# samson6460/tf2_YOLO

Hardware: AMD Instinct MI355X
Metric: images/sec training YOLOv3 416x416 bs=32/GPU (higher is better)
Workload: dtype f32-storage/fp16x2-mfma

## Files before the change

include/yolo_hip.h:

```cpp
#ifndef YOLO_HIP_H_
#define YOLO_HIP_H_

#include <stddef.h>
#include <stdint.h>

#ifdef __cplusplus
extern "C" {
#endif

typedef enum yolo_status {
  YOLO_OK = 0,
  YOLO_ERR_INVALID_ARG = -1,
  YOLO_ERR_LAUNCH = -2,
  YOLO_ERR_WORKSPACE = -3
} yolo_status;

enum { YOLO_ACT_LINEAR = 0, YOLO_ACT_LEAKY = 1, YOLO_ACT_MISH = 2 };
enum { YOLO_HEAD_V3 = 3, YOLO_HEAD_V2 = 2, YOLO_HEAD_V1 = 1, YOLO_HEAD_V4 = 4 };
enum { YOLO_NMS_HARD = 1, YOLO_NMS_SOFT = 2, YOLO_NMS_DIOU = 3 };

const char* yolo_last_error(void);
int yolo_abi_version(void);
int yolo_device_available(void);
int yolo_mfma_probe(const void* operands_f16, float* sink, int workgroups, int iters, double* flops_host, void* stream);

enum { YOLO_OPT_CONV_WIN = 0, YOLO_OPT_STAMPS = 1, YOLO_OPT_CONV_SK = 2, YOLO_OPT_CONV_PATCH = 5, YOLO_OPT_WGRAD_WIN = 6,
       YOLO_OPT_NMS_WALK = 7 ,
       YOLO_OPT_AB = 8  };
int yolo_set_option(int key, int value);
const char* yolo_last_conv_kernel(int* launches_host);
size_t yolo_conv_workspace_bytes(void);
int yolo_set_conv_workspace(void* p, size_t bytes, void* stream);
int yolo_set_debug_buffer(void* p, size_t bytes);

typedef struct yolo_conv_desc {
  int N, H, W, Cin;
  int Cout, kh, kw;
  int Ho, Wo;
  int sh, sw;
  int pad_t, pad_l;
} yolo_conv_desc;

#define YOLO_BN_STAT_SLOTS 64
#define YOLO_BN_RED_SLOTS 512
#define YOLO_SPLIT_BATCH_UNITS 4

int yolo_conv2d_fwd(const yolo_conv_desc* d, const float* x, const float* w,
                    const float* bias, float* y, double* stats, void* stream);
int yolo_conv2d_fwd_absmax(const yolo_conv_desc* d, const float* x, const float* w, const float* bias,
                           float* y, double* stats, unsigned* absmax, void* stream);

int yolo_conv2d_dgrad(const yolo_conv_desc* d, const float* dy, const float* wT,
                      float* dx, int accumulate, void* stream);

int yolo_conv2d_wgrad(const yolo_conv_desc* d, const float* x, const float* dy,
                      float* dw, float* dbias, void* stream);

int yolo_conv2d_wgrad_bias(const float* dy, long long P, int Cout, float* dbias, void* stream);

int yolo_filter_transpose(const float* w, float* wT, int Cout, int taps, int Cin, void* stream);

size_t yolo_planes_bytes(long long rows, int C);
int yolo_split_planes(const float* x, long long rows, int C, void* planes, void* stream);
int yolo_split_planes_padded(const float* x, long long rows, int C_src, int C, void* planes, void* stream);

int yolo_split_planes_batch(const void* jobs, int njobs, long long total_blocks, void* stream);
int yolo_filter_transpose_batch(const void* jobs, int njobs, long long total_blocks, void* stream);

int yolo_conv2d_fwd_planes(const yolo_conv_desc* d, const void* x_planes, const void* w_planes,
                           const float* bias, float* y, double* stats, unsigned* absmax, void* stream);
int yolo_conv2d_dgrad_planes(const yolo_conv_desc* d, const void* dy_planes, const void* wT_planes,
                             float* dx, int accumulate, void* stream);
enum { YOLO_EPI_NONE = 0, YOLO_EPI_AFFINE = 1, YOLO_EPI_AFFINE_LEAKY = 2, YOLO_EPI_AFFINE_MISH = 3 };
int yolo_conv2d_fwd_planes_epi(const yolo_conv_desc* d, const void* x_planes, const void* w_planes, const float* bias,
                               int epilogue, const float* scale, const float* shift, const float* residual, float* y,
                               unsigned* absmax, void* stream);
int yolo_split_planes_absmax(const float* x, long long rows, int C, const unsigned* absmax, const float* extra_bound,
                             void* planes, float* out_bound, void* stream);
#define YOLO_INFER_BOUND_WORDS 4096
int yolo_conv_pred_bound(const float* w, int Cout, int kdim, const float* scale, const float* shift, const float* bias,
                         float* pred2, void* stream);
int yolo_conv2d_fwd_infer_unit(const yolo_conv_desc* d, const void* x_planes, const void* w_planes, const float* bias,
                               int epilogue, const float* scale, const float* shift, const float* residual, float* y,
                               unsigned* absmax, const float* pred2, const void* in_bound, int in_n,
                               const void* residual_bound, int residual_n, void* out_planes, unsigned* out_words,
                               float* out_bound, int* out_n_host, void* stream);
int yolo_fold_bound(const void* words, int n, float* out_bound, void* stream);
int yolo_absmax_words(const float* x, long long n, unsigned* words, int* n_words_host, void* stream);
int yolo_stem_filter_prep(const float* w, const float* bias, float* wt, void* stream);
int yolo_stem_fwd_infer_unit(const yolo_conv_desc* d, const float* x, const float* wt, int epilogue, const float* scale,
                             const float* shift, const float* pred2, const void* in_bound, int in_n, float* y,
                             void* out_planes, unsigned* out_words, int* out_n_host, void* stream);
int yolo_split_planes_concat(const float* const* srcs_host, const int* channels_host, const float* const* bounds_host,
                             int nsrc, long long rows, void* planes, float* dst32, float* out_bound, void* stream);
int yolo_split_planes_concat_ex(const float* const* srcs_host, const int* channels_host, const float* const* bounds_host,
                                const int* bound_words_host, const int* upsample_host, int H, int W, int nsrc,
                                long long rows, void* planes, float* dst32, float* out_bound, void* stream);
int yolo_conv2d_fwd_head_unit(const yolo_conv_desc* d, const void* x_planes, const void* w_planes, const float* bias,
                              int A, int C, int version, const float* anchors, float* t, float* y, void* stream);
enum { YOLO_PREC_F32 = 0, YOLO_PREC_F16 = 1 };
int yolo_conv2d_fwd_planes_ex(const yolo_conv_desc* d, const void* x_planes, const void* w_planes, const float* bias,
                              float* y, double* stats, unsigned* absmax, int precision, void* stream);
int yolo_conv2d_fwd_planes_epi_ex(const yolo_conv_desc* d, const void* x_planes, const void* w_planes, const float* bias,
                                  int epilogue, const float* scale, const float* shift, const float* residual, float* y,
                                  unsigned* absmax, int precision, void* stream);
int yolo_conv2d_fwd_infer_unit_ex(const yolo_conv_desc* d, const void* x_planes, const void* w_planes, const float* bias,
                                  int epilogue, const float* scale, const float* shift, const float* residual, float* y,
                                  unsigned* absmax, const float* pred2, const void* in_bound, int in_n,
                                  const void* residual_bound, int residual_n, void* out_planes, unsigned* out_words,
                                  float* out_bound, int* out_n_host, int precision, void* stream);
int yolo_conv2d_fwd_head_unit_ex(const yolo_conv_desc* d, const void* x_planes, const void* w_planes, const float* bias,
                                 int A, int C, int version, const float* anchors, float* t, float* y, int precision,
                                 void* stream);
int yolo_conv2d_wgrad_planes(const yolo_conv_desc* d, const void* x_planes, const void* dy_planes,
                             float* dw, void* stream);

size_t yolo_wgrad_workspace_bytes(void);
int yolo_set_wgrad_workspace(void* p, size_t bytes);


int yolo_bn_stats(const float* x, long long P, int C, double* stats, void* stream);

int yolo_bn_finalize(double* stats, long long P, int C, const float* gamma, const float* beta,
                     float eps, float momentum, int unbiased_moving_var,
                     float* moving_mean, float* moving_var,
                     float* scale, float* shift, float* save_mean, float* save_invstd,
                     void* stream);

int yolo_bn_fold_inference(int C, const float* gamma, const float* beta,
                           const float* moving_mean, const float* moving_var, float eps,
                           float* scale, float* shift, void* stream);

int yolo_bn_act_fwd(const float* x, long long P, int C, const float* scale, const float* shift,
                    int act, const float* residual, float* out, void* stream);

int yolo_bn_act_bwd_reduce(const float* x, const float* dout, long long P, int C,
                           const float* scale, const float* shift,
                           const float* save_mean, const float* save_invstd,
                           int act, double* red, void* stream);
int yolo_bn_act_bwd_apply(const float* x, const float* dout, long long P, int C,
                          const float* gamma, const float* scale, const float* shift,
                          const float* save_mean, const float* save_invstd,
                          int act, double* red, float* dgamma, float* dbeta,
                          float* dx, void* stream);

int yolo_bn_finalize_bound(double* stats, long long P, int C, const float* gamma, const float* beta, float eps,
                           float momentum, int unbiased_moving_var, float* moving_mean, float* moving_var,
// ... 18 lines not shown
int yolo_bn_act_bwd_reduce_bound(const float* x, const float* dout, long long P, int C, const float* scale,
                                 const float* shift, const float* save_mean, const float* save_invstd,
                                 int act, double* red, unsigned* bound_aux, void* stream);
size_t yolo_stem_bwd_scratch_bytes(void);
int yolo_stem_bn_bwd_wgrad(const yolo_conv_desc* d, const float* y, const float* dout, const float* image, const float* scale,
                           const float* shift, const float* save_mean, const float* save_invstd, int act, const double* red,
                           float* dgamma, float* dbeta, float* dw, void* scratch, size_t scratch_bytes, void* stream);
int yolo_bn_act_bwd_apply_planes(const float* x, const float* dout, long long P, int C, const float* gamma,
                                 const float* scale, const float* shift, const float* save_mean,
                                 const float* save_invstd, int act, double* red, float* dgamma, float* dbeta,
                                 float* dx, void* planes, const unsigned* bound_aux, void* stream);
int yolo_bn_act_bwd_reduce_bound_ld(const float* x, const float* dout, long long ld_dout, long long P, int C,
                                    const float* scale, const float* shift, const float* save_mean,
                                    const float* save_invstd, int act, double* red, unsigned* bound_aux, void* stream);
#define YOLO_BN_FOLD_TICKET_WORDS 36
int yolo_bn_act_bwd_reduce_fold_ld(const float* x, const float* dout, long long ld_dout, long long P, int C,
                                   const float* scale, const float* shift, const float* save_mean,
                                   const float* save_invstd, int act, double* red, unsigned* bound_aux,
                                   unsigned* tickets, void* stream);
int yolo_bn_act_bwd_apply_planes_ld(const float* x, const float* dout, long long ld_dout, long long P, int C,
                                    const float* gamma, const float* scale, const float* shift, const float* save_mean,
                                    const float* save_invstd, int act, double* red, float* dgamma, float* dbeta,
                                    float* dx, void* planes, const unsigned* bound_aux, void* stream);

int yolo_bnred_slots_cap(const yolo_conv_desc* d);
int yolo_conv2d_dgrad_planes_bnred(const yolo_conv_desc* d, const void* dy_planes, const void* wT_planes, float* dx,
                                   int accumulate, const float* y, const float* scale, const float* shift,
                                   const float* save_mean, const float* save_invstd, int act, float* partials,
                                   int slots_cap, unsigned* bound_aux, int* nslots, void* stream);
int yolo_bn_act_bwd_sum_partials(const float* partials, int nslots, long long P, int C, const float* scale, double* red,
                                 unsigned* bound_aux, void* stream);

int yolo_act_fwd(const float* x, long long n, int act, float* out, void* stream);
int yolo_act_bwd(const float* x, const float* dout, long long n, int act, float* dx, void* stream);

int yolo_copy_channels_in(const float* src, long long P, int Csrc, float* dst, int Cdst,
                          int c_off, void* stream);
int yolo_copy_channels_out(const float* src, long long P, int Csrc, int c_off, float* dst,
                           int Cdst, int accumulate, void* stream);
int yolo_upsample2x_fwd(const float* x, int N, int H, int W, int C, float* y, int Cy, int c_off,
                        void* stream);
int yolo_upsample2x_bwd(const float* dy, int N, int H, int W, int C, int Cy, int c_off, float* dx,
                        int accumulate, void* stream);
int yolo_axpy(float* a, const float* b, long long n, void* stream);
int yolo_maxpool_fwd(const float* x, int N, int H, int W, int C, int k, int s, int pad_t, int pad_l,
                     int Ho, int Wo, float* y, int Cy, int c_off, int* argmax, void* stream);
int yolo_maxpool_bwd(const float* dy, int N, int Ho, int Wo, int C, int Cy, int c_off,
                     const int* argmax, float* dx, void* stream);
int yolo_maxpool_bwd_same(const float* dy, int N, int H, int W, int C, int Cy, int c_off, const int* argmax, int k,
                          int pad_t, int pad_l, float* dx, void* stream);
int yolo_maxpool2x2_bwd(const float* dy, int N, int Ho, int Wo, int C, const int* argmax, float* dx, int accumulate,
                        void* stream);
int yolo_space_to_depth2_fwd(const float* x, int N, int H, int W, int C, float* y, int Cy, int c_off,
                             void* stream);
int yolo_space_to_depth2_bwd(const float* dy, int N, int H, int W, int C, int Cy, int c_off, float* dx,
                             int accumulate, void* stream);

int yolo_head_act_fwd(const float* t, long long P, int A, int C, int version,
                      const float* anchors, float* y, void* stream);
int yolo_head_act_bwd(const float* y, const float* dy, long long P, int A, int C, int version,
                      const float* anchors, float* dt, float* danchors, void* stream);

typedef struct yolo_loss_cfg {
  int version;
  int N, gh, gw, A, C;
  float anchors[32];
  int   use_anchors;
  float binary_weight;
  float loss_weight[4];
  float ignore_thresh;
  int   use_focal_loss;
  float focal_gamma;
  int   use_scale;
  float wh_reg_weight;
  float truth_thresh;
  float label_smooth;
} yolo_loss_cfg;

size_t yolo_loss_workspace_bytes(const yolo_loss_cfg* cfg);
int yolo_loss_fwd_bwd(const yolo_loss_cfg* cfg, const float* y_true, const float* y_pred,
                      double* loss_out, float* dpred, float grad_scale,
                      void* workspace, size_t workspace_bytes, void* stream);

int yolo_metrics(const yolo_loss_cfg* cfg, const float* y_true, const float* y_pred,
                 float recall_thresh, double* out, void* stream);

int yolo_gap_fwd(const float* x, int N, int H, int W, int C, float* g, void* stream);
int yolo_gap_bwd(const float* dg, int N, int H, int W, int C, float* dx, int accumulate, void* stream);
int yolo_dense_softmax_fwd(const float* g, const float* W, const float* b, int N, int C, int K, float* logits, float* p,
                           void* stream);
int yolo_dense_softmax_bwd(const float* dp, const float* p, const float* g, const float* W, int N, int C, int K, float* dz,
                           float* dg, float* dW, float* db, void* stream);
int yolo_cce_fwd_bwd(const float* t, const float* p, int N, int K, double* loss_out, float* dpred, float grad_scale,
                     void* stream);
int yolo_bn_act_any_fwd(const float* y, long long P, int C, const float* gamma, const float* beta, float* moving_mean,
                        float* moving_var, const float* mean_offset, float eps, float momentum, int unbiased_moving_var,
                        int training, int act, float* scale, float* shift, float* save_mean, float* save_invstd, float* out,
                        void* stream);
int yolo_bn_act_any_bwd(const float* y, const float* dout, long long P, int C, const float* gamma, const float* scale,
                        const float* shift, const float* save_mean, const float* save_invstd, int act, float* dgamma,
                        float* dbeta, float* dy, void* stream);
int yolo_categorical_accuracy(const float* t, const float* p, int N, int K, double* out, void* stream);

int yolo_adam_step(float* p, float* g, float* m, float* v, long long n, float lr, float beta1,
                   float beta2, float eps, int step, float grad_scale, int zero_grad, void* stream);
float yolo_adam_lr_t(float lr, float beta1, float beta2, int step);
int yolo_adam_step_dev(float* p, float* g, float* m, float* v, long long n, const float* hyper, int zero_grad, void* stream);
int yolo_sgd_step(float* p, float* g, long long n, float lr, float grad_scale, int zero_grad,
                  void* stream);
int yolo_fill(float* p, long long n, float value, void* stream);

size_t yolo_grad_sqnorm_workspace_bytes(int n_chunks);
int yolo_grad_sqnorm(const float* g, const long long* chunk_off, const int* chunk_len, int n_chunks,
                     const int* var_first, int n_vars, double* var_sq, double* total_sq, void* workspace,
                     size_t workspace_bytes, void* stream);
int yolo_clip_factors(const double* var_sq, int n_vars, const double* total_sq, const double* total_sq_extra,
                      const float* hyper, int mode, float* factors, float* norm_out, void* stream);
int yolo_adam_step_clip(float* p, float* g, float* m, float* v, float* vhat, const long long* chunk_off,
                        const int* chunk_len, const int* chunk_var, int n_chunks, const float* hyper,
                        const float* factors, int clip_mode, int zero_grad, void* stream);
int yolo_sgd_step_clip(float* p, float* g, float* accum, int nesterov, const long long* chunk_off,
                       const int* chunk_len, const int* chunk_var, int n_chunks, const float* hyper,
                       const float* factors, int clip_mode, int zero_grad, void* stream);

int yolo_decode_level(const float* pred, int gh, int gw, int A, int C, int version,
                      float threshold, double* rows_out, int max_rows, int* count,
                      void* workspace, size_t workspace_bytes, void* stream);
int yolo_decode_level_f64(const double* pred, int gh, int gw, int A, int C, int version,
                          double threshold, double* rows_out, int max_rows, int* count,
                          void* workspace, size_t workspace_bytes, void* stream);
size_t yolo_decode_workspace_bytes(int gh, int gw, int A, int C);

size_t yolo_nms_workspace_bytes(int n, int class_num);
int yolo_nms(const double* rows, int n, int class_num, int mode, double nms_threshold,
             double conf_threshold, double sigma, unsigned char* keep_out,
             void* workspace, size_t workspace_bytes, void* stream);
int yolo_nms_select(const double* rows, int n, int class_num, int mode, double nms_threshold, double conf_threshold,
                    double sigma, unsigned char* keep_out, double* rows_out, int* count_out, void* workspace,
                    size_t workspace_bytes, void* stream);

size_t yolo_decode_batch_workspace_bytes(int levels, const int* gh, const int* gw, const int* A, int C, int B);
int yolo_decode_batch_count(const void* const* preds, const int* is_f64, int levels, int B, const int* gh, const int* gw,
                            const int* A, int C, int version, const double* thresholds, int* img_off, void* workspace,
                            size_t workspace_bytes, void* stream);
int yolo_decode_batch_write(const void* const* preds, const int* is_f64, int levels, int B, const int* gh, const int* gw,
                            const int* A, int C, int version, const double* thresholds, double* rows_out, int max_rows,
                            void* workspace, size_t workspace_bytes, void* stream);
size_t yolo_nms_batch_workspace_bytes(int n, int B, int class_num);
int yolo_nms_batch_prepare(const double* rows, int n, const int* img_off, int B, int class_num, long long* mask_words_out,
                           void* workspace, size_t workspace_bytes, void* stream);
int yolo_nms_batch_select(const double* rows, int n, int B, int class_num, int mode, double nms_threshold,
                          double conf_threshold, double sigma, void* mask, long long mask_words, unsigned char* keep_out,
                          double* rows_out, int* kept_off_out, void* workspace, size_t workspace_bytes, void* stream);

int yolo_cal_iou(const void* xywh_true, const void* xywh_pred, void* out, void* out2, int is_f64, int mode, int ndim,
                 const long long* shape_host, const long long* true_strides_host, const long long* pred_strides_host,
                 double grid_w, double grid_h, void* stream);


int yolo_match_detections(const double* gt_rows, int ngt, const double* det_rows, int ndet, int class_num,
                          double iou_threshold, int* best_gt, unsigned char* matched, double* best_iou,
                          unsigned char* gt_flags, long long* class_counts, void* stream);

int yolo_rank_desc(const double* key, const int* segment, int n, int* rank, void* stream);

size_t yolo_pr_curve_workspace_bytes(int n, int num_gts);
// ... 21 lines not shown
```

tf2_yolo_amd/_lib.py:

```python
import ctypes
import os
from ctypes import (POINTER, Structure, c_char_p, c_double, c_float, c_int, c_longlong,
                    c_size_t, c_void_p)

from . import tape as _tape

_HERE = os.path.dirname(os.path.abspath(__file__))
LIB_PATH = os.path.join(_HERE, "libyolo_hip.so")

ACT_LINEAR, ACT_LEAKY, ACT_MISH = 0, 1, 2
PREC_F32, PREC_F16 = 0, 1
_PRECISIONS = {"fp32": PREC_F32, "fp16": PREC_F16}


def precision_enum(precision):
    try:
        return _PRECISIONS[precision]
    except (KeyError, TypeError):
        raise ValueError(f"precision must be 'fp32' or 'fp16', got {precision!r}") from None
NMS_HARD, NMS_SOFT, NMS_DIOU = 1, 2, 3


class YoloHipError(RuntimeError):
    pass


class ConvDesc(Structure):
    _fields_ = [(n, c_int) for n in
                ("N", "H", "W", "Cin", "Cout", "kh", "kw", "Ho", "Wo", "sh", "sw", "pad_t", "pad_l")]


class LossCfg(Structure):
    _fields_ = [("version", c_int), ("N", c_int), ("gh", c_int), ("gw", c_int), ("A", c_int),
                ("C", c_int), ("anchors", c_float * 32), ("use_anchors", c_int),
                ("binary_weight", c_float), ("loss_weight", c_float * 4),
                ("ignore_thresh", c_float), ("use_focal_loss", c_int), ("focal_gamma", c_float),
                ("use_scale", c_int), ("wh_reg_weight", c_float), ("truth_thresh", c_float),
                ("label_smooth", c_float)]


_P = c_void_p
_LL = c_longlong
SIGNATURES = {
    "yolo_last_error": (c_char_p, []),
    "yolo_abi_version": (c_int, []),
    "yolo_device_available": (c_int, []),
    "yolo_set_option": (c_int, [c_int, c_int]),
    "yolo_last_conv_kernel": (c_char_p, [POINTER(c_int)]),
    "yolo_mfma_probe": (c_int, [_P, _P, c_int, c_int, POINTER(c_double), _P]),
    "yolo_set_debug_buffer": (c_int, [_P, c_size_t]),
    "yolo_encode_labels": (c_int, [_P, _P, _P, c_int, c_double, c_double, c_int, c_int, c_int, _P, _P, _P]),
    "yolo_down2xlabel": (c_int, [_P, c_int, c_int, c_int, c_int, _P, _P, _P]),
    "yolo_conv_workspace_bytes": (c_size_t, []),
    "yolo_set_conv_workspace": (c_int, [_P, c_size_t, _P]),
    "yolo_conv2d_fwd": (c_int, [POINTER(ConvDesc), _P, _P, _P, _P, _P, _P]),
    "yolo_conv2d_dgrad": (c_int, [POINTER(ConvDesc), _P, _P, _P, c_int, _P]),
    "yolo_conv2d_wgrad": (c_int, [POINTER(ConvDesc), _P, _P, _P, _P, _P]),
    "yolo_conv2d_wgrad_bias": (c_int, [_P, _LL, c_int, _P, _P]),
    "yolo_filter_transpose": (c_int, [_P, _P, c_int, c_int, c_int, _P]),
    "yolo_planes_bytes": (c_size_t, [_LL, c_int]),
    "yolo_split_planes": (c_int, [_P, _LL, c_int, _P, _P]),
    "yolo_split_planes_padded": (c_int, [_P, _LL, c_int, c_int, _P, _P]),
    "yolo_split_planes_batch": (c_int, [_P, c_int, _LL, _P]),
    "yolo_filter_transpose_batch": (c_int, [_P, c_int, _LL, _P]),
    "yolo_conv2d_fwd_planes": (c_int, [POINTER(ConvDesc), _P, _P, _P, _P, _P, _P, _P]),
    "yolo_stem_bwd_scratch_bytes": (c_size_t, []),
    "yolo_stem_bn_bwd_wgrad": (c_int, [POINTER(ConvDesc), _P, _P, _P, _P, _P, _P, _P, c_int, _P, _P, _P, _P, _P, c_size_t, _P]),
    "yolo_conv2d_fwd_planes_epi": (c_int, [POINTER(ConvDesc), _P, _P, _P, c_int, _P, _P, _P, _P, _P, _P]),
    "yolo_split_planes_absmax": (c_int, [_P, _LL, c_int, _P, _P, _P, _P, _P]),
    "yolo_conv_pred_bound": (c_int, [_P, c_int, c_int, _P, _P, _P, _P, _P]),
    "yolo_conv2d_fwd_infer_unit": (c_int, [POINTER(ConvDesc), _P, _P, _P, c_int, _P, _P, _P, _P, _P, _P, _P, c_int, _P, c_int,
                                           _P, _P, _P, POINTER(c_int), _P]),
    "yolo_fold_bound": (c_int, [_P, c_int, _P, _P]),
    "yolo_absmax_words": (c_int, [_P, _LL, _P, POINTER(c_int), _P]),
    "yolo_stem_filter_prep": (c_int, [_P, _P, _P, _P]),
    "yolo_stem_fwd_infer_unit": (c_int, [POINTER(ConvDesc), _P, _P, c_int, _P, _P, _P, _P, c_int, _P, _P, _P, POINTER(c_int), _P]),
    "yolo_split_planes_concat": (c_int, [POINTER(c_void_p), POINTER(c_int), POINTER(c_void_p), c_int, _LL, _P, _P, _P, _P]),
    "yolo_split_planes_concat_ex": (c_int, [POINTER(c_void_p), POINTER(c_int), POINTER(c_void_p), POINTER(c_int), POINTER(c_int),
                                            c_int, c_int, c_int, _LL, _P, _P, _P, _P]),
    "yolo_conv2d_fwd_head_unit": (c_int, [POINTER(ConvDesc), _P, _P, _P, c_int, c_int, c_int, _P, _P, _P, _P]),
    "yolo_conv2d_fwd_planes_ex": (c_int, [POINTER(ConvDesc), _P, _P, _P, _P, _P, _P, c_int, _P]),
    "yolo_conv2d_fwd_planes_epi_ex": (c_int, [POINTER(ConvDesc), _P, _P, _P, c_int, _P, _P, _P, _P, _P, c_int, _P]),
    "yolo_conv2d_fwd_infer_unit_ex": (c_int, [POINTER(ConvDesc), _P, _P, _P, c_int, _P, _P, _P, _P, _P, _P, _P, c_int, _P, c_int,
                                              _P, _P, _P, POINTER(c_int), c_int, _P]),
    "yolo_conv2d_fwd_head_unit_ex": (c_int, [POINTER(ConvDesc), _P, _P, _P, c_int, c_int, c_int, _P, _P, _P, c_int, _P]),
    "yolo_conv2d_fwd_absmax": (c_int, [POINTER(ConvDesc), _P, _P, _P, _P, _P, _P, _P]),
    "yolo_conv2d_dgrad_planes": (c_int, [POINTER(ConvDesc), _P, _P, _P, c_int, _P]),
    "yolo_conv2d_wgrad_planes": (c_int, [POINTER(ConvDesc), _P, _P, _P, _P]),
    "yolo_wgrad_workspace_bytes": (c_size_t, []),
    "yolo_set_wgrad_workspace": (c_int, [_P, c_size_t]),
    "yolo_bn_stats": (c_int, [_P, _LL, c_int, _P, _P]),
    "yolo_bn_finalize": (c_int, [_P, _LL, c_int, _P, _P, c_float, c_float, c_int, _P, _P, _P, _P, _P, _P, _P]),
    "yolo_bn_fold_inference": (c_int, [c_int, _P, _P, _P, _P, c_float, _P, _P, _P]),
    "yolo_bn_act_fwd": (c_int, [_P, _LL, c_int, _P, _P, c_int, _P, _P, _P]),
    "yolo_bn_act_bwd_reduce": (c_int, [_P, _P, _LL, c_int, _P, _P, _P, _P, c_int, _P, _P]),
    "yolo_bn_act_bwd_apply": (c_int, [_P, _P, _LL, c_int, _P, _P, _P, _P, _P, c_int, _P, _P, _P, _P, _P]),
    "yolo_bn_act_fwd_planes": (c_int, [_P, _LL, c_int, _P, _P, c_int, _P, _P, _P, _P, _P, _P, _P]),
    "yolo_bn_act_fwd_res_planes": (c_int, [_P, _LL, c_int, _P, _P, c_int, _P, _P, _P, _P, _P, _P]),
    "yolo_bn_act_bwd_apply_planes": (c_int, [_P, _P, _LL, c_int, _P, _P, _P, _P, _P, c_int, _P, _P, _P, _P, _P, _P,
                                             _P]),
    "yolo_bn_infer_bound": (c_int, [c_int, _P, _P, _P, _P, _P]),
    "yolo_bn_finalize_bound": (c_int, [_P, _LL, c_int, _P, _P, c_float, c_float, c_int, _P, _P, _P, _P, _P, _P, _P,
                                       _P, _P]),
    "yolo_bn_finalize_offset": (c_int, [_P, _LL, c_int, _P, _P, c_float, c_float, c_int, _P, _P, _P, _P, _P, _P, _P,
                                        _P, _P, _P]),
    "yolo_bn_act_bwd_reduce_bound": (c_int, [_P, _P, _LL, c_int, _P, _P, _P, _P, c_int, _P, _P, _P]),
    "yolo_bn_act_bwd_reduce_bound_ld": (c_int, [_P, _P, _LL, _LL, c_int, _P, _P, _P, _P, c_int, _P, _P, _P]),
    "yolo_bn_act_bwd_reduce_fold_ld": (c_int, [_P, _P, _LL, _LL, c_int, _P, _P, _P, _P, c_int, _P, _P, _P, _P]),
    "yolo_bn_act_bwd_apply_planes_ld": (c_int, [_P, _P, _LL, _LL, c_int, _P, _P, _P, _P, _P, c_int, _P, _P, _P, _P, _P, _P,
                                                _P]),
    "yolo_bnred_slots_cap": (c_int, [POINTER(ConvDesc)]),
    "yolo_conv2d_dgrad_planes_bnred": (c_int, [POINTER(ConvDesc), _P, _P, _P, c_int, _P, _P, _P, _P, _P, c_int, _P, c_int, _P,
                                               POINTER(c_int), _P]),
    "yolo_bn_act_bwd_sum_partials": (c_int, [_P, c_int, _LL, c_int, _P, _P, _P, _P]),
    "yolo_allreduce_bucket": (c_int, [_P, _P, _LL, _P]),
    "yolo_act_fwd": (c_int, [_P, _LL, c_int, _P, _P]),
    "yolo_act_bwd": (c_int, [_P, _P, _LL, c_int, _P, _P]),
    "yolo_copy_channels_in": (c_int, [_P, _LL, c_int, _P, c_int, c_int, _P]),
    "yolo_copy_channels_out": (c_int, [_P, _LL, c_int, c_int, _P, c_int, c_int, _P]),
    "yolo_upsample2x_fwd": (c_int, [_P, c_int, c_int, c_int, c_int, _P, c_int, c_int, _P]),
    "yolo_upsample2x_bwd": (c_int, [_P, c_int, c_int, c_int, c_int, c_int, c_int, _P, c_int, _P]),
    "yolo_axpy": (c_int, [_P, _P, _LL, _P]),
    "yolo_maxpool_fwd": (c_int, [_P, c_int, c_int, c_int, c_int, c_int, c_int, c_int, c_int, c_int, c_int,
                                 _P, c_int, c_int, _P, _P]),
    "yolo_maxpool_bwd": (c_int, [_P, c_int, c_int, c_int, c_int, c_int, c_int, _P, _P, _P]),
    "yolo_maxpool2x2_bwd": (c_int, [_P, c_int, c_int, c_int, c_int, _P, _P, c_int, _P]),
    "yolo_bn_act_maxpool2x2_fwd": (c_int, [_P, c_int, c_int, c_int, c_int, _P, _P, c_int, _P, _P, _P, _P, _P, _P]),
    "yolo_maxpool_bwd_same": (c_int, [_P, c_int, c_int, c_int, c_int, c_int, c_int, _P, c_int, c_int, c_int, _P, _P]),
    "yolo_space_to_depth2_fwd": (c_int, [_P, c_int, c_int, c_int, c_int, _P, c_int, c_int, _P]),
    "yolo_space_to_depth2_bwd": (c_int, [_P, c_int, c_int, c_int, c_int, c_int, c_int, _P, c_int, _P]),
    "yolo_head_act_fwd": (c_int, [_P, _LL, c_int, c_int, c_int, _P, _P, _P]),
    "yolo_head_act_bwd": (c_int, [_P, _P, _LL, c_int, c_int, c_int, _P, _P, _P, _P]),
    "yolo_loss_workspace_bytes": (c_size_t, [POINTER(LossCfg)]),
    "yolo_loss_fwd_bwd": (c_int, [POINTER(LossCfg), _P, _P, _P, _P, c_float, _P, c_size_t, _P]),
    "yolo_metrics": (c_int, [POINTER(LossCfg), _P, _P, c_float, _P, _P]),
    "yolo_gap_fwd": (c_int, [_P, c_int, c_int, c_int, c_int, _P, _P]),
    "yolo_gap_bwd": (c_int, [_P, c_int, c_int, c_int, c_int, _P, c_int, _P]),
    "yolo_dense_softmax_fwd": (c_int, [_P, _P, _P, c_int, c_int, c_int, _P, _P, _P]),
    "yolo_dense_softmax_bwd": (c_int, [_P, _P, _P, _P, c_int, c_int, c_int, _P, _P, _P, _P, _P]),
    "yolo_bn_act_any_fwd": (c_int, [_P, _LL, c_int, _P, _P, _P, _P, _P, c_float, c_float, c_int, c_int, c_int, _P, _P, _P, _P, _P,
                                    _P]),
    "yolo_bn_act_any_bwd": (c_int, [_P, _P, _LL, c_int, _P, _P, _P, _P, _P, c_int, _P, _P, _P, _P]),
    "yolo_cce_fwd_bwd": (c_int, [_P, _P, c_int, c_int, _P, _P, c_float, _P]),
    "yolo_categorical_accuracy": (c_int, [_P, _P, c_int, c_int, _P, _P]),
    "yolo_adam_step": (c_int, [_P, _P, _P, _P, _LL, c_float, c_float, c_float, c_float, c_int, c_float, c_int, _P]),
    "yolo_adam_lr_t": (c_float, [c_float, c_float, c_float, c_int]),
    "yolo_adam_step_dev": (c_int, [_P, _P, _P, _P, _LL, _P, c_int, _P]),
    "yolo_sgd_step": (c_int, [_P, _P, _LL, c_float, c_float, c_int, _P]),
    "yolo_fill": (c_int, [_P, _LL, c_float, _P]),
    "yolo_grad_sqnorm_workspace_bytes": (c_size_t, [c_int]),
    "yolo_grad_sqnorm": (c_int, [_P, _P, _P, c_int, _P, c_int, _P, _P, _P, c_size_t, _P]),
    "yolo_clip_factors": (c_int, [_P, c_int, _P, _P, _P, c_int, _P, _P, _P]),
    "yolo_adam_step_clip": (c_int, [_P, _P, _P, _P, _P, _P, _P, _P, c_int, _P, _P, c_int, c_int, _P]),
    "yolo_sgd_step_clip": (c_int, [_P, _P, _P, c_int, _P, _P, _P, c_int, _P, _P, c_int, c_int, _P]),
    "yolo_decode_level": (c_int, [_P, c_int, c_int, c_int, c_int, c_int, c_float, _P, c_int, _P, _P, c_size_t, _P]),
    "yolo_decode_level_f64": (c_int, [_P, c_int, c_int, c_int, c_int, c_int, c_double, _P, c_int, _P, _P,
                                      c_size_t, _P]),
    "yolo_decode_workspace_bytes": (c_size_t, [c_int, c_int, c_int, c_int]),
    "yolo_nms_workspace_bytes": (c_size_t, [c_int, c_int]),
    "yolo_cal_iou": (c_int, [_P, _P, _P, _P, c_int, c_int, c_int, POINTER(c_longlong), POINTER(c_longlong),
                             POINTER(c_longlong), c_double, c_double, _P]),
    "yolo_match_detections": (c_int, [_P, c_int, _P, c_int, c_int, c_double, _P, _P, _P, _P, _P, _P]),
    "yolo_rank_desc": (c_int, [_P, _P, c_int, _P, _P]),
    "yolo_pr_curve_workspace_bytes": (c_size_t, [c_int, c_int]),
    "yolo_pr_curve": (c_int, [_P, _P, _P, c_int, c_int, c_int, _P, c_size_t, _P, _P, _P]),
    "yolo_nms": (c_int, [_P, c_int, c_int, c_int, c_double, c_double, c_double, _P, _P, c_size_t, _P]),
    "yolo_nms_select": (c_int, [_P, c_int, c_int, c_int, c_double, c_double, c_double, _P, _P, _P, _P, c_size_t, _P]),
    "yolo_decode_batch_workspace_bytes": (c_size_t, [c_int, POINTER(c_int), POINTER(c_int), POINTER(c_int), c_int, c_int]),
    "yolo_decode_batch_count": (c_int, [POINTER(c_void_p), POINTER(c_int), c_int, c_int, POINTER(c_int), POINTER(c_int),
                                        POINTER(c_int), c_int, c_int, POINTER(c_double), _P, _P, c_size_t, _P]),
    "yolo_decode_batch_write": (c_int, [POINTER(c_void_p), POINTER(c_int), c_int, c_int, POINTER(c_int), POINTER(c_int),
                                        POINTER(c_int), c_int, c_int, POINTER(c_double), _P, c_int, _P, c_size_t, _P]),
    "yolo_nms_batch_workspace_bytes": (c_size_t, [c_int, c_int, c_int]),
    "yolo_nms_batch_prepare": (c_int, [_P, c_int, _P, c_int, c_int, _P, _P, c_size_t, _P]),
    "yolo_nms_batch_select": (c_int, [_P, c_int, c_int, c_int, c_int, c_double, c_double, c_double, _P, _LL, _P, _P, _P, _P,
                                      c_size_t, _P]),
    "yolo_image_prepare": (c_int, [_P, _LL, _P, c_int, c_int, c_int, c_float, c_float, _P, _P]),
}

_lib = None

_QUERIES = {"yolo_last_error", "yolo_last_conv_kernel", "yolo_abi_version", "yolo_bnred_slots_cap", "yolo_device_available", "yolo_conv_workspace_bytes", "yolo_planes_bytes",
            "yolo_stem_bwd_scratch_bytes", "yolo_loss_workspace_bytes", "yolo_decode_workspace_bytes",
            "yolo_nms_workspace_bytes", "yolo_pr_curve_workspace_bytes", "yolo_wgrad_workspace_bytes", "yolo_adam_lr_t",
            "yolo_grad_sqnorm_workspace_bytes", "yolo_decode_batch_workspace_bytes", "yolo_nms_batch_workspace_bytes",
            "yolo_set_option", "yolo_set_debug_buffer", "yolo_set_conv_workspace", "yolo_set_wgrad_workspace"}


class _Recorded:
    __slots__ = ("f", "name")

    def __init__(self, f, name):
        self.f, self.name = f, name

    def __call__(self, *a):
        rc = self.f(*a)
        if _tape.ACTIVE is not None:
            _tape.ACTIVE.c(self.f, a, self.name)
        return rc


class _Lib:

    def __init__(self, cdll):
        self._cdll = cdll

    def __getattr__(self, name):
        f = getattr(self._cdll, name)
        if name not in _QUERIES and name in SIGNATURES:
            f = _Recorded(f, name)
        setattr(self, name, f)
        return f


def load():
    global _lib
    if _lib is not None:
# ... 26 lines not shown
```

tf2_yolo_amd/capture.py:

```python
import torch

from ._lib import YoloHipError


_LEAKED = []


class _StaticInputs:

    def __init__(self, x, y_list):
        self.x = x.clone()
        self.ys = [y.clone() for y in y_list]
        self._last = [(x, x._version)] + [(y, y._version) for y in y_list]

    def load(self, x, y_list):
        for i, (dst, src) in enumerate(zip([self.x] + self.ys, [x] + list(y_list))):
            last, ver = self._last[i]
            if src is last and src._version == ver:
                continue
            dst.copy_(src, non_blocking=True)
            self._last[i] = (src, src._version)


class StepGraphs:

    def __init__(self, model, x, y_list):
        self.model = model
        self.key = self.key_of(model, x)
        net = model.net
        opt = model.optimizer
        if not getattr(opt, "capturable", False):
            raise YoloHipError("this optimizer has no capturable form")
        self.inputs = _StaticInputs(x, y_list)
        self.x, self.ys = self.inputs.x, self.inputs.ys
        self.segments = []
        opt._hyper_buffers()
        net.mark_params_changed()
        torch.cuda.synchronize()
        self._capture(net, opt)

    @staticmethod
    def key_of(model, x):
        return (tuple(x.shape), getattr(model.net, "alloc_gen", 0), tuple(id(l) for l in model.loss), id(model.optimizer),
                id(model._reducer), model.net.anchors_trainable)

    def _capture(self, net, opt):
        model = self.model
        red = model._reducer if (model._reducer is not None and model._reducer.active) else None
        pool = torch.cuda.graph_pool_handle()
        stream = torch.cuda.Stream()
        stream.wait_stream(torch.cuda.current_stream())
        state = {"g": None}

        def begin():
            g = torch.cuda.CUDAGraph()
            g.capture_begin(pool=pool, capture_error_mode="thread_local")
            state["g"] = g

        def end(action):
            state["g"].capture_end()
            self.segments.append((state["g"], action))
            state["g"] = None

        net._dyp_events = [None, None]
        net._wp_event = net._wT_event = None
        old_hook, old_overlap = net.grad_ready_hook, net._overlap_wgrad
        net._overlap_wgrad = False
        if red is not None:
            index = model._dp_unit_index

            def cut_hook(u):
                for b in red.closes[index[id(u)]]:
                    net._join_wgrad()
                    net._dyp_events = [None, None]
                    end(("reduce", b))
                    begin()
            net.grad_ready_hook = cut_hook
        try:
            with torch.cuda.stream(stream):
                begin()
                outs = net.forward(self.x, training=True)
                for i, (o, yt) in enumerate(zip(outs, self.ys)):
                    model.loss[i].fwd_bwd(yt, o, grad_scale=1.0, dpred=model._dpred[i], loss_out=model._loss_bufs[i])
                net.backward(model._dpred)
                net._dyp_events = [None, None]
                if red is not None:
                    end(("finish",))
                    begin()
                opt.step_captured()
                end(None)
        except Exception:
            _LEAKED.extend(g for g, _ in self.segments)
            if state["g"] is not None:
                _LEAKED.append(state["g"])
                try:
                    if net._wgrad_stream is not None:
                        torch.cuda.current_stream().wait_stream(net._wgrad_stream)
                    state["g"].capture_end()
                except Exception:
                    pass
            self.segments = []
            net._dyp_events = [None, None]
            net._wp_event = net._wT_event = None
            net._wgrad_pending = False
            raise
        finally:
            net.grad_ready_hook = old_hook
            net._overlap_wgrad = old_overlap
        torch.cuda.current_stream().wait_stream(stream)
        net.mark_params_changed()

    def replay(self, x, y_list):
        model, net, opt = self.model, self.model.net, self.model.optimizer
        red = model._reducer if (model._reducer is not None and model._reducer.active) else None
        self.inputs.load(x, y_list)
        opt.refresh_hyper(grad_scale=(1.0 / red.world) if red is not None else 1.0)
        for g, action in self.segments:
            g.replay()
            if action is None:
                continue
            if action[0] == "reduce":
                red.reduce_bucket(action[1])
            else:
                if net.anchors_trainable and red.world > 1:
                    import torch.distributed as dist
                    dist.all_reduce(net.anchor_grads, group=red.pg)
                red.finish()
        net.mark_params_changed()
        return model._loss_bufs


class StepTape:

    def __init__(self, model, x, y_list):
        from . import tape as tape_mod
        self.model = model
        self.key = StepGraphs.key_of(model, x)
        opt, net = model.optimizer, model.net
        if not getattr(opt, "capturable", False):
            raise YoloHipError("this optimizer has no capturable form")
        self.inputs = _StaticInputs(x, y_list)
        self.x, self.ys = self.inputs.x, self.inputs.ys
        opt._hyper_buffers()
        red = model._reducer if (model._reducer is not None and model._reducer.active) else None
        net._dyp_events = [None, None]
        net.mark_params_changed()
        self.tape = tape_mod.Tape()
        opt.refresh_hyper(grad_scale=(1.0 / red.world) if red is not None else 1.0)
        tape_mod.ACTIVE = self.tape
        try:
            outs = net.forward(self.x, training=True)
            for i, (o, yt) in enumerate(zip(outs, self.ys)):
                model.loss[i].fwd_bwd(yt, o, grad_scale=1.0, dpred=model._dpred[i], loss_out=model._loss_bufs[i])
            net.backward(model._dpred)
            if red is not None:
                if net.anchors_trainable and red.world > 1:
                    import torch.distributed as dist
                    tape_mod.host_call(lambda: dist.all_reduce(net.anchor_grads, group=red.pg))
                tape_mod.host_call(red.finish)
            opt.step_captured()
        finally:
            tape_mod.ACTIVE = None
        net.mark_params_changed()

    def replay(self, x, y_list):
        model, net, opt = self.model, self.model.net, self.model.optimizer
        red = model._reducer if (model._reducer is not None and model._reducer.active) else None
        self.inputs.load(x, y_list)
        opt.refresh_hyper(grad_scale=(1.0 / red.world) if red is not None else 1.0)
        self.tape.replay()
        net.mark_params_changed()
        return model._loss_bufs
```

tf2_yolo_amd/csrc/conv.hip:

```cpp
#include "conv_args.hpp"
#include <cstdlib>
#include <type_traits>

namespace yolo {

template <int BM, int BN, int WGM, int WGN, bool FLAT>
__global__ __launch_bounds__(256) void gather_conv_kernel(const GatherConvArgs a) {
  constexpr int BK = 32;
  constexpr int LD = BK + 4;
  constexpr int TM = BM / WGM / 32;
  constexpr int TN = BN / WGN / 32;
  constexpr int AR = BM / 32;
  constexpr int BR = BN / 32;
  static_assert(WGM * WGN == 4, "4 waves per block");
  static_assert(TM >= 1 && TN >= 1, "wave tile");

  extern __shared__ __attribute__((aligned(16))) float smem[];
  constexpr int BUF = (BM + BN) * LD;

  const int tid = threadIdx.x;
  const int lane = tid & 63;
  const int wave = tid >> 6;
  const int wm = wave / WGN, wn = wave % WGN;

// ... 980 lines not shown
                                           const float* const* bounds_host, const int* bound_words_host,
                                           const int* upsample_host, int H, int W, int nsrc, long long rows, void* planes,
                                           float* dst32, float* out_bound, void* stream) {
  YOLO_REQUIRE(srcs_host && channels_host && bounds_host && planes && nsrc >= 1 && nsrc <= 4 && rows > 0,
               "split_planes_concat: 1..4 sources, non-null tables");
  int C = 0;
  bool any_up = false;
  for (int i = 0; i < nsrc; ++i) {
    YOLO_REQUIRE(srcs_host[i] && bounds_host[i] && channels_host[i] > 0 && (channels_host[i] % 8) == 0,
                 "split_planes_concat: every source needs a pointer, a bound and a channel count that is a multiple of 8");
    YOLO_REQUIRE(bound_words_host == nullptr || (bound_words_host[i] >= 1 && bound_words_host[i] <= YOLO_INFER_BOUND_WORDS),
                 "split_planes_concat: a bound is 1..%d words", YOLO_INFER_BOUND_WORDS);
    any_up = any_up || (upsample_host != nullptr && upsample_host[i] != 0);
    C += channels_host[i];
  }
  YOLO_REQUIRE((C % 16) == 0, "split_planes_concat: the concatenated channel count must be a multiple of 16");
  YOLO_REQUIRE(!any_up || (H > 0 && W > 0 && (H % 2) == 0 && (W % 2) == 0 && rows % ((long long)H * W) == 0),
               "split_planes_concat: an upsampled source needs even H, W with rows = N * H * W (H=%d W=%d rows=%lld)", H, W, rows);
  return launch_split_planes_concat(srcs_host, channels_host, bounds_host, nsrc, rows, planes, dst32, out_bound,
                                    as_stream(stream), bound_words_host, upsample_host, H, W);
}

extern "C" int yolo_conv2d_fwd_head_unit(const yolo_conv_desc* d, const void* x_planes, const void* w_planes,
                                         const float* bias, int A, int C, int version, const float* anchors, float* t,
                                         float* y, void* stream) {
  return yolo_conv2d_fwd_head_unit_ex(d, x_planes, w_planes, bias, A, C, version, anchors, t, y, YOLO_PREC_F32, stream);
}

extern "C" int yolo_conv2d_fwd_head_unit_ex(const yolo_conv_desc* d, const void* x_planes, const void* w_planes,
                                            const float* bias, int A, int C, int version, const float* anchors, float* t,
                                            float* y, int precision, void* stream) {
  if (int rc = validate_desc(d)) return rc;
  YOLO_REQUIRE_PRECISION(precision, "conv_fwd_head_unit");
  YOLO_REQUIRE(x_planes && w_planes && t && y && A > 0 && C > 0, "conv_fwd_head_unit: bad args");
  YOLO_REQUIRE(d->Cout == A * (5 + C), "conv_fwd_head_unit: Cout = %d is not A (5 + C) = %d", d->Cout, A * (5 + C));
  GatherConvArgs a{};
  a.src = reinterpret_cast<const float*>(x_planes);
  a.wgt = reinterpret_cast<const float*>(w_planes);
  a.bias = bias;
  a.dst = t;
  fill_fwd_args(d, a);
  a.one_pass = precision == YOLO_PREC_F16;
  YOLO_REQUIRE(gather_planes_supported(a), "conv_fwd_head_unit: needs Cin %% 16 == 0 and Cout >= 32");
  if ((version == YOLO_HEAD_V3 || version == YOLO_HEAD_V4) && anchors != nullptr) {
    a.head_y = y;
    a.head_anchors = anchors;
    a.head_A = A;
    a.head_C = C;
    if (conv_small_head_supported(a)) {
      int nwg = 0;
      return launch_conv_small(a, as_stream(stream), &nwg);
    }
    a.head_y = nullptr;
  }
  if (int rc = launch_gather_planes(a, as_stream(stream))) return rc;
  return yolo_head_act_fwd(t, (long long)d->N * d->Ho * d->Wo, A, C, version, anchors, y, stream);
}

extern "C" size_t yolo_planes_bytes(long long rows, int C) {
  if (rows <= 0 || C <= 0 || (C % 16) != 0) return 0;
  return (size_t)planes_bytes(rows, C);
}

extern "C" int yolo_split_planes_batch(const void* jobs, int njobs, long long total_blocks, void* stream) {
  YOLO_REQUIRE(jobs, "split_planes_batch: null job table");
  return launch_split_planes_batch(jobs, njobs, total_blocks, as_stream(stream));
}

extern "C" int yolo_filter_transpose_batch(const void* jobs, int njobs, long long total_blocks, void* stream) {
  YOLO_REQUIRE(jobs, "filter_transpose_batch: null job table");
  return launch_filter_transpose_batch(jobs, njobs, total_blocks, as_stream(stream));
}

extern "C" int yolo_split_planes(const float* x, long long rows, int C, void* planes, void* stream) {
  YOLO_REQUIRE(x && planes, "split_planes: null pointer");
  return launch_split_planes(x, rows, C, planes, as_stream(stream));
}

extern "C" int yolo_split_planes_padded(const float* x, long long rows, int C_src, int C, void* planes, void* stream) {
  YOLO_REQUIRE(x && planes, "split_planes_padded: null pointer");
  return launch_split_planes_padded(x, rows, C_src, C, planes, as_stream(stream));
}

struct BnRedArgs {
  const float* y;
  const float* scale;
  const float* shift;
  const float* mean;
  const float* invstd;
  int act;
  float* part;
  int cap;
  unsigned* aux;
  int nslots;
};
static void set_bnred(GatherConvArgs& a, const BnRedArgs* b) {
  if (b == nullptr) return;
  a.bwd_y = b->y; a.bwd_scale = b->scale; a.bwd_shift = b->shift; a.bwd_mean = b->mean; a.bwd_invstd = b->invstd;
  a.bwd_act = b->act; a.bwd_part = b->part; a.bwd_cap = b->cap; a.bwd_aux = b->aux;
}

static int dgrad_impl(const yolo_conv_desc* d, const float* dy, const float* wT, float* dx, int accumulate,
                      void* stream, bool planes, BnRedArgs* bnred = nullptr) {
  if (int rc = validate_desc(d)) return rc;
  YOLO_REQUIRE(dy && wT && dx, "conv_dgrad: null pointer");
  const bool flat = (d->Cout % 32) != 0;
  YOLO_REQUIRE(!flat || (d->kh == 1 && d->kw == 1 && d->sh == 1 && d->sw == 1),
               "conv_dgrad: Cout %% 32 != 0 only supported for 1x1 stride-1 (head) convs");
  static const bool fuse_classes = env_int("YOLO_DGRAD_CLASSES", 1) != 0;
  if (planes && fuse_classes && d->sh * d->sw > 1 && d->sh * d->sw <= 4) {
    GatherConvArgs a{};
    a.src = dy;
    a.wgt = wT;
    a.dst = dx;
    a.N = d->N; a.Hs = d->Ho; a.Ws = d->Wo; a.Cs = d->Cout;
    a.sy = 1; a.sx = 1;
    a.Hd = d->H; a.Wd = d->W; a.Cd = d->Cin;
    a.osy = d->sh; a.osx = d->sw;
    a.Cout = d->Cin;
    a.ldw = d->kh * d->kw * d->Cout;
    a.accumulate = accumulate;
    a.kw = 1;
    int nt = 0, nc = 0;
    bool ok = true;
    for (int py = 0; py < d->sh && ok; ++py)
      for (int px = 0; px < d->sw && ok; ++px) {
        ClassGeom& c = a.cls[nc++];
        c.Hg = (d->H - py + d->sh - 1) / d->sh;
        c.Wg = (d->W - px + d->sw - 1) / d->sw;
        c.M = (long long)d->N * c.Hg * c.Wg;
        c.ooy = py; c.oox = px; c.tap0 = nt; c.ntaps = 0;
        for (int r = 0; r < d->kh; ++r) {
          const int ty = py + d->pad_t - r;
          if (((ty % d->sh) + d->sh) % d->sh != 0) continue;
          for (int s = 0; s < d->kw; ++s) {
            const int tx = px + d->pad_l - s;
            if (((tx % d->sw) + d->sw) % d->sw != 0) continue;
            a.taps[nt++] = Tap{ty / d->sh, tx / d->sw, (r * d->kw + s) * d->Cout};
            ++c.ntaps;
          }
        }
        if (c.ntaps == 0 || c.Hg <= 0 || c.Wg <= 0) ok = false;
      }
    if (ok) {
      a.ncls = nc;
      a.M = a.cls[0].M; a.Hg = a.cls[0].Hg; a.Wg = a.cls[0].Wg; a.ooy = 0; a.oox = 0; a.ntaps = a.cls[0].ntaps;
      YOLO_REQUIRE(gather_planes_supported(a), "conv_dgrad_planes: needs Cout %% 16 == 0 and Cin >= 32");
      set_bnred(a, bnred);
      const int rc = launch_gather_planes(a, as_stream(stream));
      if (bnred != nullptr) bnred->nslots = a.bwd_nslots;
      return rc;
    }
  }
  YOLO_REQUIRE(bnred == nullptr || d->sh * d->sw == 1,
               "conv_dgrad_planes_bnred: a strided data gradient needs its parity classes in one launch");
  for (int py = 0; py < d->sh; ++py) {
    for (int px = 0; px < d->sw; ++px) {
      GatherConvArgs a{};
      a.src = dy;
      a.wgt = wT;
      a.bias = nullptr;
      a.dst = dx;
      a.N = d->N; a.Hs = d->Ho; a.Ws = d->Wo; a.Cs = d->Cout;
      a.Hg = (d->H - py + d->sh - 1) / d->sh;
      a.Wg = (d->W - px + d->sw - 1) / d->sw;
      if (a.Hg <= 0 || a.Wg <= 0) continue;
// ... 154 lines not shown
```

tf2_yolo_amd/csrc/conv_args.hpp:

```cpp
#pragma once
#include "common.hpp"

namespace yolo {

constexpr int MAX_TAPS = 49;

struct Tap {
  int oy, ox, woff;
};

struct ClassGeom {
  long long M;
  int Hg, Wg, ooy, oox, tap0, ntaps;
};

struct GatherConvArgs {
  const float* src;
  const float* wgt;
  const float* bias;
  float* dst;
  double* stats;
  unsigned* absmax;
  long long M;
  int N, Hs, Ws, Cs;
// ... 10 lines not shown
  int zero_blk_src, zero_blk_wgt;
  int nt_store;
  int vec_store;
  int kc;
  int dbg;
  int one_pass;
  const float* epi_scale;
  const float* epi_shift;
  const float* epi_res;
  int epi_act;
  unsigned char* out_planes;
  const float* pl_pred;
  const unsigned* pl_in_bound;
  const unsigned* pl_res_bound;
  int pl_in_n, pl_res_n;
  unsigned* pl_out_words;
  float* head_y;
  const float* head_anchors;
  int head_A, head_C;
  int sk_grid;
  int tile_order;
  float* sk_slabs;
  unsigned* sk_tickets;
  int split_parts;
  int ncls;
  ClassGeom cls[4];
  unsigned long long* stamps;
  const float* bwd_y;
  const float* bwd_scale;
  const float* bwd_shift;
  const float* bwd_mean;
  const float* bwd_invstd;
  float* bwd_part;
  unsigned* bwd_aux;
  int bwd_act;
  int bwd_nslots;
  int bwd_cap;
  Tap taps[MAX_TAPS];
};

#define YOLO_BNRED_CHECK(a)                                                                                          \
  if ((a).bwd_y != nullptr && (a).bwd_nslots > (a).bwd_cap) {                                                        \
    set_error("conv_dgrad(bn reduce): %d partial slots needed, room for %d", (a).bwd_nslots, (a).bwd_cap);           \
    return YOLO_ERR_INVALID_ARG;                                                                                     \
  }

__device__ __forceinline__ int xcd_remap(int bid, int nblocks) {
  const int xcd = bid & 7, idx = bid >> 3;
  const int q = nblocks >> 3, r = nblocks & 7;
  const int start = (xcd < r) ? xcd * (q + 1) : r * (q + 1) + (xcd - r) * q;
  return start + idx;
}


struct WgradArgs {
  const float* src;
  const float* dy;
  float* dw;
  long long M;
  int N, Hs, Ws, Cs;
  int Hg, Wg;
  int sy, sx;
  int Cout, ldw;
  int ntaps;
  int kw, pad_t, pad_l;
  int tiles_co, tiles_j;
  int nblocks;
  long long chunk;
  unsigned src_bytes, dy_bytes;
  int zero_blk_src, zero_blk_dy;
  float* slabs;
  int splits;
};

int launch_gather_split(GatherConvArgs& a, hipStream_t st);
bool gather_split_supported(const GatherConvArgs& a);
long long planes_bytes(long long rows, int C);
int launch_split_planes(const float* x, long long rows, int C, void* planes, hipStream_t st);
int launch_split_planes_absmax(const float* x, long long rows, int C, const unsigned* absmax, const float* extra_bound, int extra_n,
                               void* planes, float* out_bound, hipStream_t st);
int launch_split_planes_concat(const float* const* xs, const int* Cs, const float* const* bounds, int nsrc, long long rows,
                               void* planes, float* dst32, float* out_bound, hipStream_t st,
                               const int* bound_words = nullptr, const int* upsample = nullptr, int H = 0, int W = 0);
int launch_split_planes_padded(const float* x, long long rows, int Csrc, int C, void* planes, hipStream_t st);
int launch_split_planes_batch(const void* jobs, int njobs, long long total_blocks, hipStream_t st);
int launch_filter_transpose_batch(const void* jobs, int njobs, long long total_blocks, hipStream_t st);
int launch_gather_planes(GatherConvArgs& a, hipStream_t st);
bool conv_small_supported(const GatherConvArgs& a);
bool conv_small_head_supported(const GatherConvArgs& a);
int launch_conv_small(GatherConvArgs& a, hipStream_t st, int* nwg);
bool gather_planes_supported(const GatherConvArgs& a);
int conv_split_parts(const GatherConvArgs& a, long long nb, int bm, int min_cb, int idle_div);
int launch_split_reduce(GatherConvArgs& a, int bm, hipStream_t st);
float* conv_split_slabs();
int launch_conv_win(GatherConvArgs& a, int variant, hipStream_t st);
bool conv_win_supported(const GatherConvArgs& a);
enum { OPT_CONV_WIN = 0, OPT_STAMPS = 1, OPT_CONV_SK = 2, OPT_DBG = 3, OPT_TILE_ORDER = 4, OPT_CONV_PATCH = 5, OPT_WGRAD_WIN = 6, OPT_NMS_WALK = 7, OPT_EXP = 8, OPT_COUNT = 16 };
int set_conv_workspace(void* p, size_t bytes, hipStream_t st);
extern void* g_dbg_buf;
extern size_t g_dbg_bytes;
extern int g_opt[OPT_COUNT];
void init_options();
void note_conv_launch(const char* family, int a = 0, int b = 0, int c = 0, int d = 0);
int launch_wgrad_planes(WgradArgs& a, hipStream_t st);
bool wgrad_planes_supported(const WgradArgs& a);
int launch_wgrad_win(WgradArgs& a, hipStream_t st);
bool wgrad_win_supported(const WgradArgs& a);
constexpr size_t WGRAD_WS_COLSUM_BYTES = 1 << 20;
void* wgrad_workspace(size_t* bytes);
bool stem_fwd_supported(const yolo_conv_desc* d);
struct StemEpiArgs {
  const float* scale;
  const float* shift;
  int act;
  void* planes;
  const float* pred;
  const unsigned* in_words;
  int in_n;
  unsigned* out_words;
};
bool stem_infer_supported(const yolo_conv_desc* d);
int launch_stem_filter_prep(const float* w, const float* bias, float* wt, hipStream_t st);
int launch_absmax_words(const float* x, long long n, unsigned* words, int* n_words, hipStream_t st);
int launch_stem_infer(const yolo_conv_desc* d, const float* x, const float* wt, float* y, const StemEpiArgs& e, int* out_n,
                      hipStream_t st);
size_t stem_bwd_scratch_bytes();
int launch_stem_bn_bwd_wgrad(const yolo_conv_desc* d, const float* y, const float* dout, const float* img, const float* scale,
                             const float* shift, const float* smean, const float* sinv, int act, const double* redsum,
                             float* dgamma, float* dbeta, float* dw, float* scratch, size_t scratch_bytes, hipStream_t st);
int launch_stem_fwd(const yolo_conv_desc* d, const float* x, const float* w, const float* bias, float* y, double* stats,
                    unsigned* absmax, hipStream_t st);
int launch_wgrad_split(WgradArgs& a, hipStream_t st);
bool wgrad_split_supported(const WgradArgs& a);

}
```

tf2_yolo_amd/csrc/conv_planes.hip:

```cpp
#include "planes_epilogue.hpp"
#include <algorithm>
#include <cstdlib>
#include <type_traits>

namespace yolo {

__global__ __launch_bounds__(256) void planes_amax_kernel(const float* __restrict__ x, long long n4,
                                                         unsigned* __restrict__ header) {
  float m = 0.f;
  for (long long i = (long long)blockIdx.x * 256 + threadIdx.x; i < n4; i += (long long)gridDim.x * 256) {
    const f32x4 v = reinterpret_cast<const f32x4*>(x)[i];
    m = fmaxf(fmaxf(m, fmaxf(fabsf(v[0]), fabsf(v[1]))), fmaxf(fabsf(v[2]), fabsf(v[3])));
  }
#pragma unroll
  for (int o = 32; o > 0; o >>= 1) m = fmaxf(m, __shfl_xor(m, o, 64));
  __shared__ float wmax[4];
  if ((threadIdx.x & 63) == 0) wmax[threadIdx.x >> 6] = m;
  __syncthreads();
  if (threadIdx.x == 0) {
    m = fmaxf(fmaxf(wmax[0], wmax[1]), fmaxf(wmax[2], wmax[3]));
    if (__builtin_bit_cast(unsigned, m) > *reinterpret_cast<volatile unsigned*>(header))
      atomicMax(header, __builtin_bit_cast(unsigned, m));
  }
}
// ... 696 lines not shown
  const BatchJob j = jobs[find_job(jobs, njobs, blockIdx.x)];
  const float* x = reinterpret_cast<const float*>(j.src);
  unsigned char* out = reinterpret_cast<unsigned char*>(j.dst);
  const long long rows = j.a;
  const int C = (int)j.b;
  unsigned* header = reinterpret_cast<unsigned*>(out + planes_body_bytes(rows, C));
  const unsigned bound = j.c != 0 ? *reinterpret_cast<const unsigned*>(j.c) : header[0];
  const float sc = planes_scale_from_bound(bound);
  const long long rows_padded = ((rows + 15) / 16 + 1) * 16;
  if ((long long)blockIdx.x == j.first_block && threadIdx.x == 0) {
    header[0] = bound;
    reinterpret_cast<float*>(header)[1] = sc;
    reinterpret_cast<float*>(header)[2] = 1.f / sc;
  }
  const BatchPos p = batch_pos(j);
  if (!p.live) return;
  f32x4 v[BATCH_UNITS][2];
#pragma unroll
  for (int u = 0; u < BATCH_UNITS; ++u) {
    const long long row = p.row0 + 16 * u;
    v[u][0] = v[u][1] = f32x4{0.f, 0.f, 0.f, 0.f};
    if (row < rows) {
      const float* q = x + row * C + p.g * 8;
      v[u][0] = *reinterpret_cast<const f32x4*>(q);
      v[u][1] = *reinterpret_cast<const f32x4*>(q + 4);
    }
  }
#pragma unroll
  for (int u = 0; u < BATCH_UNITS; ++u) {
    const long long row = p.row0 + 16 * u;
    if (row >= rows_padded) continue;
    const Planes8 s8 = split8(v[u][0], v[u][1], sc);
    unsigned char* o = out + planes_unit_offset(row, p.g, C);
    *reinterpret_cast<u32x4*>(o) = s8.h;
    *reinterpret_cast<u32x4*>(o + 512) = s8.l;
  }
}

__global__ __launch_bounds__(256) void filter_transpose_batch_kernel(const BatchJob* __restrict__ jobs, int njobs) {
  __shared__ float tile[32][33];
  const BatchJob j = jobs[find_job(jobs, njobs, blockIdx.x)];
  const float* w = reinterpret_cast<const float*>(j.src);
  float* wT = reinterpret_cast<float*>(j.dst);
  const int Cout = (int)j.a, taps = (int)j.b, Cin = (int)j.c;
  const int bx = (Cin + 31) / 32, by = (Cout + 31) / 32;
  const int lb = (int)((long long)blockIdx.x - j.first_block);
  const int t = lb / (bx * by);
  const int rem = lb - t * (bx * by);
  const int co0 = (rem / bx) * 32, ci0 = (rem % bx) * 32;
  const int tx = threadIdx.x & 31, ty = threadIdx.x >> 5;
  for (int r = ty; r < 32; r += 8) {
    const int co = co0 + r, ci = ci0 + tx;
    tile[r][tx] = (co < Cout && ci < Cin) ? w[((long long)co * taps + t) * Cin + ci] : 0.f;
  }
  __syncthreads();
  for (int r = ty; r < 32; r += 8) {
    const int ci = ci0 + r, co = co0 + tx;
    if (ci < Cin && co < Cout) wT[((long long)ci * taps + t) * Cout + co] = tile[tx][r];
  }
}

int launch_split_planes_batch(const void* jobs, int njobs, long long total_blocks, hipStream_t st) {
  if (njobs <= 0 || total_blocks <= 0 || total_blocks > 0x7fffffffLL) {
    set_error("split_planes_batch: bad job table");
    return YOLO_ERR_INVALID_ARG;
  }
  const BatchJob* jb = reinterpret_cast<const BatchJob*>(jobs);
  hipLaunchKernelGGL(planes_header_clear_batch_kernel, dim3((njobs + 255) / 256), dim3(256), 0, st, jb, njobs);
  hipLaunchKernelGGL(planes_amax_batch_kernel, dim3((unsigned)total_blocks), dim3(256), 0, st, jb, njobs);
  hipLaunchKernelGGL(split_planes_batch_kernel, dim3((unsigned)total_blocks), dim3(256), 0, st, jb, njobs);
  return check_launch("split_planes_batch_kernel");
}

int launch_filter_transpose_batch(const void* jobs, int njobs, long long total_blocks, hipStream_t st) {
  if (njobs <= 0 || total_blocks <= 0 || total_blocks > 0x7fffffffLL) {
    set_error("filter_transpose_batch: bad job table");
    return YOLO_ERR_INVALID_ARG;
  }
  hipLaunchKernelGGL(filter_transpose_batch_kernel, dim3((unsigned)total_blocks), dim3(256), 0, st,
                     reinterpret_cast<const BatchJob*>(jobs), njobs);
  return check_launch("filter_transpose_batch_kernel");
}

int launch_split_planes_padded(const float* x, long long rows, int Csrc, int C, void* planes, hipStream_t st) {
  if (C % 16 != 0 || rows <= 0 || Csrc <= 0 || Csrc > C || C - Csrc >= 16) {
    set_error("split_planes_padded: need 0 < Csrc <= C < Csrc + 16, C %% 16 == 0, rows > 0");
    return YOLO_ERR_INVALID_ARG;
  }
  const long long rows_padded = ((rows + 15) / 16 + 1) * 16;
  const long long blocks = (rows_padded * (C / 8) + 255) / 256;
  if (blocks > 0x7fffffffLL) {
    set_error("split_planes_padded: tensor too large");
    return YOLO_ERR_INVALID_ARG;
  }
  unsigned char* out = reinterpret_cast<unsigned char*>(planes);
  unsigned* header = reinterpret_cast<unsigned*>(out + planes_body_bytes(rows, C));
  if (hipMemsetAsync(header, 0, 16, st) != hipSuccess) {
    set_error("split_planes_padded: hipMemsetAsync failed");
    return YOLO_ERR_LAUNCH;
  }
  const long long n = rows * Csrc, n4 = n / 4;
  if (n4 > 0) hipLaunchKernelGGL(planes_amax_kernel, dim3(stream_grid(n4, 256)), dim3(256), 0, st, x, n4, header);
  if (n > 4 * n4)
    hipLaunchKernelGGL(planes_amax_scalar_kernel, dim3(1), dim3(256), 0, st, x + 4 * n4, n - 4 * n4, header);
  hipLaunchKernelGGL(split_planes_padded_kernel, dim3((unsigned)blocks), dim3(256), 0, st, x, rows, Csrc, C, out,
                     rows_padded);
  return check_launch("split_planes_padded_kernel");
}

int launch_split_planes_absmax(const float* x, long long rows, int C, const unsigned* absmax, const float* extra_bound, int extra_n,
                               void* planes, float* out_bound, hipStream_t st) {
  if (C % 16 != 0 || rows <= 0) {
    set_error("split_planes_absmax: C %% 16 != 0 or rows <= 0");
    return YOLO_ERR_INVALID_ARG;
  }
  const long long rows_padded = ((rows + 15) / 16 + 1) * 16;
  const long long blocks = ((rows_padded / 16 + SPLIT_BLOCKS_PER_WG - 1) / SPLIT_BLOCKS_PER_WG) * ((C / 8 + 15) / 16);
  if (blocks > 0x7fffffffLL) {
    set_error("split_planes_absmax: tensor too large");
    return YOLO_ERR_INVALID_ARG;
  }
  hipLaunchKernelGGL(split_planes_absmax_kernel, dim3((unsigned)blocks), dim3(256), 0, st, x, rows, C, absmax, extra_bound,
                     extra_n, reinterpret_cast<unsigned char*>(planes), rows_padded, out_bound);
  return check_launch("split_planes_absmax_kernel");
}

int launch_split_planes(const float* x, long long rows, int C, void* planes, hipStream_t st) {
  if (C % 16 != 0 || rows <= 0) {
    set_error("split_planes: C %% 16 != 0 or rows <= 0");
    return YOLO_ERR_INVALID_ARG;
  }
  const long long rows_padded = ((rows + 15) / 16 + 1) * 16;
  const long long blocks = ((rows_padded / 16 + SPLIT_BLOCKS_PER_WG - 1) / SPLIT_BLOCKS_PER_WG) * ((C / 8 + 15) / 16);
  if (blocks > 0x7fffffffLL) {
    set_error("split_planes: tensor too large");
    return YOLO_ERR_INVALID_ARG;
  }
  unsigned char* out = reinterpret_cast<unsigned char*>(planes);
  unsigned* header = reinterpret_cast<unsigned*>(out + planes_body_bytes(rows, C));
  if (hipMemsetAsync(header, 0, 16, st) != hipSuccess) {
    set_error("split_planes: hipMemsetAsync failed");
    return YOLO_ERR_LAUNCH;
  }
  const long long n4 = rows * (C / 4);
  hipLaunchKernelGGL(planes_amax_kernel, dim3(stream_grid(n4, 256)), dim3(256), 0, st, x, n4, header);
  hipLaunchKernelGGL(split_planes_kernel, dim3((unsigned)blocks), dim3(256), 0, st, x, rows, C, out, rows_padded);
  return check_launch("split_planes_kernel");
}

}
```

tf2_yolo_amd/csrc/conv_small.hip:

```cpp
#include "act.hpp"
#include "planes.hpp"
#include <cstdlib>

namespace yolo {

constexpr int SM_WAVES = 8;

template <int TM, int TN, int CH, int PASSES = 3>
struct SmallBuf {
  u32x4 ah[CH][TM], al[CH][TM], bh[CH][TN], bl[CH][TN];
};
template <int TM, int TN, int CH>
struct SmallBuf<TM, TN, CH, 1> {
  u32x4 ah[CH][TM], bh[CH][TN];
};

template <int TM, int TN, int NT>
struct SmallLds {
  static constexpr int NB = TM * TN;
  static constexpr int RED = 0;
  static constexpr int T32 = RED + NB * SM_WAVES * 16 * 64 * 4;
  static constexpr int AOFF = T32 + NB * 32 * 33 * 4;
  static constexpr int MX = AOFF + NT * 32 * TM * 4;
  static constexpr int BYTES = MX + 3 * SM_WAVES * 4;
};

template <int NT, int TM, int TN, int CH, bool HEAD = false, int PASSES = 3>
__global__ __launch_bounds__(64 * SM_WAVES) void conv_small_kernel(const GatherConvArgs a) {
  static_assert(planes_passes_ok(PASSES), "1 or 3 MFMA passes");
  constexpr int BMT = 32 * TM, BNT = 32 * TN, NB = TM * TN;
  constexpr int NTASK = (4 * NB + SM_WAVES - 1) / SM_WAVES;
  using LDS = SmallLds<TM, TN, NT>;
  extern __shared__ unsigned char smem[];
  float (*red)[SM_WAVES][16][64] = reinterpret_cast<float (*)[SM_WAVES][16][64]>(smem + LDS::RED);
  float (*t32)[32][33] = reinterpret_cast<float (*)[32][33]>(smem + LDS::T32);
  unsigned (*s_aoff)[BMT] = reinterpret_cast<unsigned (*)[BMT]>(smem + LDS::AOFF);
  float (*s_mx)[SM_WAVES] = reinterpret_cast<float (*)[SM_WAVES]>(smem + LDS::MX);
  const int tid = threadIdx.x, lane = tid & 63;
  const int wave = __builtin_amdgcn_readfirstlane(tid >> 6);
  const int r = lane & 31, hf = lane >> 5;
  const int tiles_m = (int)((a.M + BMT - 1) / BMT);
  const int logical = xcd_remap(blockIdx.x, a.nblocks);
  const int tile_n = logical / tiles_m, tile_m = logical - tile_n * tiles_m;
  const int KB = a.Cs >> 4;
  const int nsteps = NT * KB;
  const unsigned char* srcp = reinterpret_cast<const unsigned char*>(a.src);
  const unsigned char* wgtp = reinterpret_cast<const unsigned char*>(a.wgt);
  const unsigned lane_unit = (unsigned)(hf * 256);
  auto src_row_offset = [&](const long long mp, const int t) -> unsigned {
    long long ms = (long long)a.zero_blk_src * 16 + (mp & 15);
    if (mp < a.M) {
      const int HgWg = a.Hg * a.Wg;
      const int n = (int)(mp / HgWg);
      const int rem = (int)(mp - (long long)n * HgWg);
      const int y = rem / a.Wg, x = rem - y * a.Wg;
      const int ys = y * a.sy + a.taps[t].oy, xs = x * a.sx + a.taps[t].ox;
      if (ys >= 0 && ys < a.Hs && xs >= 0 && xs < a.Ws) ms = ((long long)n * a.Hs + ys) * a.Ws + xs;
    }
    return (unsigned)((ms >> 4) * KB) * PL_RECORD + (unsigned)(ms & 15) * 16;
  };
  unsigned aoff1[TM];
  if constexpr (NT == 1) {
    if (a.sy == 1 && a.sx == 1 && a.Hg == a.Hs && a.Wg == a.Ws && a.taps[0].oy == 0 && a.taps[0].ox == 0) {
#pragma unroll
      for (int i = 0; i < TM; ++i) {
        const long long mp = (long long)tile_m * BMT + 32 * i + r;
        const long long ms = mp < a.M ? mp : (long long)a.zero_blk_src * 16 + (mp & 15);
        aoff1[i] = (unsigned)((ms >> 4) * KB) * PL_RECORD + (unsigned)(ms & 15) * 16 + lane_unit;
      }
    } else {
#pragma unroll
      for (int i = 0; i < TM; ++i) aoff1[i] = src_row_offset((long long)tile_m * BMT + 32 * i + r, 0) + lane_unit;
    }
  } else {
    for (int e = tid; e < NT * BMT; e += 64 * SM_WAVES) {
      const int t = e / BMT, rr = e - t * BMT;
      s_aoff[t][rr] = src_row_offset((long long)tile_m * BMT + rr, t);
    }
  }
  unsigned boff[TN];
#pragma unroll
  for (int j = 0; j < TN; ++j) {
    const int crow = tile_n * BNT + 32 * j + r;
// ... 81 lines not shown
#pragma unroll
    for (int u = 0; u < CH; ++u)
#pragma unroll
      for (int i = 0; i < TM; ++i)
#pragma unroll
        for (int j = 0; j < TN; ++j) {
          const f16x8 ah = __builtin_bit_cast(f16x8, b.ah[u][i]), bh = __builtin_bit_cast(f16x8, b.bh[u][j]);
          if constexpr (PASSES == 3) {
            const f16x8 al = __builtin_bit_cast(f16x8, b.al[u][i]), bl = __builtin_bit_cast(f16x8, b.bl[u][j]);
            acc[i][j] = __builtin_amdgcn_mfma_f32_32x32x16_f16(al, bh, acc[i][j], 0, 0, 0);
            acc[i][j] = __builtin_amdgcn_mfma_f32_32x32x16_f16(ah, bl, acc[i][j], 0, 0, 0);
          }
          acc[i][j] = __builtin_amdgcn_mfma_f32_32x32x16_f16(ah, bh, acc[i][j], 0, 0, 0);
        }
  };
  Buf b0, b1;
  load(b0);
  for (int c = 0; c < nch; c += 2) {
    load(b1);
    mma(b0);
    load(b0);
    mma(b1);
  }

#pragma unroll
  for (int i = 0; i < TM; ++i)
#pragma unroll
    for (int j = 0; j < TN; ++j)
#pragma unroll
      for (int k = 0; k < 16; ++k) red[i * TN + j][wave][k][lane] = acc[i][j][k];
  if constexpr (!HEAD) {
#pragma unroll
    for (int o = 32; o > 0; o >>= 1) {
      ib = fmaxf(ib, __shfl_xor(ib, o, 64));
      rb = fmaxf(rb, __shfl_xor(rb, o, 64));
    }
    if (lane == 0) {
      s_mx[1][wave] = ib;
      s_mx[2][wave] = rb;
    }
  }
  __syncthreads();
  float psc = 1.f;
  if constexpr (!HEAD) {
    float in_b = 0.f, res_b = 0.f;
#pragma unroll
    for (int w = 0; w < SM_WAVES; ++w) {
      in_b = fmaxf(in_b, s_mx[1][w]);
      res_b = fmaxf(res_b, s_mx[2][w]);
    }
    const float bnd = (a.pl_pred[0] * in_b + a.pl_pred[1] + res_b) * 1.001f + 1e-30f;
    psc = planes_scale_from_bound(__builtin_bit_cast(unsigned, bnd));
    if (blockIdx.x == 0 && tid == 0) {
      unsigned* header = reinterpret_cast<unsigned*>(a.out_planes + planes_body_bytes(a.M, a.Cout));
      header[0] = __builtin_bit_cast(unsigned, bnd);
      reinterpret_cast<float*>(header)[1] = psc;
      reinterpret_cast<float*>(header)[2] = 1.f / psc;
    }
  }
  float mxf = 0.f;
  const int D = HEAD ? 5 + a.head_C : 1;
#pragma unroll
  for (int k = 0; k < NTASK; ++k) {
    const int t = wave + SM_WAVES * k;
    if (t < 4 * NB) {
      const int b = t >> 2, q = t & 3, bi = b / TN, bj = b - bi * TN;
      const int col = tile_n * BNT + 32 * bj + r;
      const long long mrow = (long long)tile_m * BMT + 32 * bi + 8 * q + 4 * hf;
      float anc = 0.f;
      int kk = 0;
      if constexpr (HEAD) {
        kk = col % D;
        if (col < a.Cout && (kk == 2 || kk == 3)) anc = a.head_anchors[(col / D) * 2 + (kk - 2)];
      }
#pragma unroll
      for (int e = 0; e < 4; ++e) {
        float sum = red[b][0][4 * q + e][lane];
#pragma unroll
        for (int w = 1; w < SM_WAVES; ++w) sum += red[b][w][4 * q + e][lane];
        if constexpr (HEAD) {
          if (mrow + e < a.M && col < a.Cout) {
            const float v = fmaf(sum, unscale, bv[k]);
            if (a.dst != nullptr) a.dst[(mrow + e) * a.Cd + col] = v;
            a.head_y[(mrow + e) * a.Cd + col] = (kk == 2 || kk == 3) ? expf(v) * anc : 1.f / (1.f + expf(-v));
          }
        } else {
          float v = 0.f;
          if (mrow + e < a.M) {
            v = fmaf(sum, unscale, bv[k]);
            v = act_fwd(fmaf(esc[k], v, esh[k]), a.epi_act);
            v += rv[k][e];
            a.dst[(mrow + e) * a.Cd + col] = v;
            mxf = fmaxf(mxf, fabsf(v));
          }
          t32[b][8 * q + 4 * hf + e][r] = v;
        }
      }
    }
  }
  if constexpr (HEAD) return;
#pragma unroll
  for (int o = 32; o > 0; o >>= 1) mxf = fmaxf(mxf, __shfl_xor(mxf, o, 64));
  if (lane == 0) s_mx[0][wave] = mxf;
  __syncthreads();
  for (int u = tid; u < NB * 128; u += 64 * SM_WAVES) {
    const int b = u >> 7, rr = (u >> 2) & 31, g = u & 3, bi = b / TN, bj = b - bi * TN;
    const long long mo = (long long)tile_m * BMT + 32 * bi + rr;
    const int c0 = tile_n * BNT + 32 * bj + g * 8;
    if (mo < a.M) {
      const f32x4 o0 = {t32[b][rr][g * 8 + 0], t32[b][rr][g * 8 + 1], t32[b][rr][g * 8 + 2], t32[b][rr][g * 8 + 3]};
      const f32x4 o1 = {t32[b][rr][g * 8 + 4], t32[b][rr][g * 8 + 5], t32[b][rr][g * 8 + 6], t32[b][rr][g * 8 + 7]};
      store_planes8(a.out_planes, mo, c0 >> 3, a.Cout, o0, o1, psc);
    }
  }
  if (tid == 0) {
    float m = 0.f;
#pragma unroll
    for (int w = 0; w < SM_WAVES; ++w) m = fmaxf(m, s_mx[0][w]);
    a.pl_out_words[blockIdx.x] = __builtin_bit_cast(unsigned, m);
  }
}

template <int NT, int TM, int TN, int CH, bool HEAD = false>
static bool small_limit_ok() {
  return lds_limit_ok<conv_small_kernel<NT, TM, TN, CH, HEAD>, SmallLds<TM, TN, NT>::BYTES>("conv_small_kernel");
}
static bool small_tile_fits(int ntaps, int tile, bool head) {
  if (head) return tile != 22 ? small_limit_ok<1, 1, 1, 4, true>() : small_limit_ok<1, 2, 2, 2, true>();
  if (ntaps == 1) return tile == 22 ? small_limit_ok<1, 2, 2, 2>() : tile == 21 ? small_limit_ok<1, 2, 1, 4>() : small_limit_ok<1, 1, 1, 4>();
  return tile == 22 ? small_limit_ok<9, 2, 2, 2>() : tile == 21 ? small_limit_ok<9, 2, 1, 4>() : small_limit_ok<9, 1, 1, 4>();
}

static int small_tile_policy(const GatherConvArgs& a) {
  static const int on = env_int("YOLO_CONV_SMALL", 1);
  static const int tile_env = env_int("YOLO_CONV_SMALL_TILE", 0);
  static const int grid_env = env_int("YOLO_CONV_SMALL_GRID", 0);
  if (!on) return 0;
  if (a.ntaps != 1 && a.ntaps != 9) return 0;
  if ((a.Cs % 16) != 0 || (a.Cout % 32) != 0 || a.ldw != a.ntaps * a.Cs) return 0;
  if (a.stats != nullptr || a.accumulate || a.bwd_y != nullptr || a.ncls > 1) return 0;
  if (a.out_planes == nullptr || a.epi_scale == nullptr || a.pl_pred == nullptr || a.pl_out_words == nullptr) return 0;
  if (a.osy != 1 || a.osx != 1 || a.ooy != 0 || a.oox != 0 || a.Hd != a.Hg || a.Wd != a.Wg || a.Cd != a.Cout) return 0;
  for (int t = 0; t < a.ntaps; ++t)
    if (a.taps[t].woff != t * a.Cs) return 0;
  const long long g11 = ((a.M + 31) / 32) * (a.Cout / 32);
  const long long g22 = (a.Cout % 64) == 0 ? ((a.M + 63) / 64) * (a.Cout / 64) : (1LL << 40);
  if (tile_env) {
    const long long cap = grid_env > 0 ? grid_env : 2048;
    if (g11 > (cap < YOLO_INFER_BOUND_WORDS ? cap : YOLO_INFER_BOUND_WORDS)) return 0;
    return (tile_env == 22 && (a.Cout % 64) != 0) ? 21 : tile_env;
  }
  const long long cap = grid_env > 0 ? grid_env : 256;
  if (a.ntaps == 9 && on != 3) {
    const int steps = a.ntaps * (a.Cs >> 4);
    static const int two_rounds = env_int("YOLO_CONV_SMALL_2R", 1);
    return (g22 >= 128 && ((g22 <= cap && steps <= 72) || (two_rounds && g22 <= 2 * cap && steps <= 36))) ? 22 : 0;
  }
  if (g11 <= cap) return 11;
  if (g22 <= cap) return 22;
  return 0;
}

static int small_tile(const GatherConvArgs& a) {
  const int tile = small_tile_policy(a);
  return tile != 0 && small_tile_fits(a.ntaps, tile, false) ? tile : 0;
}

// ... 68 lines not shown
```

tf2_yolo_amd/csrc/elementwise.hip:

```cpp
#include "common.hpp"
#include "planes.hpp"
#include <cfloat>

namespace yolo {

__global__ void copy_in_kernel(const float* __restrict__ src, long long P, int Cs, float* __restrict__ dst, int Cd,
                               int c_off, int vec) {
  if (vec) {
    const int Cs4 = Cs >> 2;
    const long long n = P * Cs4;
    for (long long i = (long long)blockIdx.x * blockDim.x + threadIdx.x; i < n;
         i += (long long)gridDim.x * blockDim.x) {
      const long long p = i / Cs4;
      const int c = (int)(i - p * Cs4) * 4;
      *reinterpret_cast<f32x4*>(dst + p * Cd + c_off + c) = *reinterpret_cast<const f32x4*>(src + p * Cs + c);
    }
  } else {
    const long long n = P * Cs;
    for (long long i = (long long)blockIdx.x * blockDim.x + threadIdx.x; i < n;
         i += (long long)gridDim.x * blockDim.x) {
      const long long p = i / Cs;
      const int c = (int)(i - p * Cs);
      dst[p * Cd + c_off + c] = src[i];
    }
  }
}

__global__ void copy_out_kernel(const float* __restrict__ src, long long P, int Cs, int c_off,
                                float* __restrict__ dst, int Cd, int accumulate, int vec) {
  if (vec) {
    const int Cd4 = Cd >> 2;
    const long long n = P * Cd4;
    for (long long i = (long long)blockIdx.x * blockDim.x + threadIdx.x; i < n;
         i += (long long)gridDim.x * blockDim.x) {
      const long long p = i / Cd4;
      const int c = (int)(i - p * Cd4) * 4;
      f32x4 v = *reinterpret_cast<const f32x4*>(src + p * Cs + c_off + c);
      if (accumulate) {
        const f32x4 o = *reinterpret_cast<const f32x4*>(dst + p * Cd + c);
        v += o;
      }
      *reinterpret_cast<f32x4*>(dst + p * Cd + c) = v;
    }
  } else {
    const long long n = P * Cd;
    for (long long i = (long long)blockIdx.x * blockDim.x + threadIdx.x; i < n;
         i += (long long)gridDim.x * blockDim.x) {
      const long long p = i / Cd;
      const int c = (int)(i - p * Cd);
      float v = src[p * Cs + c_off + c];
      if (accumulate) v += dst[i];
      dst[i] = v;
    }
  }
}

__global__ void upsample_fwd_kernel(const float* __restrict__ x, int N, int H, int W, int C4, float* __restrict__ y,
                                    int Cy, int c_off) {
  const int Ho = 2 * H, Wo = 2 * W;
  const long long n = (long long)N * Ho * Wo * C4;
  for (long long i = (long long)blockIdx.x * blockDim.x + threadIdx.x; i < n; i += (long long)gridDim.x * blockDim.x) {
    const int c = (int)(i % C4);
    long long p = i / C4;
    const int wo = (int)(p % Wo);
    p /= Wo;
    const int ho = (int)(p % Ho);
    const int b = (int)(p / Ho);
    const f32x4 v = *reinterpret_cast<const f32x4*>(x + (((long long)b * H + (ho >> 1)) * W + (wo >> 1)) * (C4 * 4) + c * 4);
    *reinterpret_cast<f32x4*>(y + (((long long)b * Ho + ho) * Wo + wo) * Cy + c_off + c * 4) = v;
  }
}

__global__ void upsample_bwd_kernel(const float* __restrict__ dy, int N, int H, int W, int C4, int Cy, int c_off,
                                    float* __restrict__ dx, int accumulate) {
  const int Ho = 2 * H, Wo = 2 * W;
  const long long n = (long long)N * H * W * C4;
  for (long long i = (long long)blockIdx.x * blockDim.x + threadIdx.x; i < n; i += (long long)gridDim.x * blockDim.x) {
    const int c = (int)(i % C4);
    long long p = i / C4;
    const int w = (int)(p % W);
    p /= W;
    const int h = (int)(p % H);
    const int b = (int)(p / H);
// ... 164 lines not shown
      if ((unsigned)h >= (unsigned)H) continue;
      const int idx = (h * W + wo) * POOL_CG + c;
      const unsigned short ra = rarg[idx];
      if (ra == 0xFFFF) continue;
      const float v = rval[idx];
      if (arg < 0 || v > best) {
        best = v;
        arg = h * W + ra;
      }
    }
    y[(base + p) * Cy + c_off + c0 + c] = best;
    if (argmax) argmax[(base + p) * C + c0 + c] = arg < 0 ? -1 : (int)((base + arg) * C + c0 + c);
  }
}

__global__ __launch_bounds__(256) void maxpool_plane_bwd_kernel(const float* __restrict__ dy, int H, int W, int C, int Cy,
                                                                int c_off, const int* __restrict__ argmax, int k, int pad_t,
                                                                int pad_l, float* __restrict__ dx) {
  extern __shared__ __attribute__((aligned(16))) unsigned char pool_sm[];
  const int HW = H * W, n = HW * POOL_CG;
  float* dyv = reinterpret_cast<float*>(pool_sm);
  unsigned short* win = reinterpret_cast<unsigned short*>(dyv + n);
  const int groups = C / POOL_CG;
  const int b = blockIdx.x / groups, c0 = (blockIdx.x - b * groups) * POOL_CG;
  const long long base = (long long)b * HW;
  for (int e = threadIdx.x; e < n; e += 256) {
    const int p = e / POOL_CG, c = e - p * POOL_CG;
    dyv[e] = dy[(base + p) * Cy + c_off + c0 + c];
    const int a = argmax[(base + p) * C + c0 + c];
    win[e] = (unsigned short)(a < 0 ? 0xFFFF : (int)((long long)a / C - base));
  }
  __syncthreads();
  for (int e = threadIdx.x; e < n; e += 256) {
    const int p = e / POOL_CG, c = e - p * POOL_CG;
    const int h = p / W, w = p - h * W;
    const int ho_lo = h + pad_t - (k - 1) < 0 ? 0 : h + pad_t - (k - 1), ho_hi = h + pad_t >= H ? H - 1 : h + pad_t;
    const int wo_lo = w + pad_l - (k - 1) < 0 ? 0 : w + pad_l - (k - 1), wo_hi = w + pad_l >= W ? W - 1 : w + pad_l;
    float sum = 0.f;
    for (int ho = ho_lo; ho <= ho_hi; ++ho)
      for (int wo = wo_lo; wo <= wo_hi; ++wo) {
        const int idx = (ho * W + wo) * POOL_CG + c;
        if (win[idx] == (unsigned short)p) sum += dyv[idx];
      }
    dx[(base + p) * C + c0 + c] += sum;
  }
}

static bool pool_plane_ok(int H, int W, int C, int k, int s, int Ho, int Wo) {
  static const bool on = env_int("YOLO_POOL_PLANE", 1) != 0;
  return on && s == 1 && Ho == H && Wo == W && k >= 4 && (C % POOL_CG) == 0 && H * W <= 1024;
}

__global__ void s2d_fwd_kernel(const float* __restrict__ x, int N, int H, int W, int C, float* __restrict__ y, int Cy,
                               int c_off) {
  const long long n = (long long)N * H * W * C;
  const int Ho = H >> 1, Wo = W >> 1;
  for (long long i = (long long)blockIdx.x * blockDim.x + threadIdx.x; i < n; i += (long long)gridDim.x * blockDim.x) {
    const int c = (int)(i % C);
    long long p = i / C;
    const int w = (int)(p % W);
    p /= W;
    const int h = (int)(p % H);
    const int b = (int)(p / H);
    y[(((long long)b * Ho + (h >> 1)) * Wo + (w >> 1)) * Cy + c_off + ((h & 1) * 2 + (w & 1)) * C + c] = x[i];
  }
}
__global__ void s2d_bwd_kernel(const float* __restrict__ dy, int N, int H, int W, int C, int Cy, int c_off,
                               float* __restrict__ dx, int accumulate) {
  const long long n = (long long)N * H * W * C;
  const int Ho = H >> 1, Wo = W >> 1;
  for (long long i = (long long)blockIdx.x * blockDim.x + threadIdx.x; i < n; i += (long long)gridDim.x * blockDim.x) {
    const int c = (int)(i % C);
    long long p = i / C;
    const int w = (int)(p % W);
    p /= W;
    const int h = (int)(p % H);
    const int b = (int)(p / H);
    float v = dy[(((long long)b * Ho + (h >> 1)) * Wo + (w >> 1)) * Cy + c_off + ((h & 1) * 2 + (w & 1)) * C + c];
    if (accumulate) v += dx[i];
    dx[i] = v;
  }
}

__device__ __forceinline__ float sigmoid_f(float x) { return 1.f / (1.f + expf(-x)); }

__global__ void head_fwd_pointwise_kernel(const float* __restrict__ t, long long P, int A, int C,
                                          const float* __restrict__ anchors, float* __restrict__ y) {
  const int D = 5 + C;
  const long long n = P * A * D;
  for (long long i = (long long)blockIdx.x * blockDim.x + threadIdx.x; i < n; i += (long long)gridDim.x * blockDim.x) {
    const int k = (int)(i % D);
    const int a = (int)((i / D) % A);
    const float v = t[i];
    float o;
    if (k == 2 || k == 3) o = expf(v) * anchors[a * 2 + (k - 2)];
    else o = sigmoid_f(v);
    y[i] = o;
  }
}

__global__ void head_softmax_fwd_kernel(const float* __restrict__ t, long long groups, int D, int off, int C,
                                        float* __restrict__ y) {
  for (long long g = (long long)blockIdx.x * blockDim.x + threadIdx.x; g < groups;
       g += (long long)gridDim.x * blockDim.x) {
    const float* tp = t + g * D + off;
    float* yp = y + g * D + off;
    float m = -FLT_MAX;
    for (int c = 0; c < C; ++c) m = fmaxf(m, tp[c]);
    float s = 0.f;
    for (int c = 0; c < C; ++c) s += expf(tp[c] - m);
    const float inv = 1.f / s;
    for (int c = 0; c < C; ++c) yp[c] = expf(tp[c] - m) * inv;
  }
}

__global__ void head_sigmoid_fwd_kernel(const float* __restrict__ t, long long P, int D, int nsig,
                                        float* __restrict__ y) {
  const long long n = P * nsig;
  for (long long i = (long long)blockIdx.x * blockDim.x + threadIdx.x; i < n; i += (long long)gridDim.x * blockDim.x) {
    const long long p = i / nsig;
    const int k = (int)(i - p * nsig);
    y[p * D + k] = sigmoid_f(t[p * D + k]);
  }
}

__global__ void head_bwd_pointwise_kernel(const float* __restrict__ y, const float* __restrict__ dy, long long P,
                                          int A, int C, int sigmoid_classes, float* __restrict__ dt) {
  const int D = 5 + C;
  const long long n = P * A * D;
  for (long long i = (long long)blockIdx.x * blockDim.x + threadIdx.x; i < n; i += (long long)gridDim.x * blockDim.x) {
    const int k = (int)(i % D);
    if (k >= 5 && !sigmoid_classes) continue;
    const float yv = y[i], g = dy[i];
    dt[i] = (k == 2 || k == 3) ? g * yv : g * yv * (1.f - yv);
  }
}

__global__ void head_softmax_bwd_kernel(const float* __restrict__ y, const float* __restrict__ dy, long long groups,
                                        int D, int off, int C, float* __restrict__ dt) {
  for (long long g = (long long)blockIdx.x * blockDim.x + threadIdx.x; g < groups;
       g += (long long)gridDim.x * blockDim.x) {
    const float* yp = y + g * D + off;
    const float* gp = dy + g * D + off;
    float* dp = dt + g * D + off;
    float dot = 0.f;
    for (int c = 0; c < C; ++c) dot += gp[c] * yp[c];
    for (int c = 0; c < C; ++c) dp[c] = yp[c] * (gp[c] - dot);
  }
}

__global__ void head_sigmoid_bwd_kernel(const float* __restrict__ y, const float* __restrict__ dy, long long P, int D,
                                        int nsig, float* __restrict__ dt) {
  const long long n = P * nsig;
  for (long long i = (long long)blockIdx.x * blockDim.x + threadIdx.x; i < n; i += (long long)gridDim.x * blockDim.x) {
    const long long p = i / nsig;
    const int k = (int)(i - p * nsig);
    const float yv = y[p * D + k];
    dt[p * D + k] = dy[p * D + k] * yv * (1.f - yv);
  }
}

__global__ void head_danchor_kernel(const float* __restrict__ y, const float* __restrict__ dy, long long P, int A,
                                    int C, const float* __restrict__ anchors, float* __restrict__ danchors) {
  const int D = 5 + C;
  const int slot = blockIdx.y;
  const int a = slot >> 1, j = slot & 1;
  double s = 0.0;
  for (long long p = (long long)blockIdx.x * blockDim.x + threadIdx.x; p < P; p += (long long)gridDim.x * blockDim.x) {
    const long long i = (p * A + a) * D + 2 + j;
    s += (double)dy[i] * (double)y[i];
  }
  s = wave_reduce_sum(s);
  if ((threadIdx.x & 63) == 0) atomicAdd(&danchors[slot], (float)(s / (double)anchors[slot]));
}

__global__ __launch_bounds__(256) void adam_kernel(float* __restrict__ p, float* __restrict__ g,
                                                   float* __restrict__ m, float* __restrict__ v, long long n,
                                                   float lr_t, float b1, float b2, float eps, float gs, int zero,
                                                   const float* __restrict__ hyper) {
  if (hyper != nullptr) {
    lr_t = hyper[0];
    b1 = hyper[1];
    b2 = hyper[2];
    eps = hyper[3];
    gs = hyper[4];
  }
  const long long n4 = n >> 2;
  for (long long i = (long long)blockIdx.x * blockDim.x + threadIdx.x; i < n4; i += (long long)gridDim.x * blockDim.x) {
    f32x4 pv = reinterpret_cast<f32x4*>(p)[i];
    f32x4 gv = reinterpret_cast<f32x4*>(g)[i];
    f32x4 mv = reinterpret_cast<f32x4*>(m)[i];
    f32x4 vv = reinterpret_cast<f32x4*>(v)[i];
#pragma unroll
    for (int e = 0; e < 4; ++e) {
      const float gg = gv[e] * gs;
      mv[e] = b1 * mv[e] + (1.f - b1) * gg;
      vv[e] = b2 * vv[e] + (1.f - b2) * gg * gg;
      pv[e] -= lr_t * mv[e] / (sqrtf(vv[e]) + eps);
    }
    reinterpret_cast<f32x4*>(p)[i] = pv;
    reinterpret_cast<f32x4*>(m)[i] = mv;
    reinterpret_cast<f32x4*>(v)[i] = vv;
    if (zero) reinterpret_cast<f32x4*>(g)[i] = f32x4{0.f, 0.f, 0.f, 0.f};
  }
  for (long long i = (n4 << 2) + (long long)blockIdx.x * blockDim.x + threadIdx.x; i < n;
       i += (long long)gridDim.x * blockDim.x) {
    const float gg = g[i] * gs;
    const float mm = b1 * m[i] + (1.f - b1) * gg;
    const float vv = b2 * v[i] + (1.f - b2) * gg * gg;
    m[i] = mm;
    v[i] = vv;
    p[i] -= lr_t * mm / (sqrtf(vv) + eps);
    if (zero) g[i] = 0.f;
  }
}

__global__ void sgd_kernel(float* __restrict__ p, float* __restrict__ g, long long n, float lr, float gs, int zero) {
// ... 246 lines not shown
```

tf2_yolo_amd/csrc/loss.hip:

```cpp
#include "common.hpp"
#include "conv_args.hpp"
#include <cfloat>
#include <cstdlib>

namespace yolo {

constexpr float LEPS = 1e-7f;
constexpr float ONE_M_EPS = (float)(1.0 - 1e-7);

struct D4 {
  float v;
  float d[4];
};
__device__ __forceinline__ D4 dconst(float v) { return D4{v, {0.f, 0.f, 0.f, 0.f}}; }
__device__ __forceinline__ D4 dvar(float v, int i) {
  D4 r = dconst(v);
  r.d[i] = 1.f;
  return r;
}
__device__ __forceinline__ D4 operator+(const D4& a, const D4& b) {
  D4 r{a.v + b.v, {}};
  for (int i = 0; i < 4; ++i) r.d[i] = a.d[i] + b.d[i];
  return r;
}
__device__ __forceinline__ D4 operator-(const D4& a, const D4& b) {
  D4 r{a.v - b.v, {}};
  for (int i = 0; i < 4; ++i) r.d[i] = a.d[i] - b.d[i];
  return r;
}
__device__ __forceinline__ D4 operator*(const D4& a, const D4& b) {
  D4 r{a.v * b.v, {}};
  for (int i = 0; i < 4; ++i) r.d[i] = a.d[i] * b.v + a.v * b.d[i];
  return r;
}
__device__ __forceinline__ D4 operator/(const D4& a, const D4& b) {
  D4 r{a.v / b.v, {}};
  for (int i = 0; i < 4; ++i) r.d[i] = a.d[i] / b.v - (a.v / b.v) / b.v * b.d[i];
  return r;
}
__device__ __forceinline__ D4 dmax(const D4& x, const D4& y) { return (x.v >= y.v) ? x : y; }
__device__ __forceinline__ D4 dmin(const D4& x, const D4& y) { return (x.v <= y.v) ? x : y; }
__device__ __forceinline__ D4 dsq(const D4& a) {
  D4 r{a.v * a.v, {}};
  for (int i = 0; i < 4; ++i) r.d[i] = 2.f * a.v * a.d[i];
  return r;
}
__device__ __forceinline__ D4 datan(const D4& a) {
  D4 r{atanf(a.v), {}};
  const float g = 1.f / (1.f + a.v * a.v);
  for (int i = 0; i < 4; ++i) r.d[i] = g * a.d[i];
  return r;
}

struct IouOut {
  D4 iou;
  D4 ciou;
};

template <bool CIOU>
__device__ __forceinline__ IouOut iou_dual(const float* T, const float* P, float gw, float gh) {
  const D4 px = dvar(P[0], 0), py = dvar(P[1], 1), pw = dvar(P[2], 2), ph = dvar(P[3], 3);
  const D4 cx = px / dconst(gw), cy = py / dconst(gh);
  const float tcx = T[0] / gw, tcy = T[1] / gh, tw = T[2], th = T[3];
  const float thw = tw / 2.f, thh = th / 2.f;
  const float tminx = tcx - thw, tmaxx = tcx + thw, tminy = tcy - thh, tmaxy = tcy + thh;
  const D4 hw = pw / dconst(2.f), hh = ph / dconst(2.f);
  const D4 minx = cx - hw, maxx = cx + hw, miny = cy - hh, maxy = cy + hh;
  const D4 iminx = dmax(minx, dconst(tminx)), iminy = dmax(miny, dconst(tminy));
  const D4 imaxx = dmin(maxx, dconst(tmaxx)), imaxy = dmin(maxy, dconst(tmaxy));
  const D4 iw = dmax(imaxx - iminx, dconst(0.f)), ih = dmax(imaxy - iminy, dconst(0.f));
  const D4 inter = iw * ih;
  const float tarea = tw * th;
  const D4 parea = pw * ph;
  const D4 uni = parea + dconst(tarea) - inter;
  IouOut o;
  o.iou = inter / (uni + dconst(LEPS));
  o.ciou = o.iou;
  if constexpr (CIOU) {
    const D4 eminx = dmin(minx, dconst(tminx)), eminy = dmin(miny, dconst(tminy));
    const D4 emaxx = dmax(maxx, dconst(tmaxx)), emaxy = dmax(maxy, dconst(tmaxy));
    const D4 ewx = emaxx - eminx, ewy = emaxy - eminy;
    const D4 c2 = dsq(ewx) + dsq(ewy);
    const D4 rho2 = dsq(dconst(tcx) - cx) + dsq(dconst(tcy) - cy);
    const float atan_t = atanf(tw / (th + LEPS));
// ... 91 lines not shown
      const float lo = obj * ((1.f - p) * (1.f - p));
      const float ln = noobj * (p * p);
      part[3] += (double)lo;
      part[4] += (double)ln;
      part[0] += (double)c.loss_weight[2] * ((double)lo + (double)c.binary_weight * (double)ln);
      g = c.loss_weight[2] * (-2.f * obj * (1.f - p) + 2.f * c.binary_weight * noobj * p);
    } else if (VER == 3) {
      const float cc = fminf(fmaxf(p, LEPS), ONE_M_EPS);
      const float pass = (p >= LEPS && p <= ONE_M_EPS) ? 1.f : 0.f;
      const float gm = c.focal_gamma;
      const bool g2 = gm == 2.f;
      const float a1 = g2 ? (1.f - cc) * (1.f - cc) : powf(1.f - cc, gm), l1 = logf(cc);
      const float a0 = g2 ? cc * cc : powf(cc, gm), l0 = logf(1.f - cc);
      const float lo = -obj * a1 * l1;
      const float ln = -noobj * a0 * l0;
      part[3] += (double)lo;
      part[4] += (double)ln;
      part[0] += (double)c.loss_weight[2] * ((double)lo + (double)c.binary_weight * (double)ln);
      const float d1 = -obj * (-gm * (g2 ? (1.f - cc) : powf(1.f - cc, gm - 1.f)) * l1 + a1 / cc);
      const float d0 = -noobj * (gm * (g2 ? cc : powf(cc, gm - 1.f)) * l0 - a0 / (1.f - cc));
      g = c.loss_weight[2] * (d1 + c.binary_weight * d0) * pass;
    } else {
      const float cc = fminf(fmaxf(p, LEPS), ONE_M_EPS);
      const float pass = (p >= LEPS && p <= ONE_M_EPS) ? 1.f : 0.f;
      const float gm = c.focal_gamma;
      float eo, en, deo, den;
      float omo, omn;
      if (c.label_smooth > 0.f) {
        const float uo = 1.f - c.label_smooth - cc;
        const float un = c.label_smooth - cc;
        eo = fabsf(uo);
        en = fabsf(un);
        deo = (uo > 0.f) ? -1.f : (uo < 0.f ? 1.f : 0.f);
        den = (un > 0.f) ? -1.f : (un < 0.f ? 1.f : 0.f);
        omo = 1.f - eo;
        omn = 1.f - en;
      } else {
        eo = 1.f - cc;
        en = cc;
        deo = -1.f;
        den = 1.f;
        omo = cc;
        omn = 1.f - cc;
      }
      const bool g2 = gm == 2.f;
      const float ao = g2 ? eo * eo : powf(eo, gm), lo_ = logf(omo);
      const float an_ = g2 ? en * en : powf(en, gm), ln_ = logf(omn);
      const float lo = -obj * ao * lo_;
      const float ln = -noobj * an_ * ln_;
      part[3] += (double)lo;
      part[4] += (double)ln;
      part[0] += (double)c.loss_weight[1] * ((double)lo + (double)c.binary_weight * (double)ln);
      const float dfo = gm * (g2 ? eo : powf(eo, gm - 1.f)) * lo_ - ao / omo;
      const float dfn = gm * (g2 ? en : powf(en, gm - 1.f)) * ln_ - an_ / omn;
      g = c.loss_weight[1] * (-obj * dfo * deo - c.binary_weight * noobj * dfn * den) * pass;
    }
  } else {
    const float tk = tk_cur;
    const float pc = fminf(fmaxf(p, LEPS), ONE_M_EPS);
    const float pass = (p >= LEPS && p <= ONE_M_EPS) ? 1.f : 0.f;
    const float wcls = (VER == 4) ? c.loss_weight[2] : c.loss_weight[3];
    if (VER != 1 && obj == 0.f) {
      g = 0.f;
    } else if (VER == 3 || VER == 4) {
      const float l = -obj * (tk * logf(pc) + (1.f - tk) * logf(1.f - pc));
      part[5] += (double)l;
      part[0] += (double)wcls * (double)l;
      g = -wcls * obj * (tk / pc - (1.f - tk) / (1.f - pc)) * pass;
    } else if (VER == 2) {
      const float l = -obj * (tk * logf(pc));
      part[5] += (double)l;
      part[0] += (double)wcls * (double)l;
      g = -wcls * obj * (tk / pc) * pass;
    } else {
      const float l = -t4 * tk * logf(pc);
      part[5] += (double)l;
      part[0] += (double)wcls * (double)l;
      g = -wcls * t4 * (tk / pc) * pass;
    }
  }
  return g;
}

template <int VER, bool PREF>
__global__ __launch_bounds__(256) void loss_kernel(const LossParams lp, const float* __restrict__ y_true,
                                                   const float* __restrict__ y_pred, float* __restrict__ dpred,
                                                   double* __restrict__ out) {
  const yolo_loss_cfg& c = lp.c;
  const int A = c.A, C = c.C;
  const int TD = 5 + C;
  const int PD = (VER == 1) ? 5 * A + C : A * (5 + C);
  const int lane = threadIdx.x & 63;
  const long long wave0 = ((long long)blockIdx.x * blockDim.x + threadIdx.x) >> 6;
  const long long nwaves = ((long long)gridDim.x * blockDim.x) >> 6;
  const float gw = (float)c.gw, gh = (float)c.gh;
  const double invN = 1.0 / (double)c.N;

  double part[7] = {0, 0, 0, 0, 0, 0, 0};

  float my_anchor = 1.f;
#pragma unroll
  for (int j = 0; j < 32; ++j)
    if (lane == j) my_anchor = c.use_anchors ? c.anchors[j] : 1.f;

  auto chan_of = [&](int idx, int& b, int& k) {
    if (VER == 1) {
      if (idx < 5 * A) {
        b = idx / 5;
        k = idx - b * 5;
      } else {
        b = 0;
        k = 5 + (idx - 5 * A);
      }
    } else {
      b = idx / TD;
      k = idx - b * TD;
    }
  };
  auto cell_head = [&](long long cell, const float (&Tb)[4], const float t4, const float (&Pb)[4], float& iou, float (&dI)[4],
                       int& resp) {
    iou = -1.f;
    float ciou = 0.f;
    dI[0] = dI[1] = dI[2] = dI[3] = 0.f;
    if (lane < A) {
      const IouOut o = iou_dual<VER == 4>(Tb, Pb, gw, gh);
      iou = o.iou.v;
      ciou = o.ciou.v;
      const D4& src = (VER == 4) ? o.ciou : o.iou;
      for (int i = 0; i < 4; ++i) dI[i] = src.d[i];
    }
    resp = 0;
    float best = __shfl(iou, 0, 64);
    for (int b = 1; b < A; ++b) {
      const float ib = __shfl(iou, b, 64);
      if (ib > best) {
        best = ib;
        resp = b;
      }
    }
    if (lp.dec != nullptr) {
      const unsigned long long ign = __ballot(lane < A && iou < c.ignore_thresh);
      const unsigned long long tru = __ballot(lane < A && iou > c.truth_thresh);
      if (lane == 0) {
        lp.dec[cell * 2] = resp;
        lp.dec[cell * 2 + 1] = (int)((unsigned)(ign & 0xffffu) | ((unsigned)(tru & 0xffffu) << 16));
      }
    }
    if (VER == 4 && lane < A) {
      float obj = t4 * (lane == resp ? 1.f : 0.f);
      if (c.truth_thresh < 1.f) obj = obj + ((iou > c.truth_thresh) ? 1.f : 0.f) * (1.f - obj);
      const double box = (double)(obj * (1.f - ciou));
      part[1] += box;
      part[0] += (double)c.loss_weight[0] * box;
    }
  };

  if constexpr (PREF) {
    constexpr int NCK = 4;
    float pn[NCK], tkn[NCK], tbn, pbn[4];
    auto prefetch = [&](long long cell) {
      const float* T = y_true + cell * TD;
      const float* Pc = y_pred + cell * PD;
#pragma unroll
      for (int q = 0; q < NCK; ++q) {
        int idx = q * 64 + lane;
        idx = idx < PD ? idx : PD - 1;
        int b, k;
        chan_of(idx, b, k);
        pn[q] = Pc[idx];
        tkn[q] = T[k >= 5 ? k : 4];
      }
      tbn = T[lane < 5 ? lane : 4];
      const float* P = Pc + (lane < A ? lane : 0) * TD;
#pragma unroll
      for (int j = 0; j < 4; ++j) pbn[j] = P[j];
    };
    long long cell = wave0;
    if (cell < lp.cells) prefetch(cell);
    for (; cell < lp.cells; cell += nwaves) {
      float pc[NCK], tkc[NCK], Pb[4];
#pragma unroll
      for (int q = 0; q < NCK; ++q) {
        pc[q] = pn[q];
        tkc[q] = tkn[q];
      }
#pragma unroll
      for (int j = 0; j < 4; ++j) Pb[j] = pbn[j];
      const float tbc = tbn;
      if (cell + nwaves < lp.cells) prefetch(cell + nwaves);
      float* G = dpred ? dpred + cell * PD : nullptr;
      const float Tb[4] = {__shfl(tbc, 0, 64), __shfl(tbc, 1, 64), __shfl(tbc, 2, 64), __shfl(tbc, 3, 64)};
      const float t4 = __shfl(tbc, 4, 64);
      float iou, dI[4];
      int resp;
      cell_head(cell, Tb, t4, Pb, iou, dI, resp);
#pragma unroll
      for (int q = 0; q < NCK; ++q) {
        const int base = q * 64;
        if (base < PD) {
          const bool active = (base + lane) < PD;
          const int idx = active ? (base + lane) : (PD - 1);
          int b, k;
          chan_of(idx, b, k);
          const float iou_b = __shfl(iou, b, 64);
          const float d0 = __shfl(dI[0], b, 64), d1 = __shfl(dI[1], b, 64);
          const float d2 = __shfl(dI[2], b, 64), d3 = __shfl(dI[3], b, 64);
          const float an = __shfl(my_anchor, (b * 2 + ((k == 3) ? 1 : 0)) & 31, 64);
          const float r_b = (b == resp) ? 1.f : 0.f;
          if (active) {
            const float g = loss_channel<VER>(c, b, k, pc[q], tkc[q], t4, Tb, iou_b, d0, d1, d2, d3, an, 0.f, r_b, part);
            if (G) G[idx] = g * lp.inv_n;
          }
        }
      }
    }
  } else {
  for (long long cell = wave0; cell < lp.cells; cell += nwaves) {
    const float* T = y_true + cell * TD;
    const float* Pc = y_pred + cell * PD;
    float* G = dpred ? dpred + cell * PD : nullptr;

    const float t4 = T[4];
    const float Tb[4] = {T[0], T[1], T[2], T[3]};
    float Pb[4] = {0.f, 0.f, 0.f, 0.f};
    if (lane < A) {
      const float* P = Pc + ((VER == 1) ? lane * 5 : lane * (5 + C));
      for (int j = 0; j < 4; ++j) Pb[j] = P[j];
    }
    float iou, dI[4];
    int resp;
    cell_head(cell, Tb, t4, Pb, iou, dI, resp);

    float p_nxt, tk_nxt;
    {
      const int idx0 = lane < PD ? lane : (PD - 1);
      int b0, k0;
      chan_of(idx0, b0, k0);
      p_nxt = Pc[idx0];
      tk_nxt = T[k0 >= 5 ? k0 : 4];
    }
    for (int base = 0; base < PD; base += 64) {
      const bool active = (base + lane) < PD;
      const int idx = active ? (base + lane) : (PD - 1);
      int b, k;
      chan_of(idx, b, k);
      const float p = p_nxt, tk_cur = tk_nxt;
      if (base + 64 < PD) {
        const int idn = (base + 64 + lane) < PD ? (base + 64 + lane) : (PD - 1);
        int bn, kn;
        chan_of(idn, bn, kn);
        p_nxt = Pc[idn];
        tk_nxt = T[kn >= 5 ? kn : 4];
      }
      const float iou_b = __shfl(iou, b, 64);
      const float d0 = __shfl(dI[0], b, 64), d1 = __shfl(dI[1], b, 64);
      const float d2 = __shfl(dI[2], b, 64), d3 = __shfl(dI[3], b, 64);
      const float an = __shfl(my_anchor, (b * 2 + ((k == 3) ? 1 : 0)) & 31, 64);
      const float cb = (VER == 1) ? Pc[b * 5 + 4] : 0.f;
      const float r_b = (b == resp) ? 1.f : 0.f;
      if (!active) continue;
      const float g = loss_channel<VER>(c, b, k, p, tk_cur, t4, Tb, iou_b, d0, d1, d2, d3, an, cb, r_b, part);
      if (G) G[idx] = g * lp.inv_n;
    }
  }
  }

  __shared__ double red[7][4];
  const int wave = threadIdx.x >> 6;
#pragma unroll
  for (int q = 0; q < 7; ++q) {
    const double s = wave_reduce_sum(part[q]);
    if (lane == 0) red[q][wave] = s;
  }
  __syncthreads();
  if (threadIdx.x < 7) {
    const double s = red[threadIdx.x][0] + red[threadIdx.x][1] + red[threadIdx.x][2] + red[threadIdx.x][3];
    atomicAdd(&out[threadIdx.x], s * invN);
  }
}

template <int VER>
__global__ __launch_bounds__(256) void metrics_kernel(const LossParams lp, const float* __restrict__ y_true,
                                                      const float* __restrict__ y_pred, float recall_thresh,
                                                      double* __restrict__ out) {
  const yolo_loss_cfg& c = lp.c;
  const int A = c.A, C = c.C;
  const int TD = 5 + C;
  const int PD = (VER == 1) ? 5 * A + C : A * (5 + C);
  const int lane = threadIdx.x & 63;
  const long long wave0 = ((long long)blockIdx.x * blockDim.x + threadIdx.x) >> 6;
  const long long nwaves = ((long long)gridDim.x * blockDim.x) >> 6;
  const float gw = (float)c.gw, gh = (float)c.gh;
  double part[5] = {0, 0, 0, 0, 0};

  for (long long cell = wave0; cell < lp.cells; cell += nwaves) {
    const float* T = y_true + cell * TD;
    const float* Pc = y_pred + cell * PD;
    const float t4 = T[4];
    float iou = -FLT_MAX, conf = -FLT_MAX;
    if (lane < A) {
      const float* P = Pc + ((VER == 1) ? lane * 5 : lane * (5 + C));
      const float Tb[4] = {T[0], T[1], T[2], T[3]};
      const float Pb[4] = {P[0], P[1], P[2], P[3]};
      iou = iou_dual<false>(Tb, Pb, gw, gh).iou.v;
      conf = P[4];
    }
    auto wave_argmax = [&](const float* v) -> int {
      float bv = -FLT_MAX;
      int bi = 0x7fffffff;
      for (int k = lane; k < C; k += 64) {
        const float x = v[k];
        if (x > bv) {
          bv = x;
          bi = k;
        }
      }
      for (int o = 32; o > 0; o >>= 1) {
        const float ov = __shfl_xor(bv, o, 64);
        const int oi = __shfl_xor(bi, o, 64);
        if (ov > bv || (ov == bv && oi < bi)) {
          bv = ov;
          bi = oi;
        }
      }
      return bi;
    };
    const int pi_true = wave_argmax(T + 5);
    float max_conf = -FLT_MAX, max_iou = -FLT_MAX, max_rec = -FLT_MAX;
    float eq_sum = 0.f;
    int pi_pred_cell = 0;
    if (VER == 1) pi_pred_cell = wave_argmax(Pc + 5 * A);
    for (int b = 0; b < A; ++b) {
      const float ib = __shfl(iou, b, 64);
      const float cb = __shfl(conf, b, 64);
      const int pi_pred = (VER == 1) ? pi_pred_cell : wave_argmax(Pc + b * TD + 5);
      const float eq = ((pi_pred == pi_true) ? 1.f : 0.f) * t4;
      max_conf = fmaxf(max_conf, cb);
      max_iou = fmaxf(max_iou, ib);
      max_rec = fmaxf(max_rec, ib * eq);
      eq_sum += eq;
    }
    if (lane == 0) {
      const float pred_bin = (max_conf > 0.5f) ? 1.f : 0.f;
      part[0] += (t4 == pred_bin) ? 1.0 : 0.0;
      part[1] += (double)(max_iou * t4);
      part[2] += (double)t4;
      part[3] += (VER == 1) ? (double)(((pi_pred_cell == pi_true) ? 1.f : 0.f) * t4) : (double)eq_sum;
      part[4] += (max_rec >= recall_thresh) ? 1.0 : 0.0;
    }
  }
  __shared__ double red[5][4];
  const int wave = threadIdx.x >> 6;
  if (lane == 0)
    for (int q = 0; q < 5; ++q) red[q][wave] = part[q];
  __syncthreads();
  if (threadIdx.x < 5) {
    const double s = red[threadIdx.x][0] + red[threadIdx.x][1] + red[threadIdx.x][2] + red[threadIdx.x][3];
    atomicAdd(&out[threadIdx.x], s);
  }
  if (blockIdx.x == 0 && threadIdx.x == 5) out[5] = (double)lp.cells;
}

static int validate_cfg(const yolo_loss_cfg* cfg) {
  YOLO_REQUIRE(cfg != nullptr, "loss: null cfg");
  YOLO_REQUIRE(cfg->version >= 1 && cfg->version <= 4, "loss: bad version %d", cfg->version);
  YOLO_REQUIRE(cfg->N > 0 && cfg->gh > 0 && cfg->gw > 0 && cfg->C > 0, "loss: bad shape");
  YOLO_REQUIRE(cfg->A > 0 && cfg->A <= 16, "loss: anchors per cell %d out of range [1,16]", cfg->A);
  return YOLO_OK;
}

}

using namespace yolo;

extern "C" size_t yolo_loss_workspace_bytes(const yolo_loss_cfg* cfg) {
  (void)cfg;
  return 0;
}

extern "C" int yolo_loss_fwd_bwd(const yolo_loss_cfg* cfg, const float* y_true, const float* y_pred, double* loss_out,
                                 float* dpred, float grad_scale, void* workspace, size_t workspace_bytes,
                                 void* stream) {
  if (int rc = validate_cfg(cfg)) return rc;
  YOLO_REQUIRE(y_true && y_pred && loss_out, "loss: null pointer");
  LossParams lp;
  lp.c = *cfg;
  lp.cells = (long long)cfg->N * cfg->gh * cfg->gw;
  lp.inv_n = grad_scale / (float)cfg->N;
  lp.dec = (workspace != nullptr && workspace_bytes >= (size_t)lp.cells * 8 && cfg->A <= 16) ? reinterpret_cast<int*>(workspace)
                                                                                              : nullptr;
  hipStream_t st = as_stream(stream);
  if (hipMemsetAsync(loss_out, 0, 8 * sizeof(double), st) != hipSuccess) {
    set_error("loss: memset failed");
    return YOLO_ERR_LAUNCH;
  }
  long long blocks = (lp.cells + 3) / 4;
  if (blocks > 2048) blocks = 2048;
  dim3 grid((unsigned)blocks), block(256);
  static const bool pref_env = env_int("YOLO_LOSS_PREFETCH", 1) != 0;
  const bool pref = pref_env && !(g_opt[OPT_EXP] & 8) && cfg->version != 1 && cfg->A * (5 + cfg->C) <= 256;
  switch (cfg->version) {
    case 1: hipLaunchKernelGGL((loss_kernel<1, false>), grid, block, 0, st, lp, y_true, y_pred, dpred, loss_out); break;
    case 2:
      if (pref) hipLaunchKernelGGL((loss_kernel<2, true>), grid, block, 0, st, lp, y_true, y_pred, dpred, loss_out);
      else hipLaunchKernelGGL((loss_kernel<2, false>), grid, block, 0, st, lp, y_true, y_pred, dpred, loss_out);
      break;
    case 3:
      if (pref) hipLaunchKernelGGL((loss_kernel<3, true>), grid, block, 0, st, lp, y_true, y_pred, dpred, loss_out);
      else hipLaunchKernelGGL((loss_kernel<3, false>), grid, block, 0, st, lp, y_true, y_pred, dpred, loss_out);
      break;
    default:
      if (pref) hipLaunchKernelGGL((loss_kernel<4, true>), grid, block, 0, st, lp, y_true, y_pred, dpred, loss_out);
      else hipLaunchKernelGGL((loss_kernel<4, false>), grid, block, 0, st, lp, y_true, y_pred, dpred, loss_out);
      break;
  }
  return check_launch("loss_kernel");
}

extern "C" int yolo_metrics(const yolo_loss_cfg* cfg, const float* y_true, const float* y_pred, float recall_thresh,
                            double* out, void* stream) {
  if (int rc = validate_cfg(cfg)) return rc;
  YOLO_REQUIRE(y_true && y_pred && out, "metrics: null pointer");
  LossParams lp;
  lp.c = *cfg;
  lp.cells = (long long)cfg->N * cfg->gh * cfg->gw;
  lp.inv_n = 0.f;
  hipStream_t st = as_stream(stream);
  if (hipMemsetAsync(out, 0, 8 * sizeof(double), st) != hipSuccess) {
    set_error("metrics: memset failed");
    return YOLO_ERR_LAUNCH;
  }
  long long blocks = (lp.cells + 3) / 4;
  if (blocks > 2048) blocks = 2048;
  dim3 grid((unsigned)blocks), block(256);
  switch (cfg->version) {
    case 1: hipLaunchKernelGGL(metrics_kernel<1>, grid, block, 0, st, lp, y_true, y_pred, recall_thresh, out); break;
    case 2: hipLaunchKernelGGL(metrics_kernel<2>, grid, block, 0, st, lp, y_true, y_pred, recall_thresh, out); break;
    case 3: hipLaunchKernelGGL(metrics_kernel<3>, grid, block, 0, st, lp, y_true, y_pred, recall_thresh, out); break;
    default: hipLaunchKernelGGL(metrics_kernel<4>, grid, block, 0, st, lp, y_true, y_pred, recall_thresh, out); break;
  }
  return check_launch("metrics_kernel");
}
```

tf2_yolo_amd/engine.py:

```python
import math

import contextlib

import numpy as np
import torch

from . import ops
from . import plan
from . import tape
from ._lib import ACT_LEAKY, ACT_LINEAR, ACT_MISH, YoloHipError
from .plan import AUX_WORDS, has_filter

ACT_NAMES = {ACT_LINEAR: "linear", ACT_LEAKY: "leaky", ACT_MISH: "mish"}


class ParamSpec:
    __slots__ = ("name", "shape", "offset", "size", "init", "trainable")

    def __init__(self, name, shape, offset, init, trainable):
        self.name, self.shape, self.offset = name, tuple(shape), offset
        self.size = int(np.prod(shape))
        self.init, self.trainable = init, trainable


# ... 239 lines not shown
        return out

    def softmax(self, src, name):
        if not src.rank2:
            raise ValueError(f"{name}: Softmax takes a [N, C] tensor (put gap() in front)")
        out = self._push(SoftmaxUnit(name, src), 1, 1, src.c)
        out.rank2 = True
        return out

    def output(self, t):
        if t not in self.outputs:
            self.outputs.append(t)
        return t


def count_params(builder):
    train = state = 0
    for u in builder.units:
        if has_filter(u):
            train += u.cout * u.k * u.k * u.src.c + (u.cout if u.bias else 0) + (2 * u.cout if u.bn else 0)
            state += 2 * u.cout if u.bn else 0
        elif u.kind == "dense_softmax":
            train += u.K * u.src.c + u.K
    return train, state


def conv_flops_per_image(builder):
    total = 0
    for u in builder.units:
        if has_filter(u):
            total += 2 * u.out.h * u.out.w * u.cout * u.src.c * u.k * u.k
    return total


_EPILOGUES = {ACT_LEAKY: ops.EPI_AFFINE_LEAKY, ACT_MISH: ops.EPI_AFFINE_MISH}


def _epilogue(u):
    return _EPILOGUES.get(u.act, ops.EPI_AFFINE)


class Network:
    def __init__(self, builder, device="cuda", seed=1234, unbiased_moving_var=True):
        if not torch.cuda.is_available():
            raise YoloHipError("tf2_yolo_amd needs a HIP device: there is no CPU fallback")
        self.device = torch.device(device)
        if self.device.index is not None and self.device.index != torch.cuda.current_device():
            raise YoloHipError(f"Network(device={device!r}): the kernels launch on the current device "
                               f"(cuda:{torch.cuda.current_device()}); call torch.cuda.set_device first "
                               "(one process per GPU)")
        self.tensors = builder.tensors
        self.units = builder.units
        self.input = builder.input
        self.outputs = list(builder.outputs)
        self.unbiased_moving_var = unbiased_moving_var
        self._opts = plan.Options.from_env()
        for k, v in vars(self._opts).items():
            setattr(self, "_" + k, v)
        g = self._plan = plan.plan_graph(self.units, self.tensors, self.input, self.outputs, self._opts)
        self._needs_grad, self._n_consumers = g.needs_grad, g.n_consumers
        self._bound_alias, self._up_producer = g.bound_alias, g.up_producer
        self.params = ParamStore()
        self.state = ParamStore()
        self._declare_params()
        rng = np.random.default_rng(seed)
        self.params.materialize(self.device, rng)
        self.state.materialize(self.device, rng)
        self.grads = torch.zeros_like(self.params.data)
        self._init_anchors()
        ops.create_side_streams(self.device)
        ops.ensure_conv_workspace()
        ops.ensure_wgrad_workspace()
        self._alloc_planned_buffers(g)
        self._wT_valid = self._wp_valid = self._wTp_valid = False
        self._jobs_wp = self._jobs_wTp = self._jobs_wT = None
        self._wp_event = self._wT_event = None
        self._infer_graphs = {}
        self._wgrad_stream = None
        self._wgrad_pending = False
        self.batch = None
        self.act = {}
        self.training = False
        self._precision = "fp32"
        self.grad_ready_hook = None
        self.backward_begin_hook = None
        self._infer_scale_valid = False
        self._twords = None
        self._tword_n = {}
        self._xplanes_infer = {}
        for u in self.units:
            u.concat_reads_through = False

    def _declare_params(self):
        for u in self.units:
            if u.kind == "conv":
                u.p_kernel = self.params.add(f"{u.name}_conv/kernel", (u.cout, u.k, u.k, u.src.c), u.kernel_init)
                u.p_bias = self.params.add(f"{u.name}_conv/bias", (u.cout,), init_zeros) if u.bias else None
                if u.bn:
                    u.p_gamma = self.params.add(f"{u.name}_bn/gamma", (u.cout,), init_ones)
                    u.p_beta = self.params.add(f"{u.name}_bn/beta", (u.cout,), init_zeros)
                    u.s_mean = self.state.add(f"{u.name}_bn/moving_mean", (u.cout,), init_zeros)
                    u.s_var = self.state.add(f"{u.name}_bn/moving_variance", (u.cout,), init_ones)
            elif u.kind == "head":
                u.p_kernel = self.params.add(f"{u.name}/kernel", (u.cout, 1, 1, u.src.c), u.kernel_init)
                u.p_bias = self.params.add(f"{u.name}/bias", (u.cout,), init_zeros)
            elif u.kind == "dense_softmax":
                u.p_kernel = self.params.add(f"{u.name}/kernel", (u.K, u.src.c), he_normal_dense)
                u.p_bias = self.params.add(f"{u.name}/bias", (u.K,), init_zeros)

    def _init_anchors(self):
        self._anchors_dev, self._anchor_grad_views = {}, {}
        heads = [u for u in self.units if u.kind == "head" and u.anchors is not None]
        n_anch = sum(2 * len(u.anchors) for u in heads)
        self.anchors_flat = torch.zeros(max(n_anch, 1), device=self.device, dtype=torch.float32)
        self.anchor_grads = torch.zeros_like(self.anchors_flat)
        self.anchors_trainable = False
        off = 0
        for u in heads:
            n = 2 * len(u.anchors)
            self.anchors_flat[off:off + n] = torch.tensor(np.array(u.anchors, dtype=np.float32).reshape(-1))
            self._anchors_dev[u.name] = self.anchors_flat[off:off + n]
            self._anchor_grad_views[u.name] = self.anchor_grads[off:off + n]
            off += n
        self.has_anchors = n_anch > 0

    def _alloc_planned_buffers(self, g):
        dev = self.device
        self._wT = torch.empty(g.wT_total, device=dev, dtype=torch.float32)
        self._bn_f32 = torch.zeros(max(g.bn_f32_total, 1), device=dev, dtype=torch.float32)
        self._bn_f64 = torch.zeros(max(g.bn_f64_total, 1), device=dev, dtype=torch.float64)
        self._bn_stats_total = g.bn_stats_total
        self._wplanes = torch.empty(g.wplanes_total, device=dev, dtype=torch.uint8) if g.wplanes_total else None
        self._aux = torch.zeros(g.aux_total, device=dev, dtype=torch.int32)
        self._tbound = self._aux[g.tbound_off:].view(torch.float32)
        self._tb = [self._tbound[i:i + 1] for i in range(len(self.tensors))]
        self._pred = torch.zeros(g.pred_total, device=dev, dtype=torch.float32)
        for u in self.units:
            a = u.aux_off
            u.bound = self._aux[a:a + 1]
            u.red_bound = self._aux[a + 1:a + 69]
            u.tickets = self._aux[a + 69:a + 69 + ops.BN_FOLD_TICKET_WORDS]
            u.pred = self._pred[u.pred_off:u.pred_off + 2]
            if u.kind == "conv" and u.bn:
                u.amax = self._aux[a + AUX_WORDS:a + AUX_WORDS + u.cout]
            if not has_filter(u):
                continue
            u.wT = self._wT[u.wT_off:u.wT_off + u.cout * u.k * u.k * u.src.c]
            u.wp = self._wplanes[u.wp_off:u.wp_off + u.wp_bytes] if u.planes_fwd else None
            u.wTp = self._wplanes[u.wTp_off:u.wTp_off + u.wTp_bytes] if u.planes_dgrad else None
            if u.cpad:
                u.wTp_pad = self._wplanes[u.wTp_pad_off:u.wTp_pad_off + u.wTp_pad_bytes]
                n = u.cpad * u.src.c
                u.w_pad = torch.zeros(n, device=dev, dtype=torch.float32)
                u.wT_pad = torch.empty(n, device=dev, dtype=torch.float32)
                u.dw_pad = torch.empty(n, device=dev, dtype=torch.float32)

    @property
    def num_params(self):
        return sum(self.params.specs[n].size for n in self.params.order)

    @property
    def num_state(self):
        return sum(self.state.specs[n].size for n in self.state.order)

    def allocate(self, N):
        if self.batch == N:
# ... 232 lines not shown
            side = self._wgrad_stream
            tape.wait_stream(side, torch.cuda.current_stream())
            with torch.cuda.stream(side):
                self._refresh_wplanes()
                self._wp_event = tape.record_event(side)
                self._refresh_wT()
                self._refresh_wTplanes()
                self._wT_event = tape.record_event(side)
        else:
            self._refresh_wplanes()

    def _fwd_conv(self, u, training):
        bias = self.params.view(u.p_bias.name) if u.p_bias is not None else None
        if not u.bn:
            self._conv_fwd(u, bias, u.y)
            if u.act != ACT_LINEAR:
                ops.act_fwd(u.y, u.act, out=u.a)
            if u.residual is not None:
                raise YoloHipError("residual without BN is not used by any reference graph")
            return
        scale, shift, smean, sinv, stats, _ = self._bn_bufs(u)
        if u.cout % 4:
            if u.residual is not None:
                raise YoloHipError(f"{u.name}: a residual Add needs a channel count that is a multiple of 4")
            self._conv_fwd(u, None if training else bias, u.y)
            ops.bn_act_any_fwd(u.y, u.cout, self.params.view(u.p_gamma.name), self.params.view(u.p_beta.name),
                               self.state.view(u.s_mean.name), self.state.view(u.s_var.name), scale, shift, smean, sinv, u.act,
                               u.a, training, mean_offset=bias, unbiased=self.unbiased_moving_var)
            return
        if training:
            amax = u.amax if self._tight_bound(u) else None
            self._conv_fwd(u, None, u.y, stats, amax)
            ops.bn_finalize(stats, u.y.numel() // u.cout, u.cout, self.params.view(u.p_gamma.name),
                            self.params.view(u.p_beta.name), self.state.view(u.s_mean.name), self.state.view(u.s_var.name),
                            scale, shift, smean, sinv, unbiased=self.unbiased_moving_var, bound=u.bound, absmax=amax,
                            mean_offset=bias)
            if u.pool_fuse is not None:
                return self._fwd_bn_act_pool(u, scale, shift)
        elif self._fuse_infer and (self._fused_infer_unit(u, bias, scale, shift)
                                   or (self._infer_onepass and self._stem_infer_unit(u, bias, scale, shift))):
            return
        else:
            self._conv_fwd(u, bias, u.y, absmax=u.amax)
            self._fold_infer_scale(u, scale, shift)
            ops.bn_infer_bound(u.cout, scale, shift, u.amax, u.bound)
        self._fwd_bn_act(u, training, scale, shift)

    def _fwd_bn_act_pool(self, u, scale, shift):
        pu = u.pool_fuse
        ppl = self._xplanes.get(pu.out.tid) if pu.out.c % 16 == 0 else None
        ops.bn_act_maxpool2x2_fwd(u.y, u.cout, scale, shift, u.act, pu.argmax,
                                  out=pu.buf if (pu.f32_needed or ppl is None) else None, planes=ppl,
                                  bn_bound=u.bound, out_bound=self._tb[pu.out.tid])
        self._tbound_set.add(pu.out.tid)
        if ppl is not None:
            self._xp_valid.add(pu.out.tid)
        pu.fused_this_pass = True

    def _fwd_bn_act(self, u, training, scale, shift):
        res = self.act[u.residual.tid] if u.residual is not None else None
        res_pl = None
        if (res is not None and training and self._res_from_planes and u.cout % 16 == 0
                and u.residual.tid in self._xp_valid and u.residual.tid in self._tbound_set):
            res_pl, res = self._xplanes[u.residual.tid], None
        pl = self._xplanes.get(u.out.tid) if u.cout % 16 == 0 else None
        if u.residual is not None and u.residual.tid not in self._tbound_set:
            pl = None
        else:
            self._tbound_set.add(u.out.tid)
        ops.bn_act_fwd(u.y, u.cout, scale, shift, u.act, res, out=u.a, planes=pl,
                       want_out=not (training and pl is not None and not u.a_needed), bn_bound=u.bound,
                       residual_bound=self._tb_float(u.residual.tid) if res is not None else None,
                       out_bound=self._tb[u.out.tid], residual_planes=res_pl)
        if pl is not None:
            self._xp_valid.add(u.out.tid)

    def _fwd_head(self, u, training):
        bias, anchors = self.params.view(u.p_bias.name), self._anchors_dev.get(u.name)
        if not training and self._infer_small_fuse and self._fuse_infer and u.planes_fwd:
            ops.conv2d_fwd_head_unit(u.desc, self._xp(u.src), u.wp, bias, u.A, u.C, u.version, anchors, u.t, u.yact,
                                     precision=self._precision)
            return
        self._conv_fwd(u, bias, u.t)
        ops.head_act_fwd(u.t, u.A, u.C, u.version, anchors, out=u.yact)

    def _fwd_upsample(self, u, training):
        if not training and self._infer_small_fuse and self._concat_planes and u.out.tid in self._up_producer:
            u.concat_reads_through = True
            return
        ops.upsample2x_fwd(self.act[u.src.tid], u.buf, u.out.c, 0)

    def _fwd_concat(self, u, training):
        pl = self._xplanes.get(u.out.tid) if self._concat_planes else None
        slots = [self._bound_alias.get(s.tid, s.tid) for s in u.srcs]
        ups = [self._up_producer.get(s.tid) for s in u.srcs]
        ups = [p if (p is not None and p.concat_reads_through) else None for p in ups]
        for p in ups:
            if p is not None:
                p.concat_reads_through = False
        rows, chans = self.batch * u.out.h * u.out.w, [s.c for s in u.srcs]
        dst32 = u.buf if u.f32_needed else None
        if (pl is not None and len(u.srcs) <= 4 and all(sl in self._tbound_set for sl in slots)
                and all(s.c % 8 == 0 for s in u.srcs)):
            if any(p is not None for p in ups):
                ops.split_planes_concat_ex([self.act[p.src.tid] if p is not None else self.act[s.tid]
                                            for s, p in zip(u.srcs, ups)], chans, [self._tb_words(sl) for sl in slots],
                                           rows, pl, upsample=[p is not None for p in ups], hw=(u.out.h, u.out.w),
                                           dst32=dst32, out_bound=self._tb[u.out.tid])
            else:
                ops.split_planes_concat([self.act[s.tid] for s in u.srcs], chans, [self._tb_float(sl) for sl in slots],
                                        rows, pl, dst32=dst32, out_bound=self._tb[u.out.tid])
            self._xp_valid.add(u.out.tid)
            self._tbound_set.add(u.out.tid)
            return
        for p in ups:
            if p is not None:
                ops.upsample2x_fwd(self.act[p.src.tid], p.buf, p.out.c, 0)
        off = 0
        for s in u.srcs:
            ops.copy_channels_in(self.act[s.tid], s.c, u.buf, u.out.c, off)
            off += s.c

    def _fwd_maxpool(self, u, training):
        if getattr(u, "fused_this_pass", False):
            u.fused_this_pass = False
            return
        ops.maxpool_fwd(self.act[u.src.tid], u.k, u.stride, u.pad_t, u.pad_l, u.out.h, u.out.w, u.buf,
                        u.out.c, 0, u.argmax if training else None)

    def _fwd_space_to_depth(self, u, training):
        ops.space_to_depth2_fwd(self.act[u.src.tid], u.buf, u.out.c, 0)

    def _fwd_gap(self, u, training):
        ops.gap_fwd(self.act[u.src.tid], out=u.buf)

    def _fwd_dense_softmax(self, u, training):
        ops.dense_softmax_fwd(self.act[u.src.tid], self.params.view(u.p_kernel.name), self.params.view(u.p_bias.name),
                              logits=u.logits, p=u.buf)

    def _stem_infer_unit(self, u, bias, scale, shift):
        pl = self._xplanes.get(u.out.tid)
        if u.residual is not None or pl is None or u.src.tid != self.input.tid or not ops.stem_infer_supported(u.desc):
            return False
        xin, w = self.act[u.src.tid], self.params.view(u.p_kernel.name)
        if self._fold_infer_scale(u, scale, shift):
            if getattr(u, "stem_wt", None) is None:
                u.stem_wt = torch.empty(28 * 32, device=self.device, dtype=torch.float32)
            ops.stem_filter_prep(w, bias, u.stem_wt)
            ops.zero_bytes(u.pred)
            ops.conv_pred_bound(w, u.cout, 27, scale, shift, bias, u.pred)
        row = self._tb_row(self.input.tid)
        n_in = ops.absmax_words(xin, row)
        nw = ops.stem_fwd_infer_unit(u.desc, xin, u.stem_wt, _epilogue(u), scale, shift, u.pred, row[:n_in],
                                     u.a if u.a_needed else None, pl, self._tb_row(u.out.tid))
        self._tword_n[u.out.tid] = nw
        self._tbound_set.add(u.out.tid)
        self._xp_valid.add(u.out.tid)
        return True

    def _fused_infer_unit(self, u, bias, scale, shift):
        if not u.planes_fwd or u.cout % 16 != 0:
            return False
        pl = self._xplanes.get(u.out.tid)
        own_planes = pl is not None
        if pl is None and self._infer_small_fuse and self._infer_onepass:
            rows = self.batch * u.out.h * u.out.w
            if rows <= 4096:
# ... 30 lines not shown
        self._tbound_set.add(u.out.tid)
        self._xp_valid.add(u.out.tid)
        return True

    def _stem_fused_bwd(self, u):
        return (self._stem_fused and not (u.planes_wgrad or u.planes_dgrad) and not self._needs_grad[u.src.tid]
                and ops.stem_bn_bwd_supported(u.desc))

    def _takes_grad_slice(self, u):
        return u.kind == "conv" and u.bn and u.residual is None and u.cout % 8 == 0 and not self._stem_fused_bwd(u)

    def _add_grad(self, grads, t, buf):
        if not self._needs_grad[t.tid]:
            return
        cur = grads.get(t.tid)
        if cur is None:
            grads[t.tid] = buf
        else:
            ops.axpy(cur, buf)

    def _grad_into(self, grads, t):
        cur = grads.get(t.tid)
        if cur is not None:
            return cur, True
        cur = grads[t.tid] = torch.empty((self.batch, t.h, t.w, t.c), device=self.device, dtype=torch.float32)
        return cur, False

    def _gview(self, spec):
        return self.grads[spec.offset:spec.offset + spec.size]

    def backward(self, douts):
        if not self.training:
            raise YoloHipError("backward() requires a preceding forward(training=True)")
        if self.backward_begin_hook is not None:
            tape.host_call(self.backward_begin_hook)
        if self._wT_event is not None:
            tape.wait_event(torch.cuda.current_stream(), self._wT_event)
            self._wT_event = None
        self._refresh_wT()
        self._refresh_wTplanes()
        for u in self.units:
            if getattr(u, "bnred", None) is not None:
                u.bnred_done = False
        grads = {t.tid: g for t, g in zip(self.outputs, douts)}
        for u in reversed(self.units):
            dout = grads.pop(u.out.tid, None)
            if dout is None:
                continue
            if isinstance(dout, ops.ChannelSlice) and not self._takes_grad_slice(u):
                dout = dout.dense((self.batch, u.out.h, u.out.w, u.out.c))
            getattr(self, "_bwd_" + u.kind)(u, dout, grads)
            if self.grad_ready_hook is not None and plan.has_params(u):
                tape.host_call(lambda u=u: self.grad_ready_hook(u))
        self._join_wgrad()

    def _bwd_conv(self, u, dout, grads):
        if u.bn and u.cout % 4:
            scale, shift, smean, sinv, _, _ = self._bn_bufs(u)
            dy = ops.bn_act_any_bwd(u.y, dout, u.cout, self.params.view(u.p_gamma.name), scale, shift, smean, sinv, u.act,
                                    self._gview(u.p_gamma), self._gview(u.p_beta))
            return self._filter_and_data_grad(u, dy, self._dyp(u, dy), None, grads)
        if u.bn:
            scale, shift, smean, sinv, _, red = self._bn_bufs(u)
            if u.residual is not None:
                self._add_grad(grads, u.residual, dout)
            if self._stem_fused_bwd(u):
                ops.stem_bn_bwd_wgrad(u.desc, self.act[u.src.tid], u.y, dout, scale, shift, smean, sinv, u.act, red,
                                      self._gview(u.p_gamma), self._gview(u.p_beta), self._gview(u.p_kernel),
                                      fused=self._take_fused(u, dout))
                return
            need_f32 = (not u.planes_wgrad) or (self._needs_grad[u.src.tid] and not u.planes_dgrad)
            dyp = self._next_dyp_buffer(u) if (u.planes_wgrad or u.planes_dgrad) else None
            dy = ops.bn_act_bwd(u.y, dout, u.cout, self.params.view(u.p_gamma.name), scale, shift, smean,
                                sinv, u.act, red, self._gview(u.p_gamma), self._gview(u.p_beta),
                                planes=dyp, want_dx=need_f32, bound_aux=u.red_bound, fused=self._take_fused(u, dout),
                                tickets=u.tickets if self._bn_fold else None)
        else:
            dy = ops.act_bwd(u.y, dout, u.act) if u.act != ACT_LINEAR else dout
            dyp = self._dyp(u, dy)
        dbias = self._gview(u.p_bias) if (u.p_bias is not None and not u.bn) else None
        self._filter_and_data_grad(u, dy, dyp, dbias, grads)

    def _bwd_head(self, u, dout, grads):
        dt = ops.head_act_bwd(u.yact, dout, u.A, u.C, u.version, self._anchors_dev.get(u.name),
                              danchors=self._anchor_grad_views.get(u.name) if self.anchors_trainable else None)
        if not u.cpad:
            return self._filter_and_data_grad(u, dt, self._dyp(u, dt), self._gview(u.p_bias), grads)
        rows = self.batch * u.out.h * u.out.w
        dtp = ops.split_planes_padded(dt, rows, u.out.c, out=self._next_dyp_buffer(u))
        with self._beside_backward(dt):
            ops.zero_bytes(u.dw_pad)
            ops.conv2d_wgrad_planes(u.desc_pad, self._xplanes[u.src.tid], dtp, u.dw_pad)
            ops.axpy(self._gview(u.p_kernel), u.dw_pad[:u.out.c * u.src.c])
            ops.conv2d_wgrad_bias(dt, rows, u.out.c, self._gview(u.p_bias))
        if self._needs_grad[u.src.tid]:
            had = grads.get(u.src.tid)
            b = self._bnred_of(u, had)
            cur, acc = self._grad_into(grads, u.src)
            ops.conv2d_dgrad_planes(u.desc_pad, dtp, u.wTp_pad, dx=cur, accumulate=acc, bnred=b)

    def _filter_and_data_grad(self, u, dy, dyp, dbias, grads):
        with self._beside_backward(dy):
            if u.planes_wgrad:
                ops.conv2d_wgrad_planes(u.desc, self._xplanes[u.src.tid], dyp, self._gview(u.p_kernel), dy=dy, dbias=dbias)
            else:
                ops.conv2d_wgrad(u.desc, self.act[u.src.tid], dy, self._gview(u.p_kernel), dbias)
        if not self._needs_grad[u.src.tid]:
            return
        b = self._bnred_of(u, grads.get(u.src.tid)) if u.planes_dgrad else None
        cur, acc = self._grad_into(grads, u.src)
        if u.planes_dgrad:
            ops.conv2d_dgrad_planes(u.desc, dyp, u.wTp, dx=cur, accumulate=acc, bnred=b)
        else:
            ops.conv2d_dgrad(u.desc, dy, u.wT, dx=cur, accumulate=acc)

    def _bwd_upsample(self, u, dout, grads):
        if self._needs_grad[u.src.tid]:
            cur, acc = self._grad_into(grads, u.src)
            ops.upsample2x_bwd(dout, u.out.c, 0, cur, accumulate=acc)

    def _bwd_concat(self, u, dout, grads):
        off = 0
        for s in u.srcs:
            if not self._needs_grad[s.tid]:
                pass
            elif (s.tid not in grads and self._concat_grad_slices and self._n_consumers.get(s.tid, 0) == 1
                    and s.producer is not None and self._takes_grad_slice(s.producer)
                    and s.c % 8 == 0 and off % 4 == 0 and u.out.c % 4 == 0):
                grads[s.tid] = ops.ChannelSlice(dout, u.out.c, off, s.c)
            else:
                cur, acc = self._grad_into(grads, s)
                ops.copy_channels_out(dout, u.out.c, off, cur, s.c, accumulate=acc)
            off += s.c

    def _bwd_maxpool(self, u, dout, grads):
        if not self._needs_grad[u.src.tid]:
            return
        N, had = self.batch, grads.get(u.src.tid)
        tiles = (u.k == 2 and u.stride == 2 and u.pad_t == 0 and u.pad_l == 0 and u.src.h == 2 * u.out.h
                 and u.src.w == 2 * u.out.w and u.out.c % 4 == 0 and torch.is_tensor(dout) and dout.is_contiguous()
                 and (had is None or torch.is_tensor(had)))
        cur, acc = self._grad_into(grads, u.src)
        if tiles:
            ops.maxpool2x2_bwd(dout, N, u.out.h, u.out.w, u.out.c, u.argmax, cur, acc)
            return
        if not acc:
            ops.zero_bytes(cur)
        if u.stride == 1 and (u.out.h, u.out.w) == (u.src.h, u.src.w):
            ops.maxpool_bwd_same(dout, N, u.out.h, u.out.w, u.out.c, u.out.c, 0, u.argmax, u.k, u.pad_t, u.pad_l, cur)
        else:
            ops.maxpool_bwd(dout, N, u.out.h, u.out.w, u.out.c, u.out.c, 0, u.argmax, cur)

    def _bwd_gap(self, u, dout, grads):
        if not self._needs_grad[u.src.tid]:
            return
        cur = grads.get(u.src.tid)
        if cur is None:
            grads[u.src.tid] = ops.gap_bwd(dout, u.dsrc, accumulate=False)
        else:
            ops.gap_bwd(dout, cur, accumulate=True)

    def _fwd_softmax(self, u, training):
        ops.dense_softmax_fwd(self.act[u.src.tid], None, None, p=u.buf)

    def _bwd_softmax(self, u, dout, grads):
        if self._needs_grad[u.src.tid]:
            ops.dense_softmax_bwd(dout, u.buf, None, None, u.dsrc)
            self._add_grad(grads, u.src, u.dsrc)

    def _bwd_dense_softmax(self, u, dout, grads):
        ops.dense_softmax_bwd(dout, u.buf, self.act[u.src.tid], self.params.view(u.p_kernel.name), u.dsrc,
                              dw=self._gview(u.p_kernel), db=self._gview(u.p_bias), dz=u.dz)
# ... 94 lines not shown
```

tf2_yolo_amd/model.py:

```python
import time

import numpy as np
import torch

from . import dp as dp_mod
from . import optimizers as opt_mod
from ._lib import YoloHipError, precision_enum
from .engine import Network


def _to_input(x):
    if torch.is_tensor(x):
        return x.to(device="cuda", dtype=torch.float32).contiguous()
    return torch.from_numpy(np.ascontiguousarray(np.asarray(x, dtype=np.float32))).cuda()


def _raw_images(x, what):
    if not (isinstance(x, (np.ndarray, list, tuple)) or torch.is_tensor(x)):
        raise TypeError(f"{what} with rescale= / resize= takes a uint8 array [N, h, w, 3] or a list of uint8 images, got "
                        f"{type(x).__name__}")
    return x


class LayerView:

    def __init__(self, model, name, getter, setter, trainable=True):
        self.model, self.name, self._get, self._set, self.trainable = model, name, getter, setter, trainable

    def get_weights(self):
        return self._get()

    def set_weights(self, weights):
        self.model.net.before_param_write()
        self._set(weights)
        self.model.net.mark_params_changed()


class Model:
    def __init__(self, builder, version, seed=1234, unbiased_moving_var=True):
        self.net = Network(builder, seed=seed, unbiased_moving_var=unbiased_moving_var)
        self.version = version
        self.single_output = len(self.net.outputs) == 1 and version in (0, 1, 2)
        self.optimizer = None
        self.loss = None
        self.metrics = None
        self._reducer = None
        self._loss_bufs = None
        self.stop_training = False
        self.history = None

    @property
    def input_shape(self):
        return (None, self.net.input.h, self.net.input.w, self.net.input.c)

    @property
    def output(self):
        outs = self.net.outputs
        return outs[0] if self.single_output else list(outs)

    @property
    def output_shape(self):
        outs = [o.shape for o in self.net.outputs]
        return outs[0] if self.single_output else outs

    def count_params(self):
        return self.net.num_params + self.net.num_state

    def trainable_count(self):
        return self.net.num_params

    @property
    def layers(self):
        return [self.get_layer(n) for n in self.layer_names()]

    def layer_names(self):
        names = []
        for u in self.net.units:
            if u.kind == "conv":
                names.append(f"{u.name}_conv")
                if u.bn:
                    names.append(f"{u.name}_bn")
            elif u.kind == "head":
# ... 257 lines not shown
        loss_names = {"categorical_crossentropy": loss_mod.CategoricalCrossentropy}
        metric_names = dict.fromkeys(("accuracy", "acc", "categorical_accuracy"), loss_mod.CategoricalAccuracy)
        loss = [named(l, loss_names, "loss") for l in loss] if isinstance(loss, (list, tuple)) else named(loss, loss_names, "loss")
        self.loss = list(loss) if isinstance(loss, (list, tuple)) else [loss] * nout
        if len(self.loss) != nout:
            raise ValueError(f"need {nout} losses, got {len(self.loss)}")
        if metrics is None:
            metrics = [[] for _ in range(nout)]
        elif nout == 1 and (not metrics or not isinstance(metrics[0], (list, tuple))):
            metrics = [list(metrics)]
        self.metrics = [[named(v, metric_names, "metric") for v in m] for m in metrics]
        self._loss_bufs = [torch.zeros(8, device="cuda", dtype=torch.float64) for _ in range(nout)]
        self._dpred = None
        self._drop_step_graphs()

    def enable_data_parallel(self, process_group=None, bucket_bytes=48 << 20):
        segs, units = dp_mod.network_segments(self.net)
        self._reducer = dp_mod.GradReducer(self.net.grads, segs, process_group, bucket_bytes)
        index = {id(u): i for i, u in enumerate(units)}
        self._dp_unit_index = index
        self._drop_step_graphs()
        self.net.grad_ready_hook = lambda u: self._reducer.segment_done(index[id(u)])
        self.net.backward_begin_hook = self._reducer.backward_begin
        net = self.net
        self._reducer.extra_streams = lambda: [net._wgrad_stream] if net._wgrad_stream is not None else []
        dp_mod.broadcast_parameters([self.net.params.data, self.net.state.data], 0, process_group)
        self.net.mark_params_changed()

    def _labels(self, y):
        ys = [y] if not isinstance(y, (list, tuple)) else list(y)
        out = []
        for a in ys:
            if torch.is_tensor(a):
                out.append(a.to(device="cuda", dtype=torch.float32).contiguous())
            else:
                out.append(torch.from_numpy(np.ascontiguousarray(np.asarray(a, dtype=np.float32))).cuda())
        return out

    def _drop_step_graphs(self):
        self._step_graphs = None
        self._eager_steps = {}

    def _captured_step(self, x, y_list):
        import os
        mode = os.environ.get("YOLO_STEP_MODE", "tape")
        if os.environ.get("YOLO_STEP_GRAPH", "1") == "0" or mode == "eager" or getattr(self, "_graphs_failed", False):
            return None
        if not getattr(self.optimizer, "capturable", False):
            return None
        if self.net.grad_ready_hook is not None and self._reducer is None:
            return None
        from .capture import StepGraphs, StepTape
        self.net.allocate(x.shape[0])
        key = StepGraphs.key_of(self, x)
        g = self._step_graphs
        if g is not None and g.key == key:
            return g.replay(x, y_list)
        n = self._eager_steps.get(key, 0)
        if os.environ.get("YOLO_STEP_DEBUG"):
            import sys
            print(f"[step] mode {mode} eager steps so far {n} key {key} known {list(self._eager_steps)}", file=sys.stderr)
        if n < 2 or self._dpred is None:
            self._eager_steps = {key: n + 1}
            self._step_graphs = None
            return None
        try:
            if mode == "graph":
                self._step_graphs = StepGraphs(self, x, y_list)
                return self._step_graphs.replay(x, y_list)
            self._step_graphs = StepTape(self, x, y_list)
            return self._loss_bufs
        except Exception as e:
            import sys
            import traceback
            print(f"[tf2_yolo_amd] step recording ({mode}) failed ({e!r}); training continues with eager launches\n"
                  + "".join(traceback.format_exc().splitlines(True)[-12:]), file=sys.stderr)
            self._graphs_failed = True
            self._step_graphs = None
            if mode != "graph":
                from . import ops as _ops
                _ops.zero_bytes(self.net.grads)
            return None

    def train_step_device(self, x, y_list, with_metrics=False):
        if self.optimizer is None:
            raise YoloHipError("compile() the model before training")
        from . import ops as _ops
        if not with_metrics and _ops.TIMER is None:
            bufs = self._captured_step(x, y_list)
            if bufs is not None:
                return bufs, None
        outs = self.net.forward(x, training=True)
        if self._dpred is None or self._dpred[0].shape != outs[0].shape:
            self._dpred = [torch.empty_like(o) for o in outs]
        for i, (o, yt) in enumerate(zip(outs, y_list)):
            self.loss[i].fwd_bwd(yt, o, grad_scale=1.0, dpred=self._dpred[i], loss_out=self._loss_bufs[i])
        mvals = None
        if with_metrics:
            mvals = [[m(yt, o) for m in ms] for ms, o, yt in zip(self.metrics, outs, y_list)]
        self.net.backward(self._dpred)
        if self._reducer is not None and self.net.anchors_trainable and self._reducer.world > 1:
            import torch.distributed as dist
            dist.all_reduce(self.net.anchor_grads, group=self._reducer.pg)
        scale = self._reducer.finish() if self._reducer is not None else 1.0
        self.optimizer.step(grad_scale=scale)
        return self._loss_bufs, mvals

    def train_on_batch(self, x, y, return_dict=False, rescale=None, **_):
        bufs, mvals = self.train_step_device(self._to_input(x, rescale), self._labels(y), with_metrics=bool(self.metrics))
        losses = [float(b[0].item()) for b in bufs]
        total = sum(losses)
        flat = [float(v.item()) for ms in (mvals or []) for v in ms]
        res = [total] + (losses if len(losses) > 1 else []) + flat
        return res if len(res) > 1 else res[0]

    def test_on_batch(self, x, y, rescale=None):
        outs = self.net.forward(self._to_input(x, rescale), training=False)
        ys = self._labels(y)
        losses = [float(l(yt, o).item()) for l, o, yt in zip(self.loss, outs, ys)]
        mvals = [float(m(yt, o).item()) for ms, o, yt in zip(self.metrics, outs, ys) for m in ms]
        return [sum(losses)] + (losses if len(losses) > 1 else []) + mvals

    def _iter_batches(self, x, y, batch_size, shuffle, rng):
        if y is None:
            order = np.arange(len(x))
            for i in order:
                yield x[int(i)]
            if hasattr(x, "on_epoch_end"):
                x.on_epoch_end()
            return
        n = len(x)
        order = rng.permutation(n) if shuffle else np.arange(n)
        ys = y if isinstance(y, (list, tuple)) else [y]
        for i in range(0, n, batch_size):
            sel = order[i:i + batch_size]
            yb = [a[sel] for a in ys]
            yield x[sel], (yb if isinstance(y, (list, tuple)) else yb[0])

    def _host_source(self, x, y, batch_size, shuffle, rng):
        if y is None:
            def batches():
                for i in range(len(x)):
                    yield x[int(i)]
                if hasattr(x, "on_epoch_end"):
                    x.on_epoch_end()
            return ("batches", batches())
        ys = list(y) if isinstance(y, (list, tuple)) else [y]
        if any(torch.is_tensor(a) and a.is_cuda for a in [x] + ys):
            return None
        n = len(x)
        order = rng.permutation(n) if shuffle else np.arange(n)
        return ("arrays", [x] + ys, order, batch_size)

    def fit(self, x=None, y=None, batch_size=None, epochs=1, verbose=1, validation_data=None, shuffle=True,
            initial_epoch=0, callbacks=None, rescale=None, **_):
        import os
        from .feeder import FeederBuffers, HostFeeder
        batch_size = batch_size or 32
        if rescale is not None and y is not None:
            from . import images
            images.check_batch(x, self._input_hw())
        rng = np.random.default_rng(0)
        hist = {"loss": []}
        pipelined = os.environ.get("YOLO_FIT_PIPELINE", "1") != "0"
        cbs = list(callbacks or [])

        def _cb(hook, *args):
            for c in cbs:
                f = getattr(c, hook, None)
                if f is not None:
                    f(*args)
        for c in cbs:
            if hasattr(c, "set_model"):
                c.set_model(self)
        self.stop_training = False
        _cb("on_train_begin", {})
        for ep in range(initial_epoch, epochs):
            t0 = time.time()
            _cb("on_epoch_begin", ep, {})
            tot, nb = 0.0, 0
            src = self._host_source(x, y, batch_size, shuffle, rng) if pipelined else None
            if src is not None:
                if getattr(self, "_feed_bufs", None) is None:
# ... 44 lines not shown
```

tf2_yolo_amd/ops.py:

```python
import ctypes
from ctypes import byref, c_void_p

import torch

from . import _lib
from . import tape as _tape
from ._lib import ConvDesc, LossCfg, YoloHipError, check

BN_EPS = 1e-3
BN_MOMENTUM = 0.99
BN_STAT_SLOTS = 64
BN_RED_SLOTS = 512
SPLIT_BATCH_UNITS = 4


class KernelTimer:

    def __init__(self):
        self.pending = []

    def bracket(self, flops, fn, layer=None):
        last, n = _lib.load().yolo_last_conv_kernel, ctypes.c_int(0)
        last(None)
        s, e = torch.cuda.Event(enable_timing=True), torch.cuda.Event(enable_timing=True)
# ... 158 lines not shown


def _chk_f32(*ts):
    for t in ts:
        if t is None:
            continue
        if not (t.is_cuda and t.dtype == torch.float32 and t.is_contiguous()):
            raise YoloHipError("expected a contiguous float32 CUDA tensor, got "
                               f"{t.dtype} {t.device} contiguous={t.is_contiguous()}")


def same_pad(size, k, s):
    out = -(-size // s)
    total = max((out - 1) * s + k - size, 0)
    return out, total // 2


def conv_desc(x_shape, cout, kh, kw, stride, padding):
    n, h, w, cin = x_shape
    if padding == "same":
        ho, pt = same_pad(h, kh, stride)
        wo, pl = same_pad(w, kw, stride)
    elif padding == "valid":
        ho, wo, pt, pl = (h - kh) // stride + 1, (w - kw) // stride + 1, 0, 0
    elif padding == "darknet_s2":
        ho, wo, pt, pl = (h + 1 - kh) // stride + 1, (w + 1 - kw) // stride + 1, 1, 1
    else:
        raise ValueError(f"bad padding {padding}")
    return ConvDesc(n, h, w, cin, cout, kh, kw, ho, wo, stride, stride, pt, pl)


def conv2d_fwd(d, x, w, bias=None, out=None, stats=None, absmax=None):
    _chk_f32(x, w, bias)
    if out is None:
        out = torch.empty((d.N, d.Ho, d.Wo, d.Cout), device=x.device, dtype=torch.float32)
    if x.numel() != d.N * d.H * d.W * d.Cin or w.numel() != d.Cout * d.kh * d.kw * d.Cin:
        raise YoloHipError("conv2d_fwd: tensor sizes do not match the descriptor")
    if out.numel() != d.N * d.Ho * d.Wo * d.Cout:
        raise YoloHipError("conv2d_fwd: output size does not match the descriptor")
    if stats is not None and stats.numel() != BN_STAT_SLOTS * 2 * d.Cout:
        raise YoloHipError("conv2d_fwd: stats must hold BN_STAT_SLOTS x 2 x Cout doubles")
    def run():
        check(_lib.load().yolo_conv2d_fwd_absmax(byref(d), _p(x), _p(w), _p(bias), _p(out), _p(stats), _p(absmax),
                                                 _stream()), "yolo_conv2d_fwd")
    if TIMER is not None:
        TIMER.bracket(_conv_flops(d), run)
    else:
        run()
    return out


def planes_bytes(rows, c):
    n = int(_lib.load().yolo_planes_bytes(int(rows), int(c)))
    if n == 0:
        raise YoloHipError(f"planes: unsupported shape rows={rows} C={c} (C must be a multiple of 16)")
    return n


def split_planes(x, rows, c, out=None):
    _chk_f32(x)
    if x.numel() != rows * c:
        raise YoloHipError("split_planes: tensor size does not match rows x C")
    n = planes_bytes(rows, c)
    if out is None:
        out = torch.empty(n, device=x.device, dtype=torch.uint8)
    elif out.numel() < n or out.dtype != torch.uint8:
        raise YoloHipError("split_planes: output buffer too small")
    check(_lib.load().yolo_split_planes(_p(x), int(rows), int(c), _p(out), _stream()), "yolo_split_planes")
    return out


def split_planes_padded(x, rows, c_src, out=None):
    _chk_f32(x)
    c = (c_src + 15) // 16 * 16
    if x.numel() != rows * c_src:
        raise YoloHipError("split_planes_padded: tensor size does not match rows x C_src")
    n = planes_bytes(rows, c)
    if out is None:
        out = torch.empty(n, device=x.device, dtype=torch.uint8)
    elif out.numel() < n or out.dtype != torch.uint8:
        raise YoloHipError("split_planes_padded: output buffer too small")
    check(_lib.load().yolo_split_planes_padded(_p(x), int(rows), int(c_src), int(c), _p(out), _stream()),
          "yolo_split_planes_padded")
    return out


class BatchJobs:

    def __init__(self, kind, device):
        self.kind, self.device = kind, device
        self.rows, self.blocks, self.table = [], 0, None

    def add_split(self, src, dst, rows, c, bound_from=None):
        nb = -(-((rows + 15) // 16 + 1) // SPLIT_BATCH_UNITS) * -(-c // 128)
        donor = 0 if bound_from is None else bound_from.data_ptr() + bound_from.numel() - 256
        self.rows.append([src.data_ptr(), dst.data_ptr(), rows, c, donor, self.blocks])
        self.blocks += nb

    def add_transpose(self, src, dst, cout, taps, cin):
        nb = -(-cin // 32) * -(-cout // 32) * taps
        self.rows.append([src.data_ptr(), dst.data_ptr(), cout, taps, cin, self.blocks])
        self.blocks += nb

    def run(self):
        if not self.rows:
            return
        if self.table is None:
            self.table = torch.tensor(self.rows, dtype=torch.int64).to(self.device)
        fn = _lib.load().yolo_split_planes_batch if self.kind == "split" else _lib.load().yolo_filter_transpose_batch
        check(fn(_p(self.table), len(self.rows), self.blocks, _stream()), "yolo_%s_batch" % self.kind)


precision_enum = _lib.precision_enum


def conv2d_fwd_planes(d, xp, wp, bias=None, out=None, stats=None, absmax=None, precision="fp32"):
    prec = precision_enum(precision)
    _chk_f32(bias)
    if out is None:
        out = torch.empty((d.N, d.Ho, d.Wo, d.Cout), device=xp.device, dtype=torch.float32)
    if xp.numel() < planes_bytes(d.N * d.H * d.W, d.Cin) or wp.numel() < planes_bytes(d.Cout, d.kh * d.kw * d.Cin):
        raise YoloHipError("conv2d_fwd_planes: planes buffers do not match the descriptor")
    if out.numel() != d.N * d.Ho * d.Wo * d.Cout:
        raise YoloHipError("conv2d_fwd_planes: output size does not match the descriptor")
    if stats is not None and stats.numel() != BN_STAT_SLOTS * 2 * d.Cout:
        raise YoloHipError("conv2d_fwd_planes: stats must hold BN_STAT_SLOTS x 2 x Cout doubles")
    def run():
        check(_lib.load().yolo_conv2d_fwd_planes_ex(byref(d), _p(xp), _p(wp), _p(bias), _p(out), _p(stats), _p(absmax),
                                                    prec, _stream()), "yolo_conv2d_fwd_planes_ex")
    if TIMER is not None:
        TIMER.bracket(_conv_flops(d), run, _layer_key(d, "fwd"))
    else:
        run()
    return out


EPI_NONE, EPI_AFFINE, EPI_AFFINE_LEAKY, EPI_AFFINE_MISH = 0, 1, 2, 3


def conv2d_fwd_planes_epi(d, xp, wp, bias, epilogue, scale, shift, residual=None, out=None, absmax=None, precision="fp32"):
    prec = precision_enum(precision)
    _chk_f32(bias, scale, shift, residual)
    if out is None:
        out = torch.empty((d.N, d.Ho, d.Wo, d.Cout), device=xp.device, dtype=torch.float32)
    if xp.numel() < planes_bytes(d.N * d.H * d.W, d.Cin) or wp.numel() < planes_bytes(d.Cout, d.kh * d.kw * d.Cin):
        raise YoloHipError("conv2d_fwd_planes_epi: planes buffers do not match the descriptor")
    if out.numel() != d.N * d.Ho * d.Wo * d.Cout or (residual is not None and residual.numel() != out.numel()):
        raise YoloHipError("conv2d_fwd_planes_epi: output / residual size does not match the descriptor")
    def run():
        check(_lib.load().yolo_conv2d_fwd_planes_epi_ex(byref(d), _p(xp), _p(wp), _p(bias), int(epilogue), _p(scale), _p(shift),
                                                        _p(residual), _p(out), _p(absmax), prec, _stream()),
              "yolo_conv2d_fwd_planes_epi_ex")
    if TIMER is not None:
        TIMER.bracket(_conv_flops(d), run, _layer_key(d, "fwd"))
    else:
        run()
    return out


def conv_pred_bound(w, cout, kdim, scale, shift, bias, pred2):
    _chk_f32(w, scale, shift, bias, pred2)
    if w.numel() != cout * kdim or pred2.numel() != 2:
        raise YoloHipError("conv_pred_bound: w must hold Cout x kdim floats, pred2 two")
    check(_lib.load().yolo_conv_pred_bound(_p(w), int(cout), int(kdim), _p(scale), _p(shift), _p(bias), _p(pred2), _stream()),
          "yolo_conv_pred_bound")

# ... 488 lines not shown
def maxpool_bwd_same(dy, N, H, W, C, Cy, c_off, argmax, k, pad_t, pad_l, dx):
    check(_lib.load().yolo_maxpool_bwd_same(_p(dy), N, H, W, C, Cy, c_off, _p(argmax), int(k), int(pad_t), int(pad_l), _p(dx),
                                            _stream()), "yolo_maxpool_bwd_same")


def space_to_depth2_fwd(x, y, Cy, c_off):
    n, h, w, c = x.shape
    check(_lib.load().yolo_space_to_depth2_fwd(_p(x), n, h, w, c, _p(y), Cy, c_off, _stream()),
          "yolo_space_to_depth2_fwd")


def space_to_depth2_bwd(dy, Cy, c_off, dx, accumulate=False):
    n, h, w, c = dx.shape
    check(_lib.load().yolo_space_to_depth2_bwd(_p(dy), n, h, w, c, Cy, c_off, _p(dx), int(bool(accumulate)),
                                               _stream()), "yolo_space_to_depth2_bwd")


def head_act_fwd(t, A, C, version, anchors_dev, out=None):
    if out is None:
        out = torch.empty_like(t)
    D = (5 * A + C) if version == 1 else A * (5 + C)
    P = t.numel() // D
    check(_lib.load().yolo_head_act_fwd(_p(t), P, A, C, version, _p(anchors_dev), _p(out), _stream()),
          "yolo_head_act_fwd")
    return out


def head_act_bwd(y, dy, A, C, version, anchors_dev, dt=None, danchors=None):
    if dt is None:
        dt = torch.empty_like(y)
    D = (5 * A + C) if version == 1 else A * (5 + C)
    P = y.numel() // D
    check(_lib.load().yolo_head_act_bwd(_p(y), _p(dy), P, A, C, version, _p(anchors_dev), _p(dt), _p(danchors),
                                        _stream()), "yolo_head_act_bwd")
    return dt


def make_loss_cfg(version, N, gh, gw, A, C, anchors=None, binary_weight=1.0, loss_weight=(1, 1, 1, 1),
                  ignore_thresh=0.6, use_focal_loss=False, focal_gamma=2.0, use_scale=True, wh_reg_weight=0.01,
                  truth_thresh=1.0, label_smooth=0.0):
    cfg = LossCfg()
    cfg.version, cfg.N, cfg.gh, cfg.gw, cfg.A, cfg.C = version, N, gh, gw, A, C
    if anchors is not None:
        flat = [float(v) for pair in anchors for v in pair]
        if len(flat) != 2 * A or len(flat) > 32:
            raise ValueError(f"need {A} (w,h) anchors, at most 16; got {len(flat) // 2}")
        for i, v in enumerate(flat):
            cfg.anchors[i] = v
        cfg.use_anchors = 1
    else:
        cfg.use_anchors = 0
    cfg.binary_weight = float(binary_weight)
    lw = list(loss_weight) + [0.0] * (4 - len(loss_weight))
    for i in range(4):
        cfg.loss_weight[i] = float(lw[i])
    cfg.ignore_thresh = float(ignore_thresh)
    cfg.use_focal_loss = int(bool(use_focal_loss))
    cfg.focal_gamma = float(focal_gamma)
    cfg.use_scale = int(bool(use_scale))
    cfg.wh_reg_weight = float(wh_reg_weight)
    cfg.truth_thresh = float(truth_thresh)
    cfg.label_smooth = float(label_smooth)
    return cfg


def loss_fwd_bwd(cfg, y_true, y_pred, loss_out=None, dpred=None, grad_scale=1.0, want_grad=True, decisions=None):
    _chk_f32(y_true, y_pred, dpred)
    cells = cfg.N * cfg.gh * cfg.gw
    pd = (5 * cfg.A + cfg.C) if cfg.version == 1 else cfg.A * (5 + cfg.C)
    if y_true.numel() != cells * (5 + cfg.C) or y_pred.numel() != cells * pd:
        raise YoloHipError(f"loss: tensor sizes do not match cfg (cells={cells}, C={cfg.C}, A={cfg.A})")
    if loss_out is None:
        loss_out = torch.empty(8, device=y_pred.device, dtype=torch.float64)
    if want_grad and dpred is None:
        dpred = torch.empty_like(y_pred)
    if decisions is not None and (decisions.dtype != torch.int32 or decisions.numel() < 2 * cells or not decisions.is_cuda):
        raise YoloHipError("loss: decisions must be an int32 CUDA tensor with 2 entries per cell")
    check(_lib.load().yolo_loss_fwd_bwd(byref(cfg), _p(y_true), _p(y_pred), _p(loss_out),
                                        _p(dpred if want_grad else None), float(grad_scale), _p(decisions),
                                        0 if decisions is None else decisions.numel() * 4, _stream()), "yolo_loss_fwd_bwd")
    return loss_out, dpred


def metrics(cfg, y_true, y_pred, recall_thresh=0.5, out=None):
    _chk_f32(y_true, y_pred)
    if out is None:
        out = torch.empty(8, device=y_pred.device, dtype=torch.float64)
    check(_lib.load().yolo_metrics(byref(cfg), _p(y_true), _p(y_pred), float(recall_thresh), _p(out), _stream()),
          "yolo_metrics")
    return out


def gap_fwd(x, out=None):
    _chk_f32(x, out)
    if x.dim() != 4:
        raise YoloHipError("gap_fwd: x must be [N, H, W, C]")
    n, h, w, c = x.shape
    if out is None:
        out = torch.empty((n, c), device=x.device, dtype=torch.float32)
    if out.numel() != n * c:
        raise YoloHipError("gap_fwd: the output must hold N * C floats")
    check(_lib.load().yolo_gap_fwd(_p(x), n, h, w, c, _p(out), _stream()), "yolo_gap_fwd")
    return out


def gap_bwd(dg, dx, accumulate=False):
    _chk_f32(dg, dx)
    if dx.dim() != 4:
        raise YoloHipError("gap_bwd: dx must be [N, H, W, C]")
    n, h, w, c = dx.shape
    if dg.numel() != n * c:
        raise YoloHipError("gap_bwd: dg must hold N * C floats")
    check(_lib.load().yolo_gap_bwd(_p(dg), n, h, w, c, _p(dx), int(bool(accumulate)), _stream()), "yolo_gap_bwd")
    return dx


def dense_softmax_fwd(g, w, b, logits=None, p=None):
    _chk_f32(g, w, b, logits, p)
    if g.dim() != 2 or (w is None) != (b is None):
        raise YoloHipError("dense_softmax_fwd: g must be [N, C]; kernel and bias come together")
    n, c = g.shape
    k = c if w is None else b.numel()
    if w is not None and w.numel() != k * c:
        raise YoloHipError(f"dense_softmax_fwd: the kernel must hold K * C = {k * c} floats, got {w.numel()}")
    if p is None:
        p = torch.empty((n, k), device=g.device, dtype=torch.float32)
    if w is None:
        logits = g
    elif logits is None:
        logits = torch.empty((n, k), device=g.device, dtype=torch.float32)
    if p.numel() != n * k or logits.numel() != n * k:
        raise YoloHipError("dense_softmax_fwd: logits and p must hold N * K floats")
    check(_lib.load().yolo_dense_softmax_fwd(_p(g), _p(w), _p(b), n, c, k, _p(None if w is None else logits), _p(p), _stream()),
          "yolo_dense_softmax_fwd")
    return logits, p


def dense_softmax_bwd(dp, p, g, w, dg, dw=None, db=None, dz=None):
    _chk_f32(dp, p, g, w, dg, dw, db, dz)
    if dp.dim() != 2 or p.shape != dp.shape:
        raise YoloHipError("dense_softmax_bwd: dp and p must be [N, K]")
    n, k = dp.shape
    if w is None:
        if dw is not None or db is not None or dg.numel() != n * k:
            raise YoloHipError("dense_softmax_bwd: without weights dg is [N, K] and there is no dw / db")
        c = k
    else:
        c = w.numel() // k
        if g is None or dw is None or db is None:
            raise YoloHipError("dense_softmax_bwd: the Dense form needs g, dw and db")
        if dz is None:
            dz = torch.empty_like(dp)
        if (w.numel() != k * c or g.numel() != n * c or dg.numel() != n * c or dw.numel() != k * c or db.numel() != k
                or dz.numel() != n * k):
            raise YoloHipError("dense_softmax_bwd: tensor sizes do not match N, C, K")
    check(_lib.load().yolo_dense_softmax_bwd(_p(dp), _p(p), _p(g), _p(w), n, c, k, _p(dz), _p(dg), _p(dw), _p(db), _stream()),
          "yolo_dense_softmax_bwd")
    return dg


def bn_act_any_fwd(y, C, gamma, beta, moving_mean, moving_var, scale, shift, save_mean, save_invstd, act, out, training,
                   mean_offset=None, eps=BN_EPS, momentum=BN_MOMENTUM, unbiased=False):
    _chk_f32(y, gamma, beta, moving_mean, moving_var, scale, shift, save_mean, save_invstd, out, mean_offset)
    if y.numel() % C or out.numel() != y.numel() or any(t.numel() != C for t in (gamma, beta, moving_mean, moving_var, scale,
                                                                                 shift, save_mean, save_invstd)):
        raise YoloHipError("bn_act_any_fwd: tensor sizes do not match C")
# ... 379 lines not shown
```

tf2_yolo_amd/plan.py:

```python
import os
from types import SimpleNamespace

from . import ops

AUX_WORDS = 112


class Options:

    @classmethod
    def from_env(cls, env=None):
        env = os.environ if env is None else env
        o = cls()

        def on(name):
            return env.get(name, "1") != "0"
        o.overlap_wgrad = on("YOLO_BWD_OVERLAP")
        o.prep_beside = on("YOLO_PREP_OVERLAP")
        o.stem_fused = on("YOLO_STEM_FUSED_BWD")
        o.bn_tight = int(env.get("YOLO_BN_TIGHT_BOUND", "0"))
        o.res_from_planes = on("YOLO_RES_PLANES")
        o.use_infer_graph = on("YOLO_INFER_GRAPH")
        o.fuse_infer = on("YOLO_INFER_FUSE")
        o.concat_grad_slices = on("YOLO_CONCAT_GRAD_SLICE")
        o.dyp_per_layer = on("YOLO_DYP_PER_LAYER")
        o.bn_fold = env.get("YOLO_BN_FOLD", "0") == "1"
        o.bn_fused_reduce = env.get("YOLO_BN_FUSED_REDUCE", "0")
        o.head_pad = on("YOLO_HEAD_PAD")
        o.pool_fuse = on("YOLO_POOL_FUSE")
        o.concat_planes = on("YOLO_CONCAT_PLANES")
        o.infer_onepass = on("YOLO_INFER_ONEPASS")
        o.infer_small_fuse = on("YOLO_INFER_SMALL_FUSE")
        o.dgrad_classes = on("YOLO_DGRAD_CLASSES")
        return o


def has_filter(u):
    return u.kind in ("conv", "head")


def has_params(u):
    return u.kind in ("conv", "head", "dense_softmax")


def reads_as_planes(c, t):
    return has_filter(c) and c.src.tid == t.tid and c.residual is not t and c.planes_fwd and c.planes_wgrad


def _fp32_read(t, g, also=lambda c: False):
    cs = g.consumers.get(t.tid, [])
    return t.tid in g.out_tids or not cs or any(not (reads_as_planes(c, t) or also(c)) for c in cs)


def plan_graph(units, tensors, input, outputs, opts):
    g = SimpleNamespace(out_tids={t.tid for t in outputs})
    g.needs_grad = {input.tid: False}
    for u in units:
        g.needs_grad[u.out.tid] = has_params(u) or any(g.needs_grad[t.tid] for t in u.inputs)
    g.consumers, g.n_consumers = {}, {}
    for u in units:
        for t in u.inputs:
            g.consumers.setdefault(t.tid, []).append(u)
            g.n_consumers[t.tid] = g.n_consumers.get(t.tid, 0) + 1
    for t in outputs:
        g.n_consumers[t.tid] = g.n_consumers.get(t.tid, 0) + 1
    _plan_param_buffers(g, units)
    _plan_fused_reduce(g, units, tensors, opts)
    _plan_filter_planes(g, units, opts)
    _plan_fp32_copies(g, units, opts)
    _plan_bounds(g, units, tensors)
    return g


def _plan_param_buffers(g, units):
    wT = f32 = f64 = 0
    for u in units:
        if u.kind == "conv" and u.bn:
            u.bn_f32_off = f32
            f32 += 4 * u.cout
            u.bn_f64_off = f64
            f64 += ops.BN_STAT_SLOTS * 2 * u.cout
        if has_filter(u):
            u.wT_off = wT
            wT += u.cout * u.k * u.k * u.src.c
    g.bn_stats_total = f64
    for u in units:
        if u.kind == "conv" and u.bn:
            u.bn_red_off = f64
            f64 += (ops.BN_RED_SLOTS + 1) * 2 * u.cout
    g.wT_total, g.bn_f32_total, g.bn_f64_total = wT, f32, f64


def _plan_fused_reduce(g, units, tensors, opts):
    last = {}
    for u in reversed(units):
        u.bnred_for = None
        if u.kind == "conv" and u.bn and u.residual is not None and g.needs_grad[u.residual.tid]:
            last[u.residual.tid] = ("add", u)
        if has_filter(u):
            if g.needs_grad[u.src.tid]:
                last[u.src.tid] = ("dgrad", u)
        else:
            for t in u.inputs:
                if g.needs_grad[t.tid]:
                    last[t.tid] = ("other", u)
    mode = opts.bn_fused_reduce
    if mode == "0":
        return
    for tid, (how, w) in last.items():
        p = tensors[tid].producer
        if how != "dgrad":
            continue
        one_launch = w.stride == 1 or (w.stride == 2 and w.k == 3 and opts.dgrad_classes)
        if not (one_launch and p is not None and p.kind == "conv" and p.bn and p.cout % 4 == 0):
            continue
        if w.kind == "head":
# ... 120 lines not shown
```

Measured before the change: 1093.

## Fuse head activation into loss kernel computing gradients directly on logits

Adds a head_loss kernel that reads raw head logits, applies the head activation inline, computes the YOLO loss and writes the gradient with respect to the logits. It also records the gradient absmax into the planes header. This removes the separate head activation backward pass and the absmax pre-pass (memset plus amax kernels) before splitting the head gradient into planes. The fused path is on by default for v3 heads with fixed anchors, and falls back when metrics are requested or anchors are trainable. It adds a second loss implementation that must stay numerically consistent with the original one.

```diff
diff --git a/include/yolo_hip.h b/include/yolo_hip.h
--- a/include/yolo_hip.h
+++ b/include/yolo_hip.h
@@ -63,6 +63,7 @@
 size_t yolo_planes_bytes(long long rows, int C);
 int yolo_split_planes(const float* x, long long rows, int C, void* planes, void* stream);
 int yolo_split_planes_padded(const float* x, long long rows, int C_src, int C, void* planes, void* stream);
+int yolo_split_planes_padded_bound(const float* x, long long rows, int C_src, int C, void* planes, void* stream);
 
 int yolo_split_planes_batch(const void* jobs, int njobs, long long total_blocks, void* stream);
 int yolo_filter_transpose_batch(const void* jobs, int njobs, long long total_blocks, void* stream);
@@ -247,6 +248,10 @@
                       double* loss_out, float* dpred, float grad_scale,
                       void* workspace, size_t workspace_bytes, void* stream);
 
+int yolo_head_loss_fwd_bwd(const yolo_loss_cfg* cfg, const float* y_true, const float* t, const float* head_anchors,
+                           double* loss_out, float* dt, void* amax_word, float grad_scale,
+                           void* decisions, size_t decisions_bytes, void* stream);
+
 int yolo_metrics(const yolo_loss_cfg* cfg, const float* y_true, const float* y_pred,
                  float recall_thresh, double* out, void* stream);
 
diff --git a/tf2_yolo_amd/_lib.py b/tf2_yolo_amd/_lib.py
--- a/tf2_yolo_amd/_lib.py
+++ b/tf2_yolo_amd/_lib.py
@@ -61,6 +61,7 @@
     "yolo_planes_bytes": (c_size_t, [_LL, c_int]),
     "yolo_split_planes": (c_int, [_P, _LL, c_int, _P, _P]),
     "yolo_split_planes_padded": (c_int, [_P, _LL, c_int, c_int, _P, _P]),
+    "yolo_split_planes_padded_bound": (c_int, [_P, _LL, c_int, c_int, _P, _P]),
     "yolo_split_planes_batch": (c_int, [_P, c_int, _LL, _P]),
     "yolo_filter_transpose_batch": (c_int, [_P, c_int, _LL, _P]),
     "yolo_conv2d_fwd_planes": (c_int, [POINTER(ConvDesc), _P, _P, _P, _P, _P, _P, _P]),
@@ -133,6 +134,7 @@
     "yolo_head_act_bwd": (c_int, [_P, _P, _LL, c_int, c_int, c_int, _P, _P, _P, _P]),
     "yolo_loss_workspace_bytes": (c_size_t, [POINTER(LossCfg)]),
     "yolo_loss_fwd_bwd": (c_int, [POINTER(LossCfg), _P, _P, _P, _P, c_float, _P, c_size_t, _P]),
+    "yolo_head_loss_fwd_bwd": (c_int, [POINTER(LossCfg), _P, _P, _P, _P, _P, _P, c_float, _P, c_size_t, _P]),
     "yolo_metrics": (c_int, [POINTER(LossCfg), _P, _P, c_float, _P, _P]),
     "yolo_gap_fwd": (c_int, [_P, c_int, c_int, c_int, c_int, _P, _P]),
     "yolo_gap_bwd": (c_int, [_P, c_int, c_int, c_int, c_int, _P, c_int, _P]),
diff --git a/tf2_yolo_amd/capture.py b/tf2_yolo_amd/capture.py
--- a/tf2_yolo_amd/capture.py
+++ b/tf2_yolo_amd/capture.py
@@ -79,10 +79,10 @@
         try:
             with torch.cuda.stream(stream):
                 begin()
-                outs = net.forward(self.x, training=True)
-                for i, (o, yt) in enumerate(zip(outs, self.ys)):
-                    model.loss[i].fwd_bwd(yt, o, grad_scale=1.0, dpred=model._dpred[i], loss_out=model._loss_bufs[i])
-                net.backward(model._dpred)
+                with model._heads_mode():
+                    outs = net.forward(self.x, training=True)
+                    model._losses_fwd_bwd(outs, self.ys)
+                    net.backward(model._dpred)
                 net._dyp_events = [None, None]
                 if red is not None:
                     end(("finish",))
@@ -149,10 +149,10 @@
         opt.refresh_hyper(grad_scale=(1.0 / red.world) if red is not None else 1.0)
         tape_mod.ACTIVE = self.tape
         try:
-            outs = net.forward(self.x, training=True)
-            for i, (o, yt) in enumerate(zip(outs, self.ys)):
-                model.loss[i].fwd_bwd(yt, o, grad_scale=1.0, dpred=model._dpred[i], loss_out=model._loss_bufs[i])
-            net.backward(model._dpred)
+            with model._heads_mode():
+                outs = net.forward(self.x, training=True)
+                model._losses_fwd_bwd(outs, self.ys)
+                net.backward(model._dpred)
             if red is not None:
                 if net.anchors_trainable and red.world > 1:
                     import torch.distributed as dist
diff --git a/tf2_yolo_amd/csrc/conv.hip b/tf2_yolo_amd/csrc/conv.hip
--- a/tf2_yolo_amd/csrc/conv.hip
+++ b/tf2_yolo_amd/csrc/conv.hip
@@ -1086,6 +1086,11 @@
   return launch_split_planes_padded(x, rows, C_src, C, planes, as_stream(stream));
 }
 
+extern "C" int yolo_split_planes_padded_bound(const float* x, long long rows, int C_src, int C, void* planes, void* stream) {
+  YOLO_REQUIRE(x && planes, "split_planes_padded_bound: null pointer");
+  return launch_split_planes_padded(x, rows, C_src, C, planes, as_stream(stream), true);
+}
+
 struct BnRedArgs {
   const float* y;
   const float* scale;
diff --git a/tf2_yolo_amd/csrc/conv_args.hpp b/tf2_yolo_amd/csrc/conv_args.hpp
--- a/tf2_yolo_amd/csrc/conv_args.hpp
+++ b/tf2_yolo_amd/csrc/conv_args.hpp
@@ -116,7 +116,8 @@
 int launch_split_planes_concat(const float* const* xs, const int* Cs, const float* const* bounds, int nsrc, long long rows,
                                void* planes, float* dst32, float* out_bound, hipStream_t st,
                                const int* bound_words = nullptr, const int* upsample = nullptr, int H = 0, int W = 0);
-int launch_split_planes_padded(const float* x, long long rows, int Csrc, int C, void* planes, hipStream_t st);
+int launch_split_planes_padded(const float* x, long long rows, int Csrc, int C, void* planes, hipStream_t st,
+                               bool have_bound = false);
 int launch_split_planes_batch(const void* jobs, int njobs, long long total_blocks, hipStream_t st);
 int launch_filter_transpose_batch(const void* jobs, int njobs, long long total_blocks, hipStream_t st);
 int launch_gather_planes(GatherConvArgs& a, hipStream_t st);
diff --git a/tf2_yolo_amd/csrc/conv_planes.hip b/tf2_yolo_amd/csrc/conv_planes.hip
--- a/tf2_yolo_amd/csrc/conv_planes.hip
+++ b/tf2_yolo_amd/csrc/conv_planes.hip
@@ -802,7 +802,7 @@
   return check_launch("filter_transpose_batch_kernel");
 }
 
-int launch_split_planes_padded(const float* x, long long rows, int Csrc, int C, void* planes, hipStream_t st) {
+int launch_split_planes_padded(const float* x, long long rows, int Csrc, int C, void* planes, hipStream_t st, bool have_bound) {
   if (C % 16 != 0 || rows <= 0 || Csrc <= 0 || Csrc > C || C - Csrc >= 16) {
     set_error("split_planes_padded: need 0 < Csrc <= C < Csrc + 16, C %% 16 == 0, rows > 0");
     return YOLO_ERR_INVALID_ARG;
@@ -815,14 +815,16 @@
   }
   unsigned char* out = reinterpret_cast<unsigned char*>(planes);
   unsigned* header = reinterpret_cast<unsigned*>(out + planes_body_bytes(rows, C));
-  if (hipMemsetAsync(header, 0, 16, st) != hipSuccess) {
-    set_error("split_planes_padded: hipMemsetAsync failed");
-    return YOLO_ERR_LAUNCH;
-  }
-  const long long n = rows * Csrc, n4 = n / 4;
-  if (n4 > 0) hipLaunchKernelGGL(planes_amax_kernel, dim3(stream_grid(n4, 256)), dim3(256), 0, st, x, n4, header);
-  if (n > 4 * n4)
-    hipLaunchKernelGGL(planes_amax_scalar_kernel, dim3(1), dim3(256), 0, st, x + 4 * n4, n - 4 * n4, header);
+  if (!have_bound) {
+    if (hipMemsetAsync(header, 0, 16, st) != hipSuccess) {
+      set_error("split_planes_padded: hipMemsetAsync failed");
+      return YOLO_ERR_LAUNCH;
+    }
+    const long long n = rows * Csrc, n4 = n / 4;
+    if (n4 > 0) hipLaunchKernelGGL(planes_amax_kernel, dim3(stream_grid(n4, 256)), dim3(256), 0, st, x, n4, header);
+    if (n > 4 * n4)
+      hipLaunchKernelGGL(planes_amax_scalar_kernel, dim3(1), dim3(256), 0, st, x + 4 * n4, n - 4 * n4, header);
+  }
   hipLaunchKernelGGL(split_planes_padded_kernel, dim3((unsigned)blocks), dim3(256), 0, st, x, rows, Csrc, C, out,
                      rows_padded);
   return check_launch("split_planes_padded_kernel");
diff --git a/tf2_yolo_amd/csrc/conv_small.hip b/tf2_yolo_amd/csrc/conv_small.hip
--- a/tf2_yolo_amd/csrc/conv_small.hip
+++ b/tf2_yolo_amd/csrc/conv_small.hip
@@ -1,4 +1,5 @@
 #include "act.hpp"
+#include "head_act.hpp"
 #include "planes.hpp"
 #include <cstdlib>
 
@@ -246,7 +247,7 @@
           if (mrow + e < a.M && col < a.Cout) {
             const float v = fmaf(sum, unscale, bv[k]);
             if (a.dst != nullptr) a.dst[(mrow + e) * a.Cd + col] = v;
-            a.head_y[(mrow + e) * a.Cd + col] = (kk == 2 || kk == 3) ? expf(v) * anc : 1.f / (1.f + expf(-v));
+            a.head_y[(mrow + e) * a.Cd + col] = head_act(v, kk, anc);
           }
         } else {
           float v = 0.f;
diff --git a/tf2_yolo_amd/csrc/elementwise.hip b/tf2_yolo_amd/csrc/elementwise.hip
--- a/tf2_yolo_amd/csrc/elementwise.hip
+++ b/tf2_yolo_amd/csrc/elementwise.hip
@@ -1,4 +1,5 @@
 #include "common.hpp"
+#include "head_act.hpp"
 #include "planes.hpp"
 #include <cfloat>
 
@@ -329,7 +330,6 @@
   }
 }
 
-__device__ __forceinline__ float sigmoid_f(float x) { return 1.f / (1.f + expf(-x)); }
 
 __global__ void head_fwd_pointwise_kernel(const float* __restrict__ t, long long P, int A, int C,
                                           const float* __restrict__ anchors, float* __restrict__ y) {
@@ -338,11 +338,7 @@
   for (long long i = (long long)blockIdx.x * blockDim.x + threadIdx.x; i < n; i += (long long)gridDim.x * blockDim.x) {
     const int k = (int)(i % D);
     const int a = (int)((i / D) % A);
-    const float v = t[i];
-    float o;
-    if (k == 2 || k == 3) o = expf(v) * anchors[a * 2 + (k - 2)];
-    else o = sigmoid_f(v);
-    y[i] = o;
+    y[i] = head_act(t[i], k, head_is_wh(k) ? anchors[a * 2 + (k - 2)] : 0.f);
   }
 }
 
@@ -379,7 +375,7 @@
     const int k = (int)(i % D);
     if (k >= 5 && !sigmoid_classes) continue;
     const float yv = y[i], g = dy[i];
-    dt[i] = (k == 2 || k == 3) ? g * yv : g * yv * (1.f - yv);
+    dt[i] = head_act_grad(g, yv, k);
   }
 }
 
diff --git a/tf2_yolo_amd/csrc/head_act.hpp b/tf2_yolo_amd/csrc/head_act.hpp
--- /dev/null
+++ b/tf2_yolo_amd/csrc/head_act.hpp
@@ -0,0 +1,18 @@
+#pragma once
+#include <hip/hip_runtime.h>
+
+namespace yolo {
+
+__device__ __forceinline__ float sigmoid_f(float x) { return 1.f / (1.f + expf(-x)); }
+
+__device__ __forceinline__ bool head_is_wh(int k) { return k == 2 || k == 3; }
+
+__device__ __forceinline__ float head_act(float v, int k, float anchor) {
+  return head_is_wh(k) ? expf(v) * anchor : sigmoid_f(v);
+}
+
+__device__ __forceinline__ float head_act_grad(float g, float y, int k) {
+  return head_is_wh(k) ? g * y : g * y * (1.f - y);
+}
+
+}
diff --git a/tf2_yolo_amd/csrc/loss.hip b/tf2_yolo_amd/csrc/loss.hip
--- a/tf2_yolo_amd/csrc/loss.hip
+++ b/tf2_yolo_amd/csrc/loss.hip
@@ -1,5 +1,6 @@
 #include "common.hpp"
 #include "conv_args.hpp"
+#include "head_act.hpp"
 #include <cfloat>
 #include <cstdlib>
 
@@ -257,6 +258,64 @@
   return g;
 }
 
+template <int VER>
+__device__ __forceinline__ void chan_of_idx(const int idx, const int A, const int TD, int& b, int& k) {
+  if (VER == 1) {
+    if (idx < 5 * A) {
+      b = idx / 5;
+      k = idx - b * 5;
+    } else {
+      b = 0;
+      k = 5 + (idx - 5 * A);
+    }
+  } else {
+    b = idx / TD;
+    k = idx - b * TD;
+  }
+}
+
+template <int VER>
+__device__ __forceinline__ void cell_head_lanes(const LossParams& lp, const int lane, const float gw, const float gh,
+                                                const long long cell, const float (&Tb)[4], const float t4, const float (&Pb)[4],
+                                                float& iou, float (&dI)[4], int& resp, double (&part)[7]) {
+  const yolo_loss_cfg& c = lp.c;
+  const int A = c.A;
+  iou = -1.f;
+  float ciou = 0.f;
+  dI[0] = dI[1] = dI[2] = dI[3] = 0.f;
+  if (lane < A) {
+    const IouOut o = iou_dual<VER == 4>(Tb, Pb, gw, gh);
+    iou = o.iou.v;
+    ciou = o.ciou.v;
+    const D4& src = (VER == 4) ? o.ciou : o.iou;
+    for (int i = 0; i < 4; ++i) dI[i] = src.d[i];
+  }
+  resp = 0;
+  float best = __shfl(iou, 0, 64);
+  for (int b = 1; b < A; ++b) {
+    const float ib = __shfl(iou, b, 64);
+    if (ib > best) {
+      best = ib;
+      resp = b;
+    }
+  }
+  if (lp.dec != nullptr) {
+    const unsigned long long ign = __ballot(lane < A && iou < c.ignore_thresh);
+    const unsigned long long tru = __ballot(lane < A && iou > c.truth_thresh);
+    if (lane == 0) {
+      lp.dec[cell * 2] = resp;
+      lp.dec[cell * 2 + 1] = (int)((unsigned)(ign & 0xffffu) | ((unsigned)(tru & 0xffffu) << 16));
+    }
+  }
+  if (VER == 4 && lane < A) {
+    float obj = t4 * (lane == resp ? 1.f : 0.f);
+    if (c.truth_thresh < 1.f) obj = obj + ((iou > c.truth_thresh) ? 1.f : 0.f) * (1.f - obj);
+    const double box = (double)(obj * (1.f - ciou));
+    part[1] += box;
+    part[0] += (double)c.loss_weight[0] * box;
+  }
+}
+
 template <int VER, bool PREF>
 __global__ __launch_bounds__(256) void loss_kernel(const LossParams lp, const float* __restrict__ y_true,
                                                    const float* __restrict__ y_pred, float* __restrict__ dpred,
@@ -278,57 +337,9 @@
   for (int j = 0; j < 32; ++j)
     if (lane == j) my_anchor = c.use_anchors ? c.anchors[j] : 1.f;
 
-  auto chan_of = [&](int idx, int& b, int& k) {
-    if (VER == 1) {
-      if (idx < 5 * A) {
-        b = idx / 5;
-        k = idx - b * 5;
-      } else {
-        b = 0;
-        k = 5 + (idx - 5 * A);
-      }
-    } else {
-      b = idx / TD;
-      k = idx - b * TD;
-    }
-  };
+  auto chan_of = [&](int idx, int& b, int& k) { chan_of_idx<VER>(idx, A, TD, b, k); };
   auto cell_head = [&](long long cell, const float (&Tb)[4], const float t4, const float (&Pb)[4], float& iou, float (&dI)[4],
-                       int& resp) {
-    iou = -1.f;
-    float ciou = 0.f;
-    dI[0] = dI[1] = dI[2] = dI[3] = 0.f;
-    if (lane < A) {
-      const IouOut o = iou_dual<VER == 4>(Tb, Pb, gw, gh);
-      iou = o.iou.v;
-      ciou = o.ciou.v;
-      const D4& src = (VER == 4) ? o.ciou : o.iou;
-      for (int i = 0; i < 4; ++i) dI[i] = src.d[i];
-    }
-    resp = 0;
-    float best = __shfl(iou, 0, 64);
-    for (int b = 1; b < A; ++b) {
-      const float ib = __shfl(iou, b, 64);
-      if (ib > best) {
-        best = ib;
-        resp = b;
-      }
-    }
-    if (lp.dec != nullptr) {
-      const unsigned long long ign = __ballot(lane < A && iou < c.ignore_thresh);
-      const unsigned long long tru = __ballot(lane < A && iou > c.truth_thresh);
-      if (lane == 0) {
-        lp.dec[cell * 2] = resp;
-        lp.dec[cell * 2 + 1] = (int)((unsigned)(ign & 0xffffu) | ((unsigned)(tru & 0xffffu) << 16));
-      }
-    }
-    if (VER == 4 && lane < A) {
-      float obj = t4 * (lane == resp ? 1.f : 0.f);
-      if (c.truth_thresh < 1.f) obj = obj + ((iou > c.truth_thresh) ? 1.f : 0.f) * (1.f - obj);
-      const double box = (double)(obj * (1.f - ciou));
-      part[1] += box;
-      part[0] += (double)c.loss_weight[0] * box;
-    }
-  };
+                       int& resp) { cell_head_lanes<VER>(lp, lane, gw, gh, cell, Tb, t4, Pb, iou, dI, resp, part); };
 
   if constexpr (PREF) {
     constexpr int NCK = 4;
@@ -451,6 +462,171 @@
   if (threadIdx.x < 7) {
     const double s = red[threadIdx.x][0] + red[threadIdx.x][1] + red[threadIdx.x][2] + red[threadIdx.x][3];
     atomicAdd(&out[threadIdx.x], s * invN);
+  }
+}
+
+__device__ __forceinline__ float as_stored(float v) {
+  asm volatile("" : "+v"(v));
+  return v;
+}
+
+template <int VER>
+__global__ __launch_bounds__(256) void head_loss_kernel(const LossParams lp, const float* __restrict__ y_true,
+                                                        const float* __restrict__ t, const float* __restrict__ head_anchors,
+                                                        float* __restrict__ dt, unsigned* __restrict__ amax,
+                                                        double* __restrict__ out) {
+  static_assert(VER == 3 || VER == 4, "pointwise heads with sigmoid classes");
+  const yolo_loss_cfg& c = lp.c;
+  const int A = c.A, C = c.C;
+  const int TD = 5 + C;
+  const int PD = A * TD;
+  const int lane = threadIdx.x & 63;
+  const long long wave0 = ((long long)blockIdx.x * blockDim.x + threadIdx.x) >> 6;
+  const long long nwaves = ((long long)gridDim.x * blockDim.x) >> 6;
+  const float gw = (float)c.gw, gh = (float)c.gh;
+  const double invN = 1.0 / (double)c.N;
+  constexpr int NCK = 4;
+
+  double part[7] = {0, 0, 0, 0, 0, 0, 0};
+  float mx = 0.f;
+
+  float my_anchor = 1.f;
+#pragma unroll
+  for (int j = 0; j < 32; ++j)
+    if (lane == j) my_anchor = c.use_anchors ? c.anchors[j] : 1.f;
+
+  int idxq[NCK], bq[NCK], kq[NCK];
+  float hanq[NCK], anq[NCK];
+#pragma unroll
+  for (int q = 0; q < NCK; ++q) {
+    const int i = q * 64 + lane;
+    idxq[q] = i < PD ? i : PD - 1;
+    chan_of_idx<VER>(idxq[q], A, TD, bq[q], kq[q]);
+    hanq[q] = head_is_wh(kq[q]) ? head_anchors[bq[q] * 2 + (kq[q] - 2)] : 0.f;
+    anq[q] = __shfl(my_anchor, (bq[q] * 2 + ((kq[q] == 3) ? 1 : 0)) & 31, 64);
+  }
+  const bool fast_ok = 5 * A <= 64 && !(VER == 4 && c.truth_thresh < 1.f);
+  const bool actF = lane < 5 * A;
+  const int bF = actF ? lane / 5 : 0, kF = actF ? lane - bF * 5 : 0;
+  const int idxF = bF * TD + kF;
+  const float hanF = head_is_wh(kF) ? head_anchors[bF * 2 + (kF - 2)] : 0.f;
+  const float anF = __shfl(my_anchor, (bF * 2 + ((kF == 3) ? 1 : 0)) & 31, 64);
+  const int pbA = lane < A ? lane : 0;
+  const float hanW = head_anchors[pbA * 2], hanH = head_anchors[pbA * 2 + 1];
+
+  float pn[NCK], tkn[NCK], pbn[4];
+  pn[0] = pn[1] = pn[2] = pn[3] = tkn[0] = tkn[1] = tkn[2] = tkn[3] = 0.f;
+  auto load_labels = [&](long long cell) { return y_true[cell * TD + (lane < 5 ? lane : 4)]; };
+  auto prefetch = [&](long long cell, bool fast) {
+    const float* T = y_true + cell * TD;
+    const float* Pc = t + cell * PD;
+    if (fast) {
+      pn[0] = Pc[idxF];
+    } else {
+#pragma unroll
+      for (int q = 0; q < NCK; ++q) {
+        pn[q] = Pc[idxq[q]];
+        tkn[q] = T[kq[q] >= 5 ? kq[q] : 4];
+      }
+    }
+    const float* P = Pc + pbA * TD;
+#pragma unroll
+    for (int j = 0; j < 4; ++j) pbn[j] = P[j];
+  };
+  auto no_object = [&](float tb) { return fast_ok && __shfl(tb, 4, 64) == 0.f; };
+
+  long long cell = wave0;
+  float tb0 = 0.f, tb1 = 0.f;
+  bool fastn = false;
+  if (cell < lp.cells) tb0 = load_labels(cell);
+  if (cell + nwaves < lp.cells) tb1 = load_labels(cell + nwaves);
+  if (cell < lp.cells) {
+    fastn = no_object(tb0);
+    prefetch(cell, fastn);
+  }
+  for (; cell < lp.cells; cell += nwaves) {
+    float pc[NCK], tkc[NCK], Pb[4];
+#pragma unroll
+    for (int q = 0; q < NCK; ++q) {
+      pc[q] = pn[q];
+      tkc[q] = tkn[q];
+    }
+    Pb[0] = as_stored(head_act(pbn[0], 0, 0.f));
+    Pb[1] = as_stored(head_act(pbn[1], 1, 0.f));
+    Pb[2] = as_stored(head_act(pbn[2], 2, hanW));
+    Pb[3] = as_stored(head_act(pbn[3], 3, hanH));
+    const float tbc = tb0;
+    const bool fast = fastn;
+    tb0 = tb1;
+    if (cell + 2 * nwaves < lp.cells) tb1 = load_labels(cell + 2 * nwaves);
+    if (cell + nwaves < lp.cells) {
+      fastn = no_object(tb0);
+      prefetch(cell + nwaves, fastn);
+    }
+    float* G = dt + cell * PD;
+    const float Tb[4] = {__shfl(tbc, 0, 64), __shfl(tbc, 1, 64), __shfl(tbc, 2, 64), __shfl(tbc, 3, 64)};
+    const float t4 = __shfl(tbc, 4, 64);
+    float iou, dI[4];
+    int resp;
+    cell_head_lanes<VER>(lp, lane, gw, gh, cell, Tb, t4, Pb, iou, dI, resp, part);
+    if (fast) {
+      const float iou_b = __shfl(iou, bF, 64);
+      const float d0 = __shfl(dI[0], bF, 64), d1 = __shfl(dI[1], bF, 64);
+      const float d2 = __shfl(dI[2], bF, 64), d3 = __shfl(dI[3], bF, 64);
+      const float r_b = (bF == resp) ? 1.f : 0.f;
+#pragma unroll
+      for (int q = 0; q < NCK; ++q)
+        if (q * 64 + lane < PD && kq[q] >= 5) G[q * 64 + lane] = 0.f;
+      if (actF) {
+        const float p = as_stored(head_act(pc[0], kF, hanF));
+        const float g = loss_channel<VER>(c, bF, kF, p, 0.f, t4, Tb, iou_b, d0, d1, d2, d3, anF, 0.f, r_b, part);
+        const float dv = head_act_grad(g * lp.inv_n, p, kF);
+        G[idxF] = dv;
+        mx = fmaxf(mx, fabsf(dv));
+      }
+      continue;
+    }
+#pragma unroll
+    for (int q = 0; q < NCK; ++q) {
+      const int base = q * 64;
+      if (base < PD) {
+        const bool active = (base + lane) < PD;
+        const int b = bq[q], k = kq[q];
+        const float iou_b = __shfl(iou, b, 64);
+        const float d0 = __shfl(dI[0], b, 64), d1 = __shfl(dI[1], b, 64);
+        const float d2 = __shfl(dI[2], b, 64), d3 = __shfl(dI[3], b, 64);
+        const float r_b = (b == resp) ? 1.f : 0.f;
+        if (active) {
+          const float p = as_stored(head_act(pc[q], k, hanq[q]));
+          const float g = loss_channel<VER>(c, b, k, p, tkc[q], t4, Tb, iou_b, d0, d1, d2, d3, anq[q], 0.f, r_b, part);
+          const float dv = head_act_grad(g * lp.inv_n, p, k);
+          G[idxq[q]] = dv;
+          mx = fmaxf(mx, fabsf(dv));
+        }
+      }
+    }
+  }
+
+#pragma unroll
+  for (int o = 32; o > 0; o >>= 1) mx = fmaxf(mx, __shfl_xor(mx, o, 64));
+  __shared__ double red[7][4];
+  __shared__ float wmax[4];
+  const int wave = threadIdx.x >> 6;
+#pragma unroll
+  for (int q = 0; q < 7; ++q) {
+    const double s = wave_reduce_sum(part[q]);
+    if (lane == 0) red[q][wave] = s;
+  }
+  if (lane == 0) wmax[wave] = mx;
+  __syncthreads();
+  if (threadIdx.x < 7) {
+    const double s = red[threadIdx.x][0] + red[threadIdx.x][1] + red[threadIdx.x][2] + red[threadIdx.x][3];
+    atomicAdd(&out[threadIdx.x], s * invN);
+  }
+  if (threadIdx.x == 64) {
+    const float m = fmaxf(fmaxf(wmax[0], wmax[1]), fmaxf(wmax[2], wmax[3]));
+    if (__builtin_bit_cast(unsigned, m) > *reinterpret_cast<volatile unsigned*>(amax))
+      atomicMax(amax, __builtin_bit_cast(unsigned, m));
   }
 }
 
@@ -592,6 +768,31 @@
   return check_launch("loss_kernel");
 }
 
+extern "C" int yolo_head_loss_fwd_bwd(const yolo_loss_cfg* cfg, const float* y_true, const float* t, const float* head_anchors,
+                                      double* loss_out, float* dt, void* amax_word, float grad_scale, void* decisions,
+                                      size_t decisions_bytes, void* stream) {
+  if (int rc = validate_cfg(cfg)) return rc;
+  YOLO_REQUIRE(y_true && t && head_anchors && loss_out && dt && amax_word, "head_loss: null pointer");
+  YOLO_REQUIRE(cfg->version == 3 || cfg->version == 4, "head_loss: version %d has no pointwise head with sigmoid classes",
+               cfg->version);
+  YOLO_REQUIRE(cfg->A * (5 + cfg->C) <= 256, "head_loss: %d channels per cell, at most 256", cfg->A * (5 + cfg->C));
+  LossParams lp;
+  lp.c = *cfg;
+  lp.cells = (long long)cfg->N * cfg->gh * cfg->gw;
+  lp.inv_n = grad_scale / (float)cfg->N;
+  lp.dec = (decisions != nullptr && decisions_bytes >= (size_t)lp.cells * 8) ? reinterpret_cast<int*>(decisions) : nullptr;
+  hipStream_t st = as_stream(stream);
+  if (hipMemsetAsync(loss_out, 0, 8 * sizeof(double), st) != hipSuccess || hipMemsetAsync(amax_word, 0, 4, st) != hipSuccess) {
+    set_error("head_loss: memset failed");
+    return YOLO_ERR_LAUNCH;
+  }
+  dim3 grid((unsigned)std::min<long long>((lp.cells + 3) / 4, 2048)), block(256);
+  unsigned* amax = reinterpret_cast<unsigned*>(amax_word);
+  if (cfg->version == 3) hipLaunchKernelGGL(head_loss_kernel<3>, grid, block, 0, st, lp, y_true, t, head_anchors, dt, amax, loss_out);
+  else hipLaunchKernelGGL(head_loss_kernel<4>, grid, block, 0, st, lp, y_true, t, head_anchors, dt, amax, loss_out);
+  return check_launch("head_loss_kernel");
+}
+
 extern "C" int yolo_metrics(const yolo_loss_cfg* cfg, const float* y_true, const float* y_pred, float recall_thresh,
                             double* out, void* stream) {
   if (int rc = validate_cfg(cfg)) return rc;
diff --git a/tf2_yolo_amd/engine.py b/tf2_yolo_amd/engine.py
--- a/tf2_yolo_amd/engine.py
+++ b/tf2_yolo_amd/engine.py
@@ -345,6 +345,8 @@
         self.act = {}
         self.training = False
         self._precision = "fp32"
+        self.heads_from_logits = False
+        self._head_scratch_word = None
         self.grad_ready_hook = None
         self.backward_begin_hook = None
         self._infer_scale_valid = False
@@ -743,7 +745,34 @@
                                      precision=self._precision)
             return
         self._conv_fwd(u, bias, u.t)
+        if training and self.heads_from_logits:
+            return
         ops.head_act_fwd(u.t, u.A, u.C, u.version, anchors, out=u.yact)
+
+    def head_loss_ready(self, losses):
+        from .losses import YoloLoss
+        if not self._head_loss_fused or self.anchors_trainable or len(losses) != len(self.outputs):
+            return False
+        versions = (3, 4) if self._head_loss_fused == 2 else (3,)
+        for l, o in zip(losses, self.outputs):
+            u = o.producer
+            if not (type(l) is YoloLoss and l.version in versions and u is not None and u.kind == "head"
+                    and u.version == l.version and u.anchors is not None and (u.A, u.C) == (l.bbox_num, l.class_num)
+                    and (o.h, o.w) == l.grid_shape and u.cout <= 256 and self._n_consumers.get(o.tid, 0) == 1):
+                return False
+        return True
+
+    def head_loss(self, i, loss, y_true, dt, loss_out):
+        u = self.outputs[i].producer
+        ops.head_loss_fwd_bwd(loss.cfg(self.batch), y_true, u.t, self._anchors_dev[u.name], self._head_bound_word(u),
+                              loss_out=loss_out, dt=dt)
+
+    def _head_bound_word(self, u):
+        if u.cpad and u.name in self._dyp_own:
+            return ops.planes_bound_word(self._dyp_own[u.name], self.batch * u.out.h * u.out.w, u.cpad)
+        if self._head_scratch_word is None:
+            self._head_scratch_word = torch.zeros(1, device=self.device, dtype=torch.int32)
+        return self._head_scratch_word
 
     def _fwd_upsample(self, u, training):
         if not training and self._infer_small_fuse and self._concat_planes and u.out.tid in self._up_producer:
@@ -940,12 +969,19 @@
         self._filter_and_data_grad(u, dy, dyp, dbias, grads)
 
     def _bwd_head(self, u, dout, grads):
-        dt = ops.head_act_bwd(u.yact, dout, u.A, u.C, u.version, self._anchors_dev.get(u.name),
-                              danchors=self._anchor_grad_views.get(u.name) if self.anchors_trainable else None)
+        from_logits = self.heads_from_logits
+        if from_logits:
+            dt = dout
+        else:
+            dt = ops.head_act_bwd(u.yact, dout, u.A, u.C, u.version, self._anchors_dev.get(u.name),
+                                  danchors=self._anchor_grad_views.get(u.name) if self.anchors_trainable else None)
         if not u.cpad:
             return self._filter_and_data_grad(u, dt, self._dyp(u, dt), self._gview(u.p_bias), grads)
         rows = self.batch * u.out.h * u.out.w
-        dtp = ops.split_planes_padded(dt, rows, u.out.c, out=self._next_dyp_buffer(u))
+        if from_logits and u.name in self._dyp_own:
+            dtp = ops.split_planes_padded_bound(dt, rows, u.out.c, out=self._next_dyp_buffer(u))
+        else:
+            dtp = ops.split_planes_padded(dt, rows, u.out.c, out=self._next_dyp_buffer(u))
         with self._beside_backward(dt):
             ops.zero_bytes(u.dw_pad)
             ops.conv2d_wgrad_planes(u.desc_pad, self._xplanes[u.src.tid], dtp, u.dw_pad)
diff --git a/tf2_yolo_amd/model.py b/tf2_yolo_amd/model.py
--- a/tf2_yolo_amd/model.py
+++ b/tf2_yolo_amd/model.py
@@ -1,3 +1,4 @@
+import contextlib
 import time
 
 import numpy as np
@@ -421,6 +422,22 @@
                 _ops.zero_bytes(self.net.grads)
             return None
 
+    @contextlib.contextmanager
+    def _heads_mode(self, with_metrics=False):
+        net = self.net
+        net.heads_from_logits = not with_metrics and net.head_loss_ready(self.loss)
+        try:
+            yield
+        finally:
+            net.heads_from_logits = False
+
+    def _losses_fwd_bwd(self, outs, y_list):
+        for i, (o, yt) in enumerate(zip(outs, y_list)):
+            if self.net.heads_from_logits:
+                self.net.head_loss(i, self.loss[i], yt, self._dpred[i], self._loss_bufs[i])
+            else:
+                self.loss[i].fwd_bwd(yt, o, grad_scale=1.0, dpred=self._dpred[i], loss_out=self._loss_bufs[i])
+
     def train_step_device(self, x, y_list, with_metrics=False):
         if self.optimizer is None:
             raise YoloHipError("compile() the model before training")
@@ -429,15 +446,15 @@
             bufs = self._captured_step(x, y_list)
             if bufs is not None:
                 return bufs, None
-        outs = self.net.forward(x, training=True)
-        if self._dpred is None or self._dpred[0].shape != outs[0].shape:
-            self._dpred = [torch.empty_like(o) for o in outs]
-        for i, (o, yt) in enumerate(zip(outs, y_list)):
-            self.loss[i].fwd_bwd(yt, o, grad_scale=1.0, dpred=self._dpred[i], loss_out=self._loss_bufs[i])
         mvals = None
-        if with_metrics:
-            mvals = [[m(yt, o) for m in ms] for ms, o, yt in zip(self.metrics, outs, y_list)]
-        self.net.backward(self._dpred)
+        with self._heads_mode(with_metrics):
+            outs = self.net.forward(x, training=True)
+            if self._dpred is None or self._dpred[0].shape != outs[0].shape:
+                self._dpred = [torch.empty_like(o) for o in outs]
+            self._losses_fwd_bwd(outs, y_list)
+            if with_metrics:
+                mvals = [[m(yt, o) for m in ms] for ms, o, yt in zip(self.metrics, outs, y_list)]
+            self.net.backward(self._dpred)
         if self._reducer is not None and self.net.anchors_trainable and self._reducer.world > 1:
             import torch.distributed as dist
             dist.all_reduce(self.net.anchor_grads, group=self._reducer.pg)
diff --git a/tf2_yolo_amd/ops.py b/tf2_yolo_amd/ops.py
--- a/tf2_yolo_amd/ops.py
+++ b/tf2_yolo_amd/ops.py
@@ -264,6 +264,25 @@
         raise YoloHipError("split_planes_padded: output buffer too small")
     check(_lib.load().yolo_split_planes_padded(_p(x), int(rows), int(c_src), int(c), _p(out), _stream()),
           "yolo_split_planes_padded")
+    return out
+
+
+def planes_bound_word(planes, rows, c):
+    n = planes_bytes(rows, c)
+    if planes.dtype != torch.uint8 or planes.numel() < n:
+        raise YoloHipError("planes_bound_word: buffer too small")
+    return planes[n - 256:n - 252]
+
+
+def split_planes_padded_bound(x, rows, c_src, out):
+    _chk_f32(x)
+    c = (c_src + 15) // 16 * 16
+    if x.numel() != rows * c_src:
+        raise YoloHipError("split_planes_padded_bound: tensor size does not match rows x C_src")
+    if out.numel() < planes_bytes(rows, c) or out.dtype != torch.uint8:
+        raise YoloHipError("split_planes_padded_bound: output buffer too small")
+    check(_lib.load().yolo_split_planes_padded_bound(_p(x), int(rows), int(c_src), int(c), _p(out), _stream()),
+          "yolo_split_planes_padded_bound")
     return out
 
 
@@ -918,6 +937,30 @@
     return loss_out, dpred
 
 
+def head_loss_fwd_bwd(cfg, y_true, t, head_anchors, amax_word, loss_out=None, dt=None, grad_scale=1.0, decisions=None):
+    _chk_f32(y_true, t, dt, head_anchors)
+    cells = cfg.N * cfg.gh * cfg.gw
+    if y_true.numel() != cells * (5 + cfg.C) or t.numel() != cells * cfg.A * (5 + cfg.C):
+        raise YoloHipError(f"head_loss: tensor sizes do not match cfg (cells={cells}, C={cfg.C}, A={cfg.A})")
+    if head_anchors.numel() != 2 * cfg.A:
+        raise YoloHipError(f"head_loss: need {cfg.A} (w, h) head anchors on the device")
+    if not amax_word.is_cuda or amax_word.numel() * amax_word.element_size() < 4:
+        raise YoloHipError("head_loss: amax_word must be at least one 32-bit word on the device")
+    if loss_out is None:
+        loss_out = torch.empty(8, device=t.device, dtype=torch.float64)
+    if dt is None:
+        dt = torch.empty_like(t)
+    elif dt.numel() != t.numel():
+        raise YoloHipError("head_loss: dt must have the shape of t")
+    if decisions is not None and (decisions.dtype != torch.int32 or decisions.numel() < 2 * cells or not decisions.is_cuda):
+        raise YoloHipError("head_loss: decisions must be an int32 CUDA tensor with 2 entries per cell")
+    check(_lib.load().yolo_head_loss_fwd_bwd(byref(cfg), _p(y_true), _p(t), _p(head_anchors), _p(loss_out), _p(dt),
+                                             _p(amax_word), float(grad_scale), _p(decisions),
+                                             0 if decisions is None else decisions.numel() * 4, _stream()),
+          "yolo_head_loss_fwd_bwd")
+    return loss_out, dt
+
+
 def metrics(cfg, y_true, y_pred, recall_thresh=0.5, out=None):
     _chk_f32(y_true, y_pred)
     if out is None:
diff --git a/tf2_yolo_amd/plan.py b/tf2_yolo_amd/plan.py
--- a/tf2_yolo_amd/plan.py
+++ b/tf2_yolo_amd/plan.py
@@ -32,6 +32,7 @@
         o.infer_onepass = on("YOLO_INFER_ONEPASS")
         o.infer_small_fuse = on("YOLO_INFER_SMALL_FUSE")
         o.dgrad_classes = on("YOLO_DGRAD_CLASSES")
+        o.head_loss_fused = int(env.get("YOLO_HEAD_LOSS_FUSED", "1") or 0)
         return o
 
 
```

Result: no change. 1102 (median of 6 runs) (+0.8%).
